# jkk-research/urban_road_filter

Hardware: AMD Instinct MI355X
Metric: scans/sec (64-ring x 2048-column cloud) (higher is better)
Workload: dtype f32+f64; 1 GPU; cfg3: batch of 1024 independent 64x2048 street sweeps per GPU, all three detectors + blind_spots, reference default parameters with ROI x,y widened to +-200 m, inputs resident in HBM (SoA x/y/z); scans_per_gpu=1024

## Files before the change

urban_road_filter_amd/csrc/urf_api.hip:

```cpp
#include <hip/hip_runtime.h>

#include <cmath>
#include <cstdio>
#include <cstdlib>
#include <cstring>
#include <ctime>
#include <string>
#include <vector>
#if defined(__SSE2__)
#include <emmintrin.h>
#include <xmmintrin.h>
#endif

#include "urf.h"
#ifdef URF_ENABLE_TEST_HOOKS
#include "urf_test_hooks.h"
#endif
#include "urf_internal.hpp"
#include "urf_kernels.hpp"
#include "urf_front.hpp"

#define URF_ASYNC_SLOTS 4
static_assert(URF_ASYNC_SLOTS == URF_MAX_IN_FLIGHT, "include/urf.h documents the number of sweeps in flight");

template <class T, bool Host = false>
struct lazy_buf {
    T* p = nullptr;
    size_t cap = 0;
    lazy_buf() = default;
    lazy_buf(const lazy_buf&) = delete;
    lazy_buf& operator=(const lazy_buf&) = delete;
    ~lazy_buf() { release(); }
    void release()
    {
        if (p)
            (void)(Host ? hipHostFree(p) : hipFree(p));
        p = nullptr;
        cap = 0;
    }
};

#define URF_SCRATCH_SCANS(X)                                                                                                     \
    X(rx, sstride) X(ry, sstride) X(rz, sstride) X(rec, sstride)                                                                 \
    X(sr, sstride) X(sz, sstride) X(sslot, sstride) X(ssrt16, sstride) X(ssrt, sstride) X(wsg, sstride)                          \
    X(big_r, sstride) X(big_z, sstride) X(big_i, sstride)                                                                        \
    X(tile_roi, max_tiles) X(roi_bits, max_tiles * (URF_TILE / 64)) X(troff, max_tiles * (URF_MAX_CHANNELS + 1))                 \
    X(tsoff, max_tiles * (URF_MAX_SECTORS + 1)) X(tmaxs, max_tiles * URF_MAX_CHANNELS)                                           \
    X(rpre, URF_MAX_CHANNELS * (max_tiles + 1)) X(rstart, URF_MAX_CHANNELS * max_tiles)                                          \
    X(angle, URF_MAX_CHANNELS) X(ring_thr, URF_MAX_CHANNELS * 4) X(ring_lut, URF_LUT_CELLS) X(ring_cnt, URF_MAX_CHANNELS)        \
    X(ring_off, URF_MAX_CHANNELS + 1)                                                                                            \
    X(sec_cnt, URF_MAX_SECTORS) X(sec_run, URF_MAX_SECTORS) X(sec_off, URF_MAX_SECTORS + 1) X(star_hit, URF_MAX_SECTORS)         \
    X(star_first, URF_MAX_SECTORS) X(star_list_mid, URF_MAX_SECTORS) X(star_list_big, URF_MAX_SECTORS)                           \
    X(star_list_runs, URF_MAX_SECTORS) X(tie_list, URF_MAX_SECTORS) X(tie_post, URF_MAX_SECTORS)                                 \
    X(table_upto, 1) X(table_redo, 1) X(redo_list, 1) X(table_cause, 1)                                                          \
    X(nan_mask, 4) X(nan_list, 2 * URF_MAX_CHANNELS) X(vis, URF_MAX_CHANNELS)                                                    \
    X(maxdist, URF_MAX_CHANNELS) X(quad, 4)                                                                                      \
    X(curb_cnt, URF_MAX_CHANNELS) X(curb_az, URF_MAX_CHANNELS * URF_CURB_LIST)                                                   \
    X(sufmin, URF_MAX_CHANNELS * URF_DEG_CELLS) X(premax, URF_MAX_CHANNELS * URF_DEG_CELLS)                                      \
    X(stop_f, URF_DEG_CELLS) X(stop_b, URF_DEG_CELLS)                                                                            \
    X(win, URF_MAX_CHANNELS * URF_DEG_CELLS)                                                                                     \
    X(info, 1)                                                                                                                   \
    X(front_ok, 1) X(front_pres, max_tiles * 64) X(front_maxs, max_tiles * 64) X(front_lane_ring, 64)                            \
    X(front_ring_lane, URF_MAX_CHANNELS) X(front_cand, front_cand_cap) X(front_all, front_cand_cap) X(front_ncand, 1)             \
    X(front_list, 1) X(front_st, URF_FRONT_ST_WORDS)
#define URF_SCRATCH_SLOTS(X) X(star_count, 8) X(ring_hint, 1)
#define URF_SCRATCH_CAPTURE(X) X(valpha, sstride) X(seckey, sstride) X(ringkey, sstride) X(rd2, sstride) X(caz, sstride)
#define URF_SCRATCH_ROW_MAJOR(X) X(tx, sstride) X(ty, sstride) X(tz, sstride) X(rows_v, 64) X(rows_ok, 1)
enum urf_scratch_group { URF_SCR_ALWAYS, URF_SCR_CAPTURE, URF_SCR_ROW_MAJOR };

struct __attribute__((visibility("hidden"))) urf_policy {
    uint32_t* flags = nullptr;
    uint64_t epoch = 1;
    bool speculate = true, use_hint = true;
    bool slot_lists = false, slot_nan = false, slot_ties = false;
    int front_mode = 1;
    uint32_t front_tpb = 0;
    bool want_ring_sorted = false;
    bool front_direct = false, front_off = false;
    bool front_rows = false, rows_oom = false, rows_used = false;
    uint32_t rows_probation = 0;

    template <class T>
    void set(T& field, T value)
    {
        if (field != value) {
            field = value;
            epoch++;
        }
    }
    void forget_front()
    {
        set(front_direct, false);
        set(front_off, false);
        flags[URF_FLAG_FRONT_HANDED_BACK] = flags[URF_FLAG_FRONT_ALL_HANDED_BACK] = 0;
    }
    int fold(urf_ctx* c, hipStream_t st);
    void probation_sweep() { lapse(front_rows); }
    void probation_batch(const urf_kargs& a) { lapse(a.front && front_mode != 2 && a.n_scans < URF_FRONT_MIN_SCANS); }
    void lapse(bool counts)
    {
        if (counts && !rows_used && rows_probation && --rows_probation == 0)
            epoch++;
    }
    bool on_redo(int status)
    {
        switch (status) {
        case URF_STATUS_REDO_TABLE: set(speculate, false); return true;
        case URF_STATUS_REDO_HINT: set(use_hint, false); return true;
        case URF_STATUS_REDO_LISTS: set(slot_lists, true); return true;
        case URF_STATUS_REDO_NAN: set(slot_nan, true); return true;
        case URF_STATUS_REDO_TIES: set(slot_ties, true); return true;
        }
        return false;
    }
    void plan(urf_kargs& a, const urf_dev_params& dp, bool slot, bool general_only) const
    {
        a.table_lookahead = speculate ? URF_TABLE_LOOKAHEAD : 0u;
        a.table_hint = (speculate && use_hint) ? 1u : 0u;
        a.optimistic = slot ? ((speculate ? URF_OPT_NO_REPAIR : 0u) | (slot_lists ? 0u : URF_OPT_NO_LISTS) | (slot_nan ? 0u : URF_OPT_NO_NAN) |
                               (slot_ties ? 0u : URF_OPT_NO_TIES)) : 0u;
        const unsigned L = (unsigned)dp.p.channels;
        const bool lasers = L == 64u || L == 32u || L == 16u;
        a.front_lsh = L == 16u ? 4u : (L == 32u ? 5u : 6u);
        const bool shape = front_mode != 0 && !front_off && !general_only && !want_ring_sorted && a.capture == 0 &&
                           lasers && dp.p.curbPoints == 5 && a.tiles <= URF_FRONT_MAX_TILES;
        const bool small_ok = front_rows && (rows_used || rows_probation > 0) && (L == 64u || front_mode == 2);
        a.front = (shape && (slot ? small_ok : (front_mode == 2 || small_ok || a.n_scans >= (L == 64u ? URF_FRONT_MIN_SCANS : (L == 32u ? URF_FRONT_MIN_SCANS_32 : URF_FRONT_MIN_SCANS_16))))) ? 1u : 0u;
        a.front_sight = (shape && !a.front && !front_rows && !rows_oom && (L == 64u || front_mode == 2)) ? 1u : 0u;
        a.front_tpb = front_tpb ? front_tpb : (a.n_scans >= URF_FRONT_TPB_SCANS ? URF_FRONT_TPB_LARGE : (a.n_scans >= 16u ? URF_FRONT_TPB_SMALL : 1u));
        a.front_lists = (a.front && !front_direct && !slot) ? 1u : 0u;
        a.front_rows = (a.front && front_rows) ? 1u : 0u;
    }
};

enum urf_last_kind { URF_LAST_NONE, URF_LAST_SOA, URF_LAST_PC2, URF_LAST_SWEEP };
struct urf_last_call {
    int kind = URF_LAST_NONE;
    uint32_t scans = 0;
    urf_kargs a;
    urf_dev_params dp;
    uint32_t row = 0;
    uint64_t gen = 0;
};

struct urf_ctx {
    int device = 0;
    uint32_t max_points = 0, max_batch = 0;
    uint32_t max_tiles = 0;
    uint32_t sstride = 0;
    uint32_t debug_flags = 0;
    unsigned n_cus = 256;
    hipStream_t own_stream = nullptr;
    hipStream_t stream = nullptr;
    urf_params params;
    urf_dev_params dp;
    urf_kargs k;
    std::vector<void*> allocs;
    lazy_buf<float> sx, sy, sz;
    struct slot_t {
        lazy_buf<uint8_t, true> h_in;
        lazy_buf<uint8_t> d_raw;
        lazy_buf<uint8_t, true> h_labels;
        lazy_buf<uint8_t> d_labels;
        lazy_buf<urf_scan_info, true> h_info;
        hipEvent_t ev_done = nullptr;
        hipGraph_t graph = nullptr;
        hipGraphExec_t exec = nullptr;
        uint64_t key[3] = { 0, 0, 0 };
        urf_kargs cap_a;
        urf_dev_params cap_dp;
        bool pending = false, used = false;
        uint64_t gen = 0;
        uint32_t n_points = 0, ticket = 0;
        uint32_t point_step = 0, off_x = 0, off_y = 0, off_z = 0;
        bool planes = false;
    } slots[URF_ASYNC_SLOTS];
    bool streams_made = false;
    urf_policy pol;
    uint32_t n_rerun = 0;
    hipStream_t row_stream[URF_ASYNC_SLOTS] = { nullptr, nullptr, nullptr, nullptr };
    hipEvent_t ev_main = nullptr;
    uint64_t main_seq = 1;
    uint64_t row_seen[URF_ASYNC_SLOTS] = { 0, 0, 0, 0 };
    uint64_t row_gen[URF_ASYNC_SLOTS] = { 0, 0, 0, 0 };
    uint32_t next_ticket = 0;
    lazy_buf<unsigned long long> ord_keys;
    lazy_buf<uint32_t> ord_pos;
    lazy_buf<uint32_t> ord_cls;
    lazy_buf<uint32_t> ord_lists;
    lazy_buf<float> mk_d;
    lazy_buf<uint32_t> mk_pos;
    lazy_buf<uint8_t> mk_red;
    lazy_buf<float> mk_out;
    lazy_buf<int32_t> mk_ghost;
    uint32_t* compact_cnt = nullptr;
    lazy_buf<urf_u32x4> cl_tiles;
    lazy_buf<uint32_t> cl_lists;
    float* d_newY = nullptr;
    urf_beam* d_beams = nullptr;
    uint32_t beams_cap = 0;
    int capture = 0;
    bool timing = false;
    std::vector<std::vector<hipEvent_t>> timing_events;
    size_t timing_used = 0;
    uint32_t* offsets_copy = nullptr;
    hipStream_t side_stream = nullptr;
    hipEvent_t ev_fork = nullptr, ev_join = nullptr;
    urf_last_call last;
    std::string last_error;
    double ht[8] = { 0, 0, 0, 0, 0, 0, 0, 0 };
    bool ht_on = false;
};

#define URF_HIP(ctx, call)                                                              \
    do {                                                                                \
        hipError_t e_ = (call);                                                         \
        if (e_ != hipSuccess) {                                                         \
            (ctx)->last_error = std::string(#call) + ": " + hipGetErrorString(e_);      \
            return e_ == hipErrorOutOfMemory ? URF_ERR_OOM : URF_ERR_HIP;               \
        }                                                                               \
    } while (0)

template <class T>
static int dev_alloc(urf_ctx* c, T** p, size_t count)
{
    void* v = nullptr;
    URF_HIP(c, hipMalloc(&v, (count ? count : 1) * sizeof(T)));
    c->allocs.push_back(v);
    *p = (T*)v;
    return URF_OK;
}

template <class T, bool Host>
static int grow(urf_ctx* c, lazy_buf<T, Host>& b, size_t count, hipStream_t st = nullptr)
{
    if (count <= b.cap)
        return URF_OK;
    if (st)
        URF_HIP(c, hipStreamSynchronize(st));
    b.release();
    void* v = nullptr;
    URF_HIP(c, Host ? hipHostMalloc(&v, count * sizeof(T), hipHostMallocDefault) : hipMalloc(&v, count * sizeof(T)));
    b.p = (T*)v;
    b.cap = count;
    return URF_OK;
}

template <class F>
static void scratch_walk(const urf_ctx* c, urf_kargs& k, F&& f)
{
    const size_t sstride = c->sstride, max_tiles = c->max_tiles, front_cand_cap = k.front_cand_cap;
#define URF_X_SCANS(field, n) f(URF_SCR_ALWAYS, k.field, (size_t)c->max_batch, (size_t)(n));
#define URF_X_SLOTS(field, n) f(URF_SCR_ALWAYS, k.field, (size_t)URF_ASYNC_SLOTS, (size_t)(n));
#define URF_X_CAPTURE(field, n) f(URF_SCR_CAPTURE, k.field, (size_t)c->max_batch, (size_t)(n));
#define URF_X_ROW_MAJOR(field, n) f(URF_SCR_ROW_MAJOR, k.field, (size_t)c->max_batch, (size_t)(n));
    URF_SCRATCH_SCANS(URF_X_SCANS)
    URF_SCRATCH_SLOTS(URF_X_SLOTS)
    URF_SCRATCH_CAPTURE(URF_X_CAPTURE)
    URF_SCRATCH_ROW_MAJOR(URF_X_ROW_MAJOR)
#undef URF_X_SCANS
#undef URF_X_SLOTS
#undef URF_X_CAPTURE
#undef URF_X_ROW_MAJOR
}

static int scratch_alloc(urf_ctx* c, urf_scratch_group group)
{
    int rc = URF_OK;
    scratch_walk(c, c->k, [&](urf_scratch_group g, auto*& p, size_t rows, size_t n) {
        if (g == group && !p && rc == URF_OK)
            rc = dev_alloc(c, &p, rows * n);
    });
    return rc;
}

int urf_policy::fold(urf_ctx* c, hipStream_t st)
{
    if (front_mode != 0 && !front_rows && !rows_oom && flags[URF_FLAG_ROWS_SIGHTED]) {
        URF_HIP(c, hipStreamSynchronize(st));
        if (scratch_alloc(c, URF_SCR_ROW_MAJOR) == URF_OK) {
            set(front_rows, true);
            rows_probation = 16;
            forget_front();
        } else {
            set(rows_oom, true);
            c->last_error.clear();
        }
    }
    if (front_rows && flags[URF_FLAG_ROWS_TAKEN])
        set(rows_used, true);
    if (flags[URF_FLAG_LOOKAHEAD_FAILED])
        set(speculate, false);
    if (flags[URF_FLAG_HINT_FAILED])
        set(use_hint, false);
    if (flags[URF_FLAG_FRONT_HANDED_BACK])
        set(front_direct, true);
    if (flags[URF_FLAG_FRONT_ALL_HANDED_BACK] && front_mode != 2)
        set(front_off, true);
    return URF_OK;
}

static void beam_init(std::vector<urf_beam>& beams, int rep, float width)
{
    beams.resize((size_t)rep);
    const float off = (float)(0.5 * (double)width);
    for (int i = 0; i < rep; i++) {
        const float fi = (float)((double)(i * 2) * M_PI / (double)rep);
        if (std::fabs(std::tan(fi)) > 1) {
            beams[i].yx = 1;
            beams[i].d = (float)std::tan(0.5 * M_PI - (double)fi);
            beams[i].o = std::fabs(off / std::sin(fi));
        } else {
            beams[i].yx = 0;
            beams[i].d = std::tan(fi);
            beams[i].o = std::fabs(off / std::cos(fi));
        }
    }
}

static float urf_angle_threshold(float angle_filter)
{
    auto alpha_of = [](float b) { return (float)((double)(urf_acosf(b) * 180.0f) / M_PI); };
    auto from_key = [](uint32_t k) {
        const uint32_t one = 0x3f800000u;
        const uint32_t u = k <= one ? 0x80000000u | (one - k) : k - one - 1u;
        float f;
        std::memcpy(&f, &u, 4);
        return f;
    };
    if (!(alpha_of(1.0f) <= angle_filter))
        return 2.0f;
    uint32_t lo = 0, hi = 2u * 0x3f800000u + 1u;
    while (lo < hi) {
        const uint32_t mid = lo + (hi - lo) / 2;
        if (alpha_of(from_key(mid)) <= angle_filter)
            hi = mid;
        else
            lo = mid + 1;
    }
    return from_key(lo);
}

static int upload_params(urf_ctx* c)
{
    const urf_params& p = c->params;
    urf_dev_params& dp = c->dp;
    dp.p = p;
    dp.slope_param = (float)((double)p.angleFilter3 * (M_PI / 180));
    dp.Kfi = (float)((double)p.sectors / (2 * M_PI));
    dp.fwd_limit = 360.0f - p.beamZone;
    dp.bwd_limit = 0.0f + p.beamZone;
    dp.inv_cp = 1.0f / (float)p.curbPoints;
    dp.x_angle_thr = urf_angle_threshold(p.angleFilter1);
    dp.z_angle_thr = urf_angle_threshold(p.angleFilter2);
    dp.sec_keybits = 1;
    while ((1u << dp.sec_keybits) <= (unsigned)p.sectors)
        dp.sec_keybits++;
    dp.ring_keybits = 1;
    while ((1u << dp.ring_keybits) <= (unsigned)p.channels)
        dp.ring_keybits++;
    dp.exp_flags = c->debug_flags;
    dp.sector_margin = URF_FAST_SECTOR_ERR * (p.sectors > 360 ? (float)p.sectors / 360.0f : 1.0f);
    std::vector<urf_beam> beams;
    beam_init(beams, p.sectors, p.beam_width);
    URF_HIP(c, hipMemcpyAsync(c->d_beams, beams.data(), beams.size() * sizeof(urf_beam), hipMemcpyHostToDevice, c->stream));
    URF_HIP(c, hipStreamSynchronize(c->stream));
    return URF_OK;
}

extern "C" int urf_create(urf_ctx** out, int device_id, uint32_t max_points, uint32_t max_batch)
{
    if (!out || max_points == 0 || max_batch == 0)
        return URF_ERR_INVALID_ARG;
    *out = nullptr;
    const unsigned long long max_tiles = ((unsigned long long)max_points + URF_TILE - 1) / URF_TILE;
    const unsigned long long sstride = max_tiles * URF_TILE + URF_SCAN_PAD;
    if (max_tiles > URF_MAX_TILES || sstride * max_batch >= (1ull << 32))
        return URF_ERR_CAPACITY;
    int ndev = 0;
    if (hipGetDeviceCount(&ndev) != hipSuccess || ndev <= 0 || device_id < 0 || device_id >= ndev)
        return URF_ERR_NO_DEVICE;
    urf_ctx* c = new urf_ctx();
    c->device = device_id;
    c->max_points = max_points;
    c->max_batch = max_batch;
    c->max_tiles = (uint32_t)max_tiles;
    c->sstride = (uint32_t)sstride;
    int rc = URF_OK;
    auto fail = [&](int code) {
        urf_destroy(c);
        return code;
    };
    if (hipSetDevice(device_id) != hipSuccess)
        return fail(URF_ERR_NO_DEVICE);
    if (hipStreamCreateWithFlags(&c->own_stream, hipStreamNonBlocking) != hipSuccess)
        return fail(URF_ERR_HIP);
    c->stream = c->own_stream;
    {
        hipDeviceProp_t prop;
        if (hipGetDeviceProperties(&prop, device_id) == hipSuccess && prop.multiProcessorCount > 0)
            c->n_cus = (unsigned)prop.multiProcessorCount;
    }
    urf_default_params(&c->params);
    std::memset(&c->k, 0, sizeof(c->k));
    std::memset(&c->last.a, 0, sizeof(c->last.a));
    urf_kargs& k = c->k;
    k.front_cand_cap = max_points / 8 > 4096 ? max_points / 8 : 4096;
    if ((rc = scratch_alloc(c, URF_SCR_ALWAYS)) != URF_OK || (rc = dev_alloc(c, &c->offsets_copy, (size_t)max_batch + 1)) != URF_OK ||
        (rc = dev_alloc(c, &c->compact_cnt, (size_t)max_batch * c->max_tiles * 4)) != URF_OK ||
        (rc = dev_alloc(c, &c->d_newY, (size_t)max_points)) != URF_OK || (rc = dev_alloc(c, &c->d_beams, (size_t)URF_MAX_SECTORS)) != URF_OK)
        return fail(rc);
    {
        urf_wu* tab = nullptr;
        const size_t nt = (size_t)max_points + 32;
        if ((rc = dev_alloc(c, &tab, nt)) != URF_OK)
            return fail(rc);
        hipLaunchKernelGGL(k_walk_table, dim3((unsigned)((nt + 255) / 256)), dim3(256), 0, c->stream, tab, (unsigned)nt);
        k.walk_tab = tab;
    }
    k.sstride = c->sstride;
    if (const char* e = std::getenv("URF_FRONT_TPB"))
        c->pol.front_tpb = (uint32_t)std::atoi(e) > 0 ? (uint32_t)std::atoi(e) : c->pol.front_tpb;
    {
        void* hp = nullptr;
        if (hipHostMalloc(&hp, URF_FLAG_WORDS * sizeof(uint32_t), hipHostMallocMapped) != hipSuccess)
            return fail(URF_ERR_HIP);
        c->pol.flags = (uint32_t*)hp;
        std::memset(hp, 0, URF_FLAG_WORDS * sizeof(uint32_t));
        if (hipMemset(k.ring_hint, 0, URF_ASYNC_SLOTS * sizeof(uint32_t)) != hipSuccess)
            return fail(URF_ERR_HIP);
        void* dp_ = nullptr;
        if (hipHostGetDevicePointer(&dp_, hp, 0) != hipSuccess)
            return fail(URF_ERR_HIP);
        k.flags = (uint32_t*)dp_;
// ... 1412 lines not shown
```

urban_road_filter_amd/csrc/urf_device.hpp:

```cpp
#ifndef URF_DEVICE_HPP
#define URF_DEVICE_HPP

#include <hip/hip_runtime.h>

#include "urf_internal.hpp"
#include "urf_libm.h"

#define URF_WAVE 64

__device__ __forceinline__ unsigned urf_lane() { return __lane_id(); }

__device__ __forceinline__ unsigned long long urf_match_any(unsigned key, unsigned nbits)
{
    unsigned long long m = ~0ull;
    for (unsigned b = 0; b < nbits; b++) {
        const bool bit = (key >> b) & 1u;
        const unsigned long long bal = __ballot(bit);
        m &= bit ? bal : ~bal;
    }
    return m;
}

__device__ __forceinline__ unsigned long long urf_match_any_fast(unsigned key, unsigned nbits)
{
// ... 45 lines not shown
}
__device__ __forceinline__ unsigned urf_wave_max(unsigned v)
{
    URF_DPP_STEP(urf_umax, 0u, 0x111, 0xf);
    URF_DPP_STEP(urf_umax, 0u, 0x112, 0xf);
    URF_DPP_STEP(urf_umax, 0u, 0x114, 0xf);
    URF_DPP_STEP(urf_umax, 0u, 0x118, 0xf);
    URF_DPP_STEP(urf_umax, 0u, 0x142, 0xa);
    URF_DPP_STEP(urf_umax, 0u, 0x143, 0xc);
    return (unsigned)__builtin_amdgcn_readlane((int)v, 63);
}

__device__ __forceinline__ unsigned urf_uadd(unsigned a, unsigned b) { return a + b; }
__device__ __forceinline__ unsigned urf_wave_scan_add(unsigned v)
{
    URF_DPP_STEP(urf_uadd, 0u, 0x111, 0xf);
    URF_DPP_STEP(urf_uadd, 0u, 0x112, 0xf);
    URF_DPP_STEP(urf_uadd, 0u, 0x114, 0xf);
    URF_DPP_STEP(urf_uadd, 0u, 0x118, 0xf);
    URF_DPP_STEP(urf_uadd, 0u, 0x142, 0xa);
    URF_DPP_STEP(urf_uadd, 0u, 0x143, 0xc);
    return v;
}
__device__ __forceinline__ unsigned urf_wave_scan_max(unsigned v)
{
    URF_DPP_STEP(urf_umax, 0u, 0x111, 0xf);
    URF_DPP_STEP(urf_umax, 0u, 0x112, 0xf);
    URF_DPP_STEP(urf_umax, 0u, 0x114, 0xf);
    URF_DPP_STEP(urf_umax, 0u, 0x118, 0xf);
    URF_DPP_STEP(urf_umax, 0u, 0x142, 0xa);
    URF_DPP_STEP(urf_umax, 0u, 0x143, 0xc);
    return v;
}

__device__ __forceinline__ void urf_wave_lds_sync()
{
    __builtin_amdgcn_fence(__ATOMIC_RELEASE, "wavefront");
    __builtin_amdgcn_wave_barrier();
    __builtin_amdgcn_fence(__ATOMIC_ACQUIRE, "wavefront");
}

__device__ __forceinline__ void urf_scan_range(const urf_kargs& a, unsigned s, unsigned& off, unsigned& len)
{
    if (a.offsets) {
        off = a.offsets[s];
        len = a.offsets[s + 1] - off;
        len = len > a.max_len ? a.max_len : len;
    } else {
        off = s * a.n_per_scan;
        len = a.n_per_scan;
    }
}

__device__ __forceinline__ unsigned urf_sbase(const urf_kargs& a, unsigned s) { return s * a.sstride; }

__device__ __forceinline__ unsigned urf_ring_slot(const urf_kargs& a, unsigned s, unsigned C, unsigned c, unsigned ntiles,
                                                  unsigned p)
{
    const unsigned* P = a.rpre + ((size_t)s * C + c) * (a.tiles + 1);
    unsigned lo = 0, hi = ntiles;
    while (hi - lo > 1) {
        const unsigned mid = (lo + hi) >> 1;
        if (P[mid] <= p)
            lo = mid;
        else
            hi = mid;
    }
    return lo * URF_TILE + a.rstart[((size_t)s * C + c) * a.tiles + lo] + (p - P[lo]);
}


__device__ __forceinline__ double urf_div_pi(double a)
{
    const double rpi = 0x1.45f306dc9c883p-2;
    const double q = a * rpi;
    const double r = __builtin_fma(-q, URF_PI_D, a);
    return __builtin_fma(r, rpi, q);
}

__device__ __forceinline__ bool urf_in_roi(const urf_params& p, float x, float y, float z)
{
    return x >= p.min_X && x <= p.max_X && y >= p.min_Y && y <= p.max_Y &&
           z >= p.min_Z && z <= p.max_Z && (x + y) + z != 0.0f;
}

__device__ __forceinline__ float urf_vertical_angle(float x, float y, float z)
{
    const float d = (float)__builtin_sqrt((double)x * (double)x + (double)y * (double)y + (double)z * (double)z);
    float b = __builtin_fabsf(z) / d;
    if (b < -1.0f)
        b = -1.0f;
    else if (b > 1.0f)
        b = 1.0f;
    if (z < 0.0f)
        return (float)urf_div_pi((double)(urf_acosf(b) * 180.0f));
    return (float)(urf_div_pi((double)(urf_asinf(b) * 180.0f)) + 90.0);
}

__device__ __forceinline__ float urf_azimuth(float x, float y, float* d_out)
{
    const float d = (float)__builtin_sqrt((double)x * (double)x + (double)y * (double)y);
    *d_out = d;
    float b = __builtin_fabsf(x) / d;
    if (b < -1.0f)
        b = -1.0f;
    else if (b > 1.0f)
        b = 1.0f;
    const double t = urf_div_pi((double)(urf_asinf(b) * 180.0f));
    if (x >= 0.0f && y <= 0.0f)
        return (float)t;
    if (x >= 0.0f && y > 0.0f)
        return (float)(180.0 - t);
    if (x < 0.0f && y >= 0.0f)
        return (float)(180.0 + t);
    return (float)(360.0 - t);
}

__device__ __forceinline__ unsigned urf_sector(float x, float y, float Kfi, unsigned sectors)
{
    float fi = urf_atan2f(y, x);
    if (fi < 0.0f)
        fi = (float)((double)fi + 2.0 * URF_PI_D);
    const int f = (int)(fi * Kfi);
    return ((unsigned)f >= sectors) ? 0u : (unsigned)f;
}

#define URF_FAST_ATAN_ERR 2.0e-6f
__device__ __forceinline__ float urf_fast_atan2f(float y, float x)
{
    const float ax = __builtin_fabsf(x), ay = __builtin_fabsf(y);
    const float mx = ax > ay ? ax : ay, mn = ax > ay ? ay : ax;
    const float t = mn * __builtin_amdgcn_rcpf(mx);
    const bool big = t > 0.41421357f;
    const float tt = big ? (t - 1.0f) * __builtin_amdgcn_rcpf(t + 1.0f) : t;
    const float v = tt * tt;
    float q = -0.06451718869358958f;
    q = __builtin_fmaf(q, v, 0.10743668324830098f);
    q = __builtin_fmaf(q, v, -0.14263949753605723f);
    q = __builtin_fmaf(q, v, 0.1999954031495797f);
    q = __builtin_fmaf(q, v, -0.33333331760434554f);
    float r = __builtin_fmaf(tt * v, q, tt);
    if (big)
        r += 0.78539816339744831f;
    if (ay > ax)
        r = 1.57079632679489662f - r;
    if (x < 0.0f)
        r = 3.14159265358979324f - r;
    return y < 0.0f ? -r : r;
}

#define URF_FAST_VALPHA_ERR 3.0e-4f
#define URF_FAST_MIN 1.0e-15f
#define URF_FAST_MAX 1.0e18f
__device__ __forceinline__ bool urf_fast_vertical_angle(float x, float y, float z, float* out)
{
    const float rho = __builtin_amdgcn_sqrtf(x * x + y * y);
    *out = urf_fast_atan2f(rho, -z) * 57.295779513082323f;
    return (rho >= URF_FAST_MIN) & (rho <= URF_FAST_MAX) & (__builtin_fabsf(z) <= 4.0f * rho);
}

#define URF_FAST_MIN2 2.0e-30f
#define URF_FAST_MAX2 1.0e36f
__device__ __forceinline__ bool urf_fast_cot(float x, float y, float z, float* u_out, bool* planar_ok)
{
    const float rho2 = x * x + y * y;
    const float u = -z * __builtin_amdgcn_rsqf(rho2);
    *u_out = u;
    *planar_ok = (rho2 >= URF_FAST_MIN2) & (rho2 <= URF_FAST_MAX2);
    return *planar_ok & (__builtin_fabsf(u) <= URF_LUT_UMAX);
}

__host__ __device__ __forceinline__ double urf_cot_deg(double deg)
{
    deg = deg < 1.0 ? 1.0 : (deg > 179.0 ? 179.0 : deg);
    const double h = (90.0 - deg) * (URF_PI_D / 360.0);
    const double v = h * h;
    double sn = -1.0 / 121645100408832000.0;
    sn = __builtin_fma(sn, v, 1.0 / 355687428096000.0);
    sn = __builtin_fma(sn, v, -1.0 / 1307674368000.0);
    sn = __builtin_fma(sn, v, 1.0 / 6227020800.0);
    sn = __builtin_fma(sn, v, -1.0 / 39916800.0);
    sn = __builtin_fma(sn, v, 1.0 / 362880.0);
    sn = __builtin_fma(sn, v, -1.0 / 5040.0);
    sn = __builtin_fma(sn, v, 1.0 / 120.0);
    sn = __builtin_fma(sn, v, -1.0 / 6.0);
    sn = __builtin_fma(sn * v, h, h);
    double cs = 1.0 / 6402373705728000.0;
    cs = __builtin_fma(cs, v, -1.0 / 20922789888000.0);
    cs = __builtin_fma(cs, v, 1.0 / 87178291200.0);
    cs = __builtin_fma(cs, v, -1.0 / 479001600.0);
    cs = __builtin_fma(cs, v, 1.0 / 3628800.0);
    cs = __builtin_fma(cs, v, -1.0 / 40320.0);
    cs = __builtin_fma(cs, v, 1.0 / 720.0);
    cs = __builtin_fma(cs, v, -1.0 / 24.0);
    cs = __builtin_fma(cs, v, 0.5);
    cs = __builtin_fma(-cs, v, 1.0);
    const double th = sn / cs;
    return 2.0 * th / (1.0 - th * th);
}

struct urf_ring_thr { float x, y, z, w; };
__device__ __forceinline__ urf_ring_thr urf_ring_thresholds(float angle, float interval, float e)
{
    const double a = (double)angle, iv = (double)interval, ee = (double)e;
    urf_ring_thr t;
    t.x = (float)urf_cot_deg(a + iv + ee);
    t.y = (float)urf_cot_deg(a + iv - ee);
    t.z = (float)urf_cot_deg(a - iv + ee);
    t.w = (float)urf_cot_deg(a - iv - ee);
    return t;
}

__device__ __forceinline__ float urf_ring_threshold(float angle, float interval, float e, unsigned which)
{
    const double a = (double)angle, iv = (double)interval, ee = (double)e;
    const double arg = which == 0 ? a + iv + ee : (which == 1 ? a + iv - ee : (which == 2 ? a - iv + ee : a - iv - ee));
    return (float)urf_cot_deg(arg);
}

#define URF_FAST_SECTOR_ERR 2.5e-4f
__device__ __forceinline__ float urf_fast_polar(float x, float y)
{
    const float fi = urf_fast_atan2f(y, x);
    return fi < 0.0f ? fi + 6.28318530717958648f : fi;
}
__device__ __forceinline__ int urf_fast_sector_of(float fi, float x, float y, float Kfi, unsigned sectors, float margin)
{
    const float mx = __builtin_fmaxf(__builtin_fabsf(x), __builtin_fabsf(y));
    const float u = fi * Kfi;
    const float f = __builtin_floorf(u);
    const float fr = u - f;
    const bool ok = (mx >= URF_FAST_MIN) & (mx <= URF_FAST_MAX) & (fr > margin) & (fr < 1.0f - margin) & (f >= 0.0f) &
                    (f < (float)sectors);
    return ok ? (int)f : -1;
}
__device__ __forceinline__ int urf_fast_sector_ranged(float fi, float Kfi, unsigned sectors, float margin)
{
    const float u = fi * Kfi;
    const float f = __builtin_floorf(u);
    const float fr = u - f;
    const bool ok = (fr > margin) & (fr < 1.0f - margin) & (f < (float)sectors);
    return ok ? (int)f : -1;
}
__device__ __forceinline__ int urf_fast_sector(float x, float y, float Kfi, unsigned sectors, float margin)
{
    return urf_fast_sector_of(urf_fast_polar(x, y), x, y, Kfi, sectors, margin);
}

#define URF_FAST_AZ_ERR 5.0e-4f
#define URF_FAST_AZ_RATIO 1024.0f
__device__ __forceinline__ float urf_fast_az_eps(float az)
{
    const float delta = __builtin_fminf(__builtin_fabsf(az - 90.0f), __builtin_fabsf(az - 270.0f));
    return URF_FAST_AZ_ERR + 6.0e-4f * __builtin_amdgcn_rcpf(__builtin_fmaxf(delta, 0.04f));
}
__device__ __forceinline__ float urf_fast_azimuth_of(float fi)
{
    const float az = fi * 57.295779513082323f + 90.0f;
    return az >= 360.0f ? az - 360.0f : az;
}
static_assert(URF_TILE == URF_REC_SRC_MASK + 1u, "the record's source field holds an index inside a tile");
__device__ __forceinline__ unsigned urf_az_code(float az)
{
    const unsigned c = (unsigned)(az * URF_REC_AZ_SCALE);
    return c < URF_REC_AZ_UNKNOWN - 1u ? c : URF_REC_AZ_UNKNOWN - 1u;
}
__device__ __forceinline__ float urf_az_decode(unsigned code)
{
    return code == URF_REC_AZ_UNKNOWN ? URF_AZ_UNKNOWN : ((float)code + 0.5f) * URF_REC_AZ_STEP;
}
__device__ __forceinline__ bool urf_fast_az_ok(float x, float y)
{
    const float ax = __builtin_fabsf(x), ay = __builtin_fabsf(y);
    return (ay * URF_FAST_AZ_RATIO >= ax) & (ay >= URF_FAST_MIN) & (ax <= URF_FAST_MAX) & (ay <= URF_FAST_MAX);
}
__device__ __forceinline__ bool urf_fast_azimuth(float x, float y, float* out)
{
    *out = urf_fast_azimuth_of(urf_fast_polar(x, y));
    return urf_fast_az_ok(x, y);
}

__device__ __forceinline__ bool urf_in_beam(const urf_beam& b, float x, float y)
{
    if (b.yx) {
        const float c = b.d * y;
        return (c - b.o) < x && x < (c + b.o);
    }
    const float c = b.d * x;
    return (c - b.o) < y && y < (c + b.o);
}

__device__ __forceinline__ float urf_sqrt_rn_normal(float x)
{
    float r = __builtin_amdgcn_sqrtf(x);
    const float rd = __uint_as_float(__float_as_uint(r) - 1u), ru = __uint_as_float(__float_as_uint(r) + 1u);
    const float ed = __builtin_fmaf(-rd, r, x), eu = __builtin_fmaf(-ru, r, x);
    r = ed <= 0.0f ? rd : r;
    r = eu > 0.0f ? ru : r;
    return r;
}

__device__ __forceinline__ unsigned urf_fbits(float f) { return __float_as_uint(f); }

#endif
```

urban_road_filter_amd/csrc/urf_front.hpp:

```cpp
#ifndef URF_FRONT_HPP
#define URF_FRONT_HPP

#define URF_FRONT_HPRE 8u
#ifndef URF_FRONT_HPOST
#define URF_FRONT_HPOST 8u
#endif
#define URF_FRONT_LANES 64u
#define URF_FRONT_STEPS (URF_TILE / URF_FRONT_LANES)
#define URF_FRONT_MIN_SCANS 192u
#define URF_FRONT_MIN_SCANS_32 0xffffffffu
#define URF_FRONT_MIN_SCANS_16 0xffffffffu
#define URF_FRONT_TPB_SMALL 2u
#define URF_FRONT_TPB_LARGE 4u
#define URF_FRONT_TPB_SCANS 512u
#define URF_FRONT_MAX_TILES 128u
#define URF_FRONT_RING_NONE 0x7fu
#define URF_FC_XZ 1u
#define URF_FC_ZZ 2u
#define URF_FC_EDGE_X 4u
#define URF_FC_EDGE_Z 8u
#ifndef URF_FRONT_NT
#define URF_FRONT_NT 0
#endif
#ifndef URF_FRONT_WAVES
#define URF_FRONT_WAVES 5
#endif

struct urf_front_thr {
    float y, z, below;
};
__device__ __forceinline__ urf_front_thr urf_front_load_thr(const urf_kargs& a, unsigned s, unsigned C, unsigned e, unsigned nR)
{
    urf_front_thr t;
    const bool valid = e < nR;
    const float4 tv = ((const float4*)a.ring_thr)[(size_t)s * C + (valid ? e : 0u)];
    const float bl = a.ring_thr[((size_t)s * C + ((valid && e) ? e - 1u : 0u)) * 4];
    t.y = valid ? tv.y : __builtin_inff();
    t.z = tv.z;
    t.below = e ? bl : __builtin_inff();
    return t;
}

__device__ __forceinline__ __amdgpu_buffer_rsrc_t urf_buf(const void* p, unsigned bytes)
{
    return __builtin_amdgcn_make_buffer_rsrc((void*)p, 0, (int)bytes, 0x00020000);
}
#define URF_OOB 0xffffffffu

__device__ __forceinline__ void urf_front_src(const urf_kargs& a, unsigned s, unsigned off, unsigned ok, const float*& gx, const float*& gy, const float*& gz)
{
    const bool rows = ok == URF_FRONT_ROWS;
    const size_t o = rows ? (size_t)urf_sbase(a, s) : (size_t)off;
    gx = (rows ? (const float*)a.tx : a.x) + o;
    gy = (rows ? (const float*)a.ty : a.y) + o;
    gz = (rows ? (const float*)a.tz : a.z) + o;
}

__global__ __launch_bounds__(256) void k_transpose(urf_kargs a)
{
    __shared__ float T[3][64 * 33];
    const unsigned s = blockIdx.y, t = blockIdx.x, tid = threadIdx.x;
    const unsigned lsh = a.front_lsh, L = 1u << lsh, wsh = 11u - lsh, W = 1u << wsh, RS = W + 1u;
    static_assert(URF_TILE == 2048u, "a tile's columns: 1 << (11 - lsh)");
    if (a.front_ok[s] != URF_FRONT_ROWS)
        return;
    unsigned off, len;
    urf_scan_range(a, s, off, len);
    const unsigned F = len >> lsh, f0 = t * W;
    if (f0 >= F)
        return;
    const unsigned c = tid & (W - 1u), r8 = tid >> wsh, RP = 256u >> wsh;
    const bool in = f0 + c < F;
    float vx[8], vy[8], vz[8];
#pragma unroll
    for (unsigned j = 0; j < 8; j++) {
        const size_t i = (size_t)off + (size_t)(j * RP + r8) * F + f0 + (in ? c : 0u);
        vx[j] = a.x[i];
        vy[j] = a.y[i];
        vz[j] = a.z[i];
    }
#pragma unroll
    for (unsigned j = 0; j < 8; j++) {
        T[0][(j * RP + r8) * RS + c] = vx[j];
        T[1][(j * RP + r8) * RS + c] = vy[j];
        T[2][(j * RP + r8) * RS + c] = vz[j];
    }
    __syncthreads();
    const size_t ob = (size_t)urf_sbase(a, s) + (size_t)f0 * L;
    const unsigned nf = F - f0 < W ? F - f0 : W;
#pragma unroll
    for (unsigned j = 0; j < 8; j++) {
        const unsigned v = j * 256u + tid, f = v >> lsh, l = v & (L - 1u);
        if (f < nf) {
            a.tx[ob + v] = T[0][l * RS + f];
            a.ty[ob + v] = T[1][l * RS + f];
            a.tz[ob + v] = T[2][l * RS + f];
        }
    }
}

#define URF_FO_ADOPT 0x20000000u
#define URF_FO_NONE 0x40000000u
#define URF_FO_FAIL 0x80000000u
__device__ __noinline__ unsigned urf_front_open(const float* tab, unsigned nR, float interval, float x, float y, float z, unsigned sectors, float Kfi,
                                                unsigned E, unsigned econf)
{
    const urf_exact_key ek = urf_exact_keys_body(tab, nR, interval, x, y, z, sectors, Kfi);
    unsigned r = sectors ? ((ek.sector + 1u) & 0x7ffu) << 1 : 0u;
    if (ek.ring == URF_RING_NONE)
        r |= URF_FO_NONE;
    else if (x == 0.0f && y == 0.0f)
        r |= URF_FO_FAIL;
    else if (ek.ring == E)
        r |= 1u;
    else if (!econf)
        r |= 1u | URF_FO_ADOPT | (ek.ring << 12);
    else
        r |= URF_FO_FAIL;
    return r;
}

#define URF_FRONT_CBUF 256u
__device__ __forceinline__ void urf_front_flush(const urf_kargs& a, unsigned s, urf_u2* cbuf, unsigned& ncb, bool& overflow)
{
    if (ncb == 0u)
        return;
    urf_wave_lds_sync();
    unsigned base = 0;
    if (urf_lane() == 0u)
        base = atomicAdd(&a.front_ncand[s], ncb);
    base = (unsigned)__builtin_amdgcn_readfirstlane((int)base);
    for (unsigned j = urf_lane(); j < ncb; j += 64u) {
        if (base + j < a.front_cand_cap)
            a.front_cand[(size_t)s * a.front_cand_cap + base + j] = cbuf[j];
        else
            overflow = true;
    }
    urf_wave_lds_sync();
    ncb = 0;
}
__device__ __forceinline__ void urf_front_push(urf_u2* cbuf, unsigned& ncb, bool has, unsigned idx, unsigned what)
{
    const unsigned long long m = __ballot(has);
    if (has)
        cbuf[ncb + urf_popc_below(m)] = urf_u2{ idx, what };
    ncb += (unsigned)__popcll(m);
}

template <bool STAR, bool BEAM, unsigned L>
__device__ __forceinline__ void urf_front_body(const urf_kargs& a, const urf_dev_params& dp, urf_u2* cbuf)
{
    const unsigned s = blockIdx.y, b = blockIdx.x, lane = threadIdx.x;
    unsigned off, len;
    urf_scan_range(a, s, off, len);
    const unsigned TPB = a.front_tpb;
    const unsigned t_first = b * TPB;
    if (t_first * URF_TILE >= len)
        return;
    const unsigned ok = a.front_ok[s];
    if (ok == 0u)
        return;
    constexpr unsigned C = L;
    constexpr unsigned STEPS = URF_TILE / L;
    static_assert(L == 64u || L == 32u || L == 16u, "a firing fills the wave, half of it or a quarter");
    const unsigned K = (unsigned)dp.p.sectors;
    const unsigned nf = (len + L - 1u) / L;
    const unsigned F0 = t_first * STEPS;
    const unsigned F1 = F0 + TPB * STEPS < nf ? F0 + TPB * STEPS : nf;
    const unsigned Fs = F0 > URF_FRONT_HPRE ? F0 - URF_FRONT_HPRE : 0u;
    const unsigned Fe = F1 + URF_FRONT_HPOST < nf ? F1 + URF_FRONT_HPOST : nf;
    const bool from_start = Fs == 0u;
    const bool to_end = Fe == nf;
    static_assert(URF_FRONT_HPRE % 4u == 0u && STEPS % 4u == 0u, "the march runs in groups of four firings");
    const unsigned sb = urf_sbase(a, s);
    const float *gx, *gy, *gz;
    urf_front_src(a, s, off, ok, gx, gy, gz);
    const __amdgpu_buffer_rsrc_t brec = urf_buf(a.rec + sb, len * 4u);
    const __amdgpu_buffer_rsrc_t bsr = urf_buf(a.sr + sb, a.tiles * URF_TILE * 4u), bsz = urf_buf(a.sz + sb, a.tiles * URF_TILE * 4u);
    const __amdgpu_buffer_rsrc_t bss = urf_buf(a.sslot + sb, a.tiles * URF_TILE * 2u);
    const unsigned nR = a.info[s].n_rings;
    const unsigned upto_v = a.table_upto[s];
    const unsigned upto = ok == URF_FRONT_ROWS ? 0u : (nR < C ? upto_v : 0xffffffffu);
    const float* const tab = a.angle + (size_t)s * dp.p.channels;
    const float curbH = dp.p.curbHeight;
    const bool use_x = dp.p.x_zero_method != 0, use_z = dp.p.z_zero_method != 0;

    unsigned E = lane;
    bool econf = false;
    urf_front_thr th = urf_front_load_thr(a, s, C, E, nR);
    bool failed = false, overflow = false;
    unsigned long long failed_m = 0;
    unsigned ncb = 0;

    float w0 = 0.f, w1 = 0.f, w2 = 0.f, w3 = 0.f, w4 = 0.f, w5 = 0.f, w6 = 0.f, w7 = 0.f, w8 = 0.f, w9 = 0.f, w10 = 0.f;
    unsigned fwA = 0, fwB = 0, fwC = 0;
    unsigned wc = 0;
    unsigned tot = 0, nin = 0;
    double maxs = 0.0;
    unsigned pw = 0;
    unsigned troi = 0, tstar = 0;
    int stepkey_v = (int)URF_SEC_NONE, stepcnt_v = 0;
    int stepkey_w = (int)URF_SEC_NONE, stepcnt_w = 0;

    auto step = [&](auto ph, const unsigned f, const float x, const float y, const float z) {
        constexpr unsigned PH = decltype(ph)::value;
        const unsigned stp = f % STEPS;
        const unsigned i = f * L + lane;
        const bool roi = (L == 64u || lane < L) && i < len && urf_in_roi(dp.p, x, y, z);
        const unsigned long long roim = __ballot(roi);
        if (PH == 1u && lane == 0u) {
            if (L == 64u)
                a.roi_bits[((size_t)s * a.tiles + f / STEPS) * STEPS + stp] = roim;
            else if (L == 32u)
                ((uint32_t*)(a.roi_bits + (size_t)s * a.tiles * (URF_TILE / 64u)))[f] = (uint32_t)roim;
            else
                ((uint16_t*)(a.roi_bits + (size_t)s * a.tiles * (URF_TILE / 64u)))[f] = (uint16_t)roim;
        }
        if (roim == 0ull)
            return;
        const float rho2 = x * x + y * y;
        const float u = -z * __builtin_amdgcn_rsqf(rho2);
        const bool fast = (rho2 >= URF_FAST_MIN2) & (rho2 <= URF_FAST_MAX2) & (__builtin_fabsf(u) <= URF_LUT_UMAX) & roi;
        const bool on_f = fast & (u >= th.y) & (u <= th.z) & (u < th.below);
        float fi = 0.f;
        int fs = -1;
        if (PH == 1u) {
            fi = urf_fast_polar(x, y);
            if (STAR)
                fs = fast ? urf_fast_sector_ranged(fi, dp.Kfi, K, dp.sector_margin) : -1;
        }
        bool on = on_f;
        const bool open = roi && !(on_f && (PH != 1u || !STAR || fs >= 0));
        if (open) {
            const unsigned r = urf_front_open(tab, nR, dp.p.interval, x, y, z, (PH == 1u && STAR) ? K : 0u, dp.Kfi, E, econf ? 1u : 0u);
            on = (r & 1u) != 0u;
            fs = (int)((r >> 1) & 0x7ffu) - 1;
            if (r & URF_FO_FAIL)
                failed = true;
            if (PH == 1u && (r & URF_FO_NONE) && i >= upto)
                a.table_redo[s] = 1u;
            if (r & URF_FO_ADOPT) {
                E = (r >> 12) & 0x7fu;
                th = urf_front_load_thr(a, s, C, E, nR);
            }
        }
        if (PH == 1u) {
            const unsigned azc_v = urf_az_code(urf_fast_azimuth_of(fi));
            const unsigned azc = urf_fast_az_ok(x, y) ? azc_v : URF_REC_AZ_UNKNOWN;
            __builtin_amdgcn_raw_buffer_store_b32((azc << URF_REC_AZ_SHIFT) | (on ? E : URF_FRONT_RING_NONE), brec, (L == 64u || lane < L) ? i * 4u : URF_OOB, 0, URF_FRONT_NT);
            if (STAR) {
                unsigned sk = (unsigned)fs;
                if (BEAM && roi && !urf_in_beam(a.beams[fs < 0 ? 0 : fs], x, y))
                    sk = URF_SEC_NONE;
                const unsigned long long psm = roim & __builtin_amdgcn_ballot_w64(sk != URF_SEC_NONE) & __builtin_amdgcn_ballot_w64((int)sk >= 0);
                const bool ons = roi && sk != URF_SEC_NONE && (int)sk >= 0;
                const unsigned src = psm ? (unsigned)__ffsll((long long)psm) - 1u : 0u;
                const unsigned f0 = psm ? (unsigned)__builtin_amdgcn_readlane((int)sk, (int)src) : URF_SEC_NONE;
                failed_m |= psm & __builtin_amdgcn_ballot_w64(sk != f0);
                const unsigned so = (f / STEPS) * URF_TILE + tstar + urf_popc_below(psm);
                const unsigned o4 = ons ? so * 4u : URF_OOB;
                const float pr = urf_sqrt_rn_normal(rho2);
                failed_m |= psm & ~(__builtin_amdgcn_ballot_w64(rho2 >= 0x1p-90f) & __builtin_amdgcn_ballot_w64(rho2 <= 0x1p126f));
                __builtin_amdgcn_raw_buffer_store_b32(__float_as_uint(pr), bsr, o4, 0, URF_FRONT_NT);
                __builtin_amdgcn_raw_buffer_store_b32(__float_as_uint(z), bsz, o4, 0, URF_FRONT_NT);
                __builtin_amdgcn_raw_buffer_store_b16((short)((stp * L + lane) | (on ? 0u : URF_SLOT_OFF)), bss, ons ? so * 2u : URF_OOB, 0, URF_FRONT_NT);
                if (STEPS <= 64u || stp < 64u) {
                    stepkey_v = lane == stp ? (int)f0 : stepkey_v;
                    stepcnt_v = lane == stp ? (int)__popcll(psm) : stepcnt_v;
                } else {
                    stepkey_w = lane == stp - 64u ? (int)f0 : stepkey_w;
                    stepcnt_w = lane == stp - 64u ? (int)__popcll(psm) : stepcnt_w;
                }
                tstar += (unsigned)__popcll(psm);
            }
            troi += (unsigned)__popcll(roim);
        }
        if (on) {
            if (PH == 1u) {
                const double s2 = (double)x * (double)x + (double)y * (double)y;
                maxs = s2 > maxs ? s2 : maxs;
                pw |= 1u << (f & 31u);
            }
            econf = true;
            w0 = w1; w1 = w2; w2 = w3; w3 = w4; w4 = w5; w5 = w6; w6 = w7; w7 = w8; w8 = w9; w9 = w10;
            w10 = z;
            fwA = __builtin_amdgcn_alignbit(fwB, fwA, 16);
            fwB = __builtin_amdgcn_alignbit(fwC, fwB, 16);
            fwC = __builtin_amdgcn_alignbit(f - Fs, fwC, 16);
            wc = wc < 11u ? wc + 1u : 11u;
            if (PH >= 1u)
                tot++;
            if (PH == 1u)
                nin++;
        }
        if (PH == 0u)
            return;
        const bool full = wc == 11u;
        const bool c_in = on & (tot >= 6u) & (tot - 5u <= nin);
        const bool p_in = on & (tot >= 4u) & (tot - 3u <= nin);
        const float a5 = __builtin_fabsf(w5);
        float m1, m2, t1, t2;
        asm("v_max3_f32 %0, |%1|, |%2|, |%3|" : "=v"(t1) : "v"(w0), "v"(w1), "v"(w2));
        asm("v_max3_f32 %0, %1, |%2|, |%3|" : "=v"(t1) : "v"(t1), "v"(w3), "v"(w4));
        asm("v_max_f32_e64 %0, %1, |%2|" : "=v"(m1) : "v"(t1), "v"(w5));
        asm("v_max3_f32 %0, |%1|, |%2|, |%3|" : "=v"(t2) : "v"(w10), "v"(w9), "v"(w8));
        asm("v_max3_f32 %0, %1, |%2|, |%3|" : "=v"(t2) : "v"(t2), "v"(w7), "v"(w6));
        asm("v_max_f32_e64 %0, %1, |%2|" : "=v"(m2) : "v"(t2), "v"(w5));
        const bool hz = ((m1 - a5 >= curbH) | (m2 - a5 >= curbH)) & (__builtin_fabsf(m1 - m2) >= 0.05f);
        const bool hx = ((__builtin_fabsf(w5 - w7) >= curbH) | (__builtin_fabsf(w10 - w7) >= curbH)) & (__builtin_fabsf(w5 - w10) >= 0.05f);
        bool zz = false, xz = false, ez = false, ex = false;
        if (use_z) {
            zz = c_in && full && hz;
            if (!from_start)
                ez = c_in && !full;
        }
        if (use_x) {
            xz = p_in && full && hx;
            if (!from_start)
                ex = p_in && !full;
        }
        if (__ballot(zz | xz | ez | ex) != 0ull) {
            urf_front_push(cbuf, ncb, zz | ez, ((fwA & 0xffffu) + Fs) * L + lane, zz ? URF_FC_ZZ : URF_FC_EDGE_Z);
            urf_front_push(cbuf, ncb, xz | ex, ((fwB & 0xffffu) + Fs) * L + lane, xz ? URF_FC_XZ : URF_FC_EDGE_X);
            if (ncb > URF_FRONT_CBUF - 128u)
                urf_front_flush(a, s, cbuf, ncb, overflow);
        }
    };
    auto pres_end = [&](const unsigned pt) {
        if (lane < L)
            a.front_pres[(size_t)s * a.tiles * 64u + (size_t)pt * L + lane] = pw;
        pw = 0;
    };
    auto tile_end = [&](const unsigned t) {
        const size_t row = (size_t)s * a.tiles + t;
        if (L == 64u) {
            a.front_pres[row * 64u + lane] = pw;
            pw = 0;
        }
        if (lane == 0)
            a.tile_roi[row] = troi;
        if (STAR && STEPS > 32u) {
            constexpr unsigned NH = STEPS > 64u ? 2u : 1u;
            unsigned fk[NH], sbase_h[NH];
            unsigned carry = 0, total = 0;
#pragma unroll
            for (unsigned h = 0; h < NH; h++) {
                const unsigned key = (unsigned)(h ? stepkey_w : stepkey_v), sc = (unsigned)(h ? stepcnt_w : stepcnt_v);
                const unsigned k1 = key != URF_SEC_NONE ? key + 1u : 0u;
                unsigned m = urf_wave_scan_max(k1);
                m = m > carry ? m : carry;
                unsigned exc = (unsigned)__shfl_up((int)m, 1);
                exc = lane == 0 ? carry : exc;
                if (__ballot(k1 != 0u && k1 < exc) != 0ull)
                    failed = true;
                fk[h] = m;
                carry = (unsigned)__builtin_amdgcn_readlane((int)m, 63);
                const unsigned sinc = urf_wave_scan_add(sc) + total;
                sbase_h[h] = sinc - sc;
                total = (unsigned)__builtin_amdgcn_readlane((int)sinc, 63);
            }
            for (unsigned k0 = 0; k0 <= K; k0 += 64u) {
                const unsigned k = k0 + lane;
                unsigned cnt = 0;
#pragma unroll
                for (unsigned h = 0; h < NH; h++) {
                    unsigned lo = 0;
#pragma unroll
                    for (unsigned st = 32u; st > 0; st >>= 1) {
                        const unsigned v = (unsigned)__shfl((int)fk[h], (int)(lo + st - 1u));
                        lo += v < k + 1u ? st : 0u;
                    }
                    const unsigned v = (unsigned)__shfl((int)fk[h], (int)lo);
                    lo += (lo == 63u && v < k + 1u) ? 1u : 0u;
                    cnt += lo;
                }
                unsigned so = total;
#pragma unroll
                for (unsigned h = 0; h < NH; h++) {
                    const unsigned v = (unsigned)__shfl((int)sbase_h[h], (int)(cnt & 63u));
                    so = (cnt >> 6) == h ? v : so;
                }
                if (k <= K)
                    a.tsoff[row * (K + 1) + k] = (uint16_t)so;
            }
        }
        if (STAR && STEPS == 32u) {
            const unsigned k1 = (lane < URF_FRONT_STEPS && (unsigned)stepkey_v != URF_SEC_NONE) ? (unsigned)stepkey_v + 1u : 0u;
            const unsigned fk = urf_wave_scan_max(k1);
            unsigned exc = (unsigned)__shfl_up((int)fk, 1);
            exc = lane == 0 ? 0u : exc;
            if (__ballot(k1 != 0u && k1 < exc) != 0ull)
                failed = true;
            const unsigned sc = lane < URF_FRONT_STEPS ? (unsigned)stepcnt_v : 0u;
            const unsigned sinc = urf_wave_scan_add(sc);
            const unsigned sbase_l = sinc - sc;
            for (unsigned k0 = 0; k0 <= K; k0 += 64u) {
                const unsigned k = k0 + lane;
                unsigned lo = 0;
#pragma unroll
                for (unsigned st = URF_FRONT_STEPS / 2; st > 0; st >>= 1) {
                    const unsigned v = (unsigned)__shfl((int)fk, (int)(lo + st - 1u));
                    lo += v < k + 1u ? st : 0u;
                }
                {
                    const unsigned v = (unsigned)__shfl((int)fk, (int)lo);
                    lo += (lo == URF_FRONT_STEPS - 1u && v < k + 1u) ? 1u : 0u;
                }
                const unsigned so = (unsigned)__shfl((int)sbase_l, (int)lo);
                if (k <= K)
                    a.tsoff[row * (K + 1) + k] = (uint16_t)so;
            }
        }
        troi = 0;
        tstar = 0;
        stepkey_v = (int)URF_SEC_NONE;
        stepcnt_v = 0;
        stepkey_w = (int)URF_SEC_NONE;
        stepcnt_w = 0;
    };

    float px[4], py[4], pz[4];
    auto ld = [&](const unsigned j, const unsigned f) {
        const unsigned i = f * L + lane, o = ((L == 64u || lane < L) && i < len) ? i : len - 1u;
        px[j] = gx[o];
        py[j] = gy[o];
        pz[j] = gz[o];
    };
#pragma unroll
    for (unsigned j = 0; j < 4; j++)
        ld(j, Fs + j);
    for (unsigned f = Fs; f < F0; f += 4) {
#pragma unroll
        for (unsigned j = 0; j < 4; j++) {
            step(std::integral_constant<unsigned, 0u>{}, f + j, px[j], py[j], pz[j]);
            ld(j, f + j + 4u);
        }
    }
    for (unsigned f = F0; f < F1; f += 4) {
#pragma unroll
        for (unsigned j = 0; j < 4; j++) {
            if (f + j < F1)
                step(std::integral_constant<unsigned, 1u>{}, f + j, px[j], py[j], pz[j]);
            ld(j, f + j + 4u);
        }
        if (L != 64u && (((f + 4u) & 31u) == 0u || f + 4u >= F1))
            pres_end(f >> 5);
        if (((f + 4u) % STEPS) == 0u || f + 4u >= F1) {
            tile_end(f / STEPS);
            if (failed_m != 0ull || __ballot(failed | overflow) != 0ull) {
                a.front_ok[s] = 0u;
                if (ok == URF_FRONT_ROWS)
                    a.table_redo[s] = 1u;
                return;
            }
        }
    }
    for (unsigned f = F1; f < Fe; f += 4) {
#pragma unroll
        for (unsigned j = 0; j < 4; j++) {
            if (f + j < Fe)
                step(std::integral_constant<unsigned, 2u>{}, f + j, px[j], py[j], pz[j]);
            ld(j, f + j + 4u);
        }
    }
    if (!to_end) {
        const unsigned fr[5] = { fwA >> 16, fwB & 0xffffu, fwB >> 16, fwC & 0xffffu, fwC >> 16 };
#pragma unroll
        for (unsigned e = 0; e < 5; e++) {
            const unsigned back = 4u - e;
            const bool in = tot > back && tot - back <= nin;
            const unsigned what = (use_z ? URF_FC_EDGE_Z : 0u) | ((use_x && e >= 2u) ? URF_FC_EDGE_X : 0u);
            if (ncb > URF_FRONT_CBUF - 64u)
                urf_front_flush(a, s, cbuf, ncb, overflow);
            urf_front_push(cbuf, ncb, in && what != 0u, (fr[e] + Fs) * L + lane, what);
        }
    }
    urf_front_flush(a, s, cbuf, ncb, overflow);
    a.front_maxs[((size_t)s * a.tiles + b) * 64u + lane] = (unsigned long long)__double_as_longlong(maxs);
    if (econf) {
        const unsigned o1 = atomicCAS(&a.front_lane_ring[(size_t)s * 64u + lane], 0xffffffffu, E);
        const unsigned o2 = atomicCAS(&a.front_ring_lane[(size_t)s * C + E], 0xffffffffu, lane);
        failed = failed | (o1 != 0xffffffffu && o1 != E) | (o2 != 0xffffffffu && o2 != lane);
    }
    if (failed_m != 0ull || __ballot(failed | overflow) != 0ull) {
        a.front_ok[s] = 0u;
        if (ok == URF_FRONT_ROWS)
            a.table_redo[s] = 1u;
    }
}

template <unsigned L>
__device__ __forceinline__ void urf_front_kernel(const urf_kargs& a, const urf_dev_params& dp, urf_u2* cbuf)
{
    if (!dp.p.star_shaped_method)
        urf_front_body<false, false, L>(a, dp, cbuf);
    else if (!dp.p.starbeam_filter)
        urf_front_body<true, false, L>(a, dp, cbuf);
    else
        urf_front_body<true, true, L>(a, dp, cbuf);
}
#define URF_FRONT_KERNEL(name, L)                                                                                                             \
    __global__ __launch_bounds__(64) __attribute__((amdgpu_waves_per_eu(URF_FRONT_WAVES, URF_FRONT_WAVES))) void name(urf_kargs a, urf_dev_params dp) \
    {                                                                                                                                         \
        __shared__ urf_u2 cbuf[URF_FRONT_CBUF];                                                                                               \
        urf_front_kernel<L>(a, dp, cbuf);                                                                                                     \
    }
URF_FRONT_KERNEL(k_front, 64u)
URF_FRONT_KERNEL(k_front32, 32u)
URF_FRONT_KERNEL(k_front16, 16u)

#define URF_FRONT_ST_WORDS 72u
#define URF_FINISH_CHUNK 768u
#ifndef URF_FINISH_THREADS
#define URF_FINISH_THREADS 256
#endif
struct urf_finish_shared {
    unsigned n[64];
    unsigned ring[64];
    unsigned ncurb[URF_FRONT_LANES];
    int q[4];
    unsigned n_pend;
    unsigned nx, nz;
    unsigned qsum[URF_FINISH_THREADS / 64][64];
};

__device__ __forceinline__ unsigned urf_front_prev(const unsigned* P, unsigned lsh, unsigned l, unsigned f)
{
    unsigned t = f >> 5;
    unsigned w = P[(t << lsh) + l] & ((1u << (f & 31u)) - 1u);
    while (w == 0u) {
        if (t == 0u)
            return 0xffffffffu;
        t--;
        w = P[(t << lsh) + l];
    }
    return t * 32u + 31u - (unsigned)__clz((int)w);
}
__device__ __forceinline__ unsigned urf_front_next(const unsigned* P, unsigned lsh, unsigned ntiles, unsigned l, unsigned f)
{
    unsigned t = f >> 5;
    unsigned w = (f & 31u) == 31u ? 0u : P[(t << lsh) + l] & ~((2u << (f & 31u)) - 1u);
    while (w == 0u) {
        t++;
        if (t >= ntiles)
            return 0xffffffffu;
        w = P[(t << lsh) + l];
    }
    return t * 32u + (unsigned)__ffs((int)w) - 1u;
}

__global__ __launch_bounds__(URF_FINISH_THREADS) void k_front_finish(urf_kargs a, urf_dev_params dp, unsigned part)
{
    __shared__ urf_finish_shared S;
    extern __shared__ unsigned sh_finish[];
    const unsigned s = blockIdx.x, tid = threadIdx.x;
    const unsigned ok = a.front_ok[s];
    if (!ok)
        return;
    unsigned off, len;
    urf_scan_range(a, s, off, len);
    const unsigned ntiles = (len + URF_TILE - 1) / URF_TILE;
    const unsigned lsh = a.front_lsh, L = 1u << lsh, lm = L - 1u;
    const unsigned npt = (((len + lm) >> lsh) + 31u) >> 5;
    const unsigned C = (unsigned)dp.p.channels, K = (unsigned)dp.p.sectors;
    const urf_scan_info in = a.info[s];
    if (in.status != URF_OK)
        return;
    unsigned* const P = sh_finish;
    uint16_t* const B = (uint16_t*)(sh_finish + a.tiles * 64u);
    urf_u2* const chunk = (urf_u2*)(sh_finish + a.tiles * 96u);
    unsigned* const st = a.front_st + (size_t)s * URF_FRONT_ST_WORDS;
    urf_u2* const pend = a.front_all + (size_t)s * a.front_cand_cap;
    const unsigned sb = urf_sbase(a, s);
    const float *gx, *gy, *gz;
    urf_front_src(a, s, off, ok, gx, gy, gz);
    auto passed = [&](unsigned idx, unsigned flag) {
        const unsigned e = atomicAdd(&S.n_pend, 1u);
        if (e < a.front_cand_cap)
            pend[e] = urf_u2{ idx, flag };
    };
    unsigned m_from = 0;
    if (part != 2u) {
    const urf_u2* const cand = a.front_cand + (size_t)s * a.front_cand_cap;
    const unsigned nc_raw = a.front_ncand[s];
    const unsigned nc = nc_raw < a.front_cand_cap ? nc_raw : a.front_cand_cap;
    for (unsigned k = tid; k < npt * L; k += URF_FINISH_THREADS)
        P[k] = a.front_pres[(size_t)s * a.tiles * 64u + k];
    if (tid < URF_FRONT_LANES)
        S.ncurb[tid] = 0;
    if (tid < 64)
        S.ring[tid] = a.front_lane_ring[(size_t)s * 64u + tid];
    if (tid == 0) {
        st[70] = 0;
        S.q[0] = (int)urf_fbits(0.f);
        S.q[1] = (int)urf_fbits(180.f);
        S.q[2] = (int)urf_fbits(180.f);
        S.q[3] = (int)urf_fbits(360.f);
        S.n_pend = 0;
    }
    __syncthreads();
    {
        constexpr unsigned NP = URF_FINISH_THREADS / 64u;
        const unsigned l = tid & 63u, prt = tid >> 6;
        const unsigned nt = l < L ? npt : 0u;
        const unsigned tq = (nt + NP - 1u) / NP, ta = prt * tq < nt ? prt * tq : nt, tb = ta + tq < nt ? ta + tq : nt;
        unsigned run = 0;
        for (unsigned t = ta; t < tb; t++)
            run += (unsigned)__popc(P[(t << lsh) + l]);
        S.qsum[prt][l] = run;
        __syncthreads();
        unsigned add = 0, all = 0;
        for (unsigned p = 0; p < NP; p++) {
            add += p < prt ? S.qsum[p][l] : 0u;
            all += S.qsum[p][l];
        }
        for (unsigned t = ta; t < tb; t++) {
            B[(t << lsh) + l] = (uint16_t)add;
            add += (unsigned)__popc(P[(t << lsh) + l]);
        }
        if (prt == 0)
            S.n[l] = all;
    }
    if (tid < C)
        a.ring_cnt[(size_t)s * C + tid] = 0;
    __syncthreads();
    if (tid < 64) {
        const unsigned r = S.ring[tid], n = r != 0xffffffffu ? S.n[tid] : 0u;
        unsigned tot = n;
        for (int o = 32; o > 0; o >>= 1)
            tot += __shfl_xor(tot, o);
        if (r != 0xffffffffu) {
            a.ring_cnt[(size_t)s * C + r] = n;
            unsigned long long m = 0;
            const unsigned nblk = (ntiles + a.front_tpb - 1u) / a.front_tpb;
            for (unsigned b0 = 0; b0 < nblk; b0 += 8u) {
                unsigned long long v[8];
#pragma unroll
                for (unsigned b = 0; b < 8; b++)
                    v[b] = a.front_maxs[((size_t)s * a.tiles + (b0 + b < nblk ? b0 + b : b0)) * 64u + tid];
#pragma unroll
                for (unsigned b = 0; b < 8; b++)
                    m = v[b] > m ? v[b] : m;
            }
            a.maxdist[(size_t)s * C + r] = (float)__builtin_sqrt(__longlong_as_double((long long)m));
            a.vis[(size_t)s * C + r] = urf_vis{ __builtin_inff(), -__builtin_inff() };
            if (r == 10u)
                st[70] = n;
        }
        if (tid == 0)
            st[69] = tot;
    }
    constexpr unsigned CH = URF_FINISH_CHUNK;
    for (unsigned c0 = 0; c0 < nc; c0 += CH) {
        const unsigned cn = nc - c0 < CH ? nc - c0 : CH;
        if (tid == 0) {
            S.nx = 0;
            S.nz = 0;
        }
        __syncthreads();
        for (unsigned e = tid; e < cn; e += URF_FINISH_THREADS) {
            const urf_u2 cd = cand[c0 + e];
            if (cd.y & (URF_FC_XZ | URF_FC_EDGE_X))
                chunk[atomicAdd(&S.nx, 1u)] = cd;
            if (cd.y & (URF_FC_ZZ | URF_FC_EDGE_Z))
                chunk[2u * CH - 1u - atomicAdd(&S.nz, 1u)] = cd;
        }
        __syncthreads();
        const unsigned nx = S.nx, nz = S.nz;
        if (dp.p.x_zero_method)
            for (unsigned e = tid; e < nx; e += URF_FINISH_THREADS) {
                const urf_u2 cd = chunk[e];
                const unsigned idx = cd.x, l = idx & lm, f = idx >> lsh;
                const unsigned n = S.n[l];
                const unsigned p = (unsigned)B[((f >> 5) << lsh) + l] + (unsigned)__popc(P[((f >> 5) << lsh) + l] & ((1u << (f & 31u)) - 1u));
                if (!(p >= 7u && p + 3u < n))
                    continue;
                unsigned fj = urf_front_prev(P, lsh, l, f);
                fj = urf_front_prev(P, lsh, l, fj);
                unsigned f3 = urf_front_next(P, lsh, npt, l, f);
                f3 = urf_front_next(P, lsh, npt, l, f3);
                f3 = urf_front_next(P, lsh, npt, l, f3);
                const unsigned ij = (fj << lsh) + l, i3 = (f3 << lsh) + l;
                const float pz = gz[idx], xj = gx[ij], yj = gy[ij], zj = gz[ij], x3 = gx[i3], y3 = gy[i3], z3 = gz[i3];
                const float nyj = a.newY[p - 2u], ny2 = a.newY[p], ny3 = a.newY[p + 3u];
                bool heights = true;
                if (cd.y & URF_FC_EDGE_X)
                    heights = (__builtin_fabsf(zj - pz) >= dp.p.curbHeight || __builtin_fabsf(z3 - pz) >= dp.p.curbHeight) &&
                              (double)__builtin_fabsf(zj - z3) >= 0.05;
                if (heights && urf_x_zero_angle_vals(nyj, ny2, ny3, dp.p.angleFilter1, dp.x_angle_thr, xj, yj, x3, y3, zj, pz, z3))
                    passed(idx, 2u);
            }
        if (dp.p.z_zero_method)
            for (unsigned e = tid; e < nz; e += URF_FINISH_THREADS) {
                const urf_u2 cd = chunk[2u * CH - 1u - e];
                const unsigned idx = cd.x, l = idx & lm, f = idx >> lsh;
                const unsigned n = S.n[l];
                const unsigned p = (unsigned)B[((f >> 5) << lsh) + l] + (unsigned)__popc(P[((f >> 5) << lsh) + l] & ((1u << (f & 31u)) - 1u));
                if (!(p >= 5u && p + 5u < n))
                    continue;
                unsigned im[5], ip[5];
                {
                    unsigned g = f;
#pragma unroll
                    for (unsigned k = 0; k < 5; k++) {
                        g = urf_front_prev(P, lsh, l, g);
                        im[k] = (g << lsh) + l;
                    }
                    g = f;
#pragma unroll
                    for (unsigned k = 0; k < 5; k++) {
                        g = urf_front_next(P, lsh, npt, l, g);
                        ip[k] = (g << lsh) + l;
                    }
                }
                const bool needz = (cd.y & URF_FC_EDGE_Z) != 0u;
                float xm[5], ym[5], zm[5] = { 0.f, 0.f, 0.f, 0.f, 0.f }, xp[5], yp[5], zp[5] = { 0.f, 0.f, 0.f, 0.f, 0.f };
                const float px = gx[idx], py = gy[idx], pz = gz[idx];
#pragma unroll
                for (unsigned k = 0; k < 5; k++) {
                    xm[k] = gx[im[k]];
                    ym[k] = gy[im[k]];
                    xp[k] = gx[ip[k]];
                    yp[k] = gy[ip[k]];
                }
                if (__ballot(needz) != 0ull) {
#pragma unroll
                    for (unsigned k = 0; k < 5; k++) {
                        zm[k] = gz[needz ? im[k] : idx];
                        zp[k] = gz[needz ? ip[k] : idx];
                    }
                }
                bool heights = true;
                if (needz) {
                    const float azp = __builtin_fabsf(pz);
                    float max1 = azp, max2 = azp;
#pragma unroll
                    for (unsigned k = 0; k < 5; k++) {
                        const float za = __builtin_fabsf(zm[k]), zb = __builtin_fabsf(zp[k]);
                        max1 = za > max1 ? za : max1;
                        max2 = zb > max2 ? zb : max2;
                    }
                    heights = (max1 - azp >= dp.p.curbHeight || max2 - azp >= dp.p.curbHeight) && (double)__builtin_fabsf(max1 - max2) >= 0.05;
                }
                if (heights) {
                    auto xy = [&](int pos, float& xx, float& yy) {
                        const int rel = pos - (int)p;
                        xx = rel < 0 ? xm[-rel - 1] : xp[rel - 1];
                        yy = rel < 0 ? ym[-rel - 1] : yp[rel - 1];
                    };
                    if (urf_z_zero_angle(dp.inv_cp, dp.p.angleFilter2, dp.z_angle_thr, xy, (int)p, 5, px, py))
                        passed(idx, 4u);
                }
            }
        __syncthreads();
    }
    } else {
        if (tid < URF_FRONT_LANES) {
            S.ncurb[tid] = st[tid];
            S.ring[tid] = a.front_lane_ring[(size_t)s * 64u + tid];
        }
        if (tid < 4)
            S.q[tid] = (int)st[64u + tid];
        if (tid == 0)
            S.n_pend = st[68];
        m_from = st[68];
        __syncthreads();
    }
    if (part != 1u && dp.p.star_shaped_method)
        for (unsigned k = tid; k < K; k += URF_FINISH_THREADS) {
            const int h = a.star_hit[(size_t)s * K + k];
            if (h >= 0)
                passed((unsigned)h, 1u);
        }
    __syncthreads();
    const unsigned n_pend = S.n_pend < a.front_cand_cap ? S.n_pend : a.front_cand_cap;
    for (unsigned e = m_from + tid; e < n_pend; e += URF_FINISH_THREADS) {
        const urf_u2 pd = pend[e];
        const unsigned idx = pd.x, r = S.ring[idx & lm];
        const float px = gx[idx], py = gy[idx];
        const unsigned old = atomicOr(&a.rec[sb + idx], pd.y << URF_REC_FLAG_SHIFT);
        float d2;
        const float az = urf_azimuth(px, py, &d2);
        urf_u2 out = urf_u2{ 0u, 0xffffffffu };
        if (((old >> URF_REC_FLAG_SHIFT) & 7u) == 0u) {
            const unsigned ec = atomicAdd(&S.ncurb[r], 1u);
            if (ec < URF_CURB_LIST)
                a.curb_az[((size_t)s * C + r) * URF_CURB_LIST + ec] = az;
            out = urf_u2{ __float_as_uint(az), r };
            if (r == 1u && dp.p.blind_spots) {
                const int ab = (int)urf_fbits(az);
                if (az >= 0.f && az < 90.f)
                    atomicMax(&S.q[0], ab);
                else if (az >= 90.f && az < 180.f)
                    atomicMin(&S.q[1], ab);
                else if (az >= 180.f && az < 270.f)
                    atomicMax(&S.q[2], ab);
                else if (az < 360.f)
                    atomicMin(&S.q[3], ab);
// ... 253 lines not shown
```

urban_road_filter_amd/csrc/urf_internal.hpp:

```cpp
#ifndef URF_INTERNAL_HPP
#define URF_INTERNAL_HPP

#include <cstddef>
#include <cstdint>

#include "urf.h"

#define URF_MAX_CHANNELS    128
#define URF_MAX_SECTORS     1022
#define URF_MAX_CURB_POINTS 30
#define URF_LUT_UMAX        4.0f
#define URF_LUT_SCALE       512.0f
#define URF_LUT_CELLS       4100
#define URF_DEG_CELLS       361

#define URF_TILE            2048
#ifndef URF_TILE_THREADS
#define URF_TILE_THREADS    512
#endif
#define URF_TILE_GROUPS     (URF_TILE / 64)
#define URF_MAX_TILES       4096
#define URF_SCAN_PAD        512
#define URF_SLOT_NONE       0xFFFFu
#define URF_SLOT_OFF        0x8000u
#define URF_TABLE_LOOKAHEAD 8192

#define URF_REC_SRC_MASK    0x7FFu
#define URF_REC_FLAG_SHIFT  11
#define URF_REC_AZ_SHIFT    14
#define URF_REC_AZ_UNKNOWN  0x3FFFFu
#define URF_REC_AZ_SCALE    (262143.0f / 360.0f)
#define URF_REC_AZ_STEP     (360.0f / 262143.0f)
#define URF_REC_AZ_QERR     9.0e-4f
#define URF_OPT_NO_REPAIR 1u
#define URF_OPT_NO_LISTS 2u
#define URF_OPT_NO_NAN 4u
#define URF_OPT_NO_TIES 8u
#define URF_STATUS_REDO_TABLE 0x7f000001
#define URF_STATUS_REDO_LISTS 0x7f000002
#define URF_STATUS_REDO_NAN 0x7f000003
#define URF_STATUS_REDO_HINT 0x7f000004
#define URF_STATUS_REDO_TIES 0x7f000005
enum urf_flag {
    URF_FLAG_LOOKAHEAD_FAILED = 0,
    URF_FLAG_HINT_FAILED = 1,
    URF_FLAG_FRONT_HANDED_BACK = 2,
    URF_FLAG_FRONT_ALL_HANDED_BACK = 3,
    URF_FLAG_ROWS_SIGHTED = 4,
    URF_FLAG_ROWS_TAKEN = 6,
    URF_FLAG_WORDS = 8
};
#define URF_TIE_FLAG 0x80000000u
#define URF_TIE_NEXT 0x40000000u
#define URF_TIE_DONE 0x20000000u
#define URF_TIE_POST 0x10000000u
#define URF_TIE_INDEX 0x00ffffffu
#define URF_TIE_CAP 2048u
#define URF_AZ_UNKNOWN      -1.0f
#define URF_RING_NONE       0xFFu
#define URF_SEC_NONE        0x3FFu

int urf_validate_params(const urf_params* p);

struct urf_beam {
    int32_t yx;
    float   d;
    float   o;
};

struct urf_dev_params {
    urf_params p;
    float    slope_param;
    float    Kfi;
    float    sector_margin;
    float    fwd_limit;
    float    bwd_limit;
    float    inv_cp;
    float    x_angle_thr;
    float    z_angle_thr;
    uint32_t sec_keybits;
    uint32_t ring_keybits;
    uint32_t exp_flags;
};

#define URF_RUNS_FLAG 0x40000000u
struct urf_sec_run { uint32_t a0, c0, a1, nruns; };

struct alignas(8) urf_sg { float slp, g; };
struct alignas(8) urf_wu { float w, u; };

struct alignas(8) urf_vis { float f_hi, b_lo; };

struct alignas(8) urf_u2 { uint32_t x, y; };

struct urf_win { float hi, lo; };

struct urf_kargs {
    const float* x;
    const float* y;
    const float* z;
    const uint32_t* offsets;
    uint32_t n_per_scan;
    uint32_t n_scans;
    uint32_t max_len;
    uint32_t tiles;
    uint32_t sstride;
    uint32_t table_lookahead;
    uint32_t table_hint;
    uint32_t optimistic;
    uint32_t capture;
    uint32_t  front;
    uint32_t  front_tpb;
    uint32_t  front_cand_cap;
    uint32_t  front_pad_;
    uint8_t* labels;
    urf_scan_info* info;
    float*    valpha;
    uint16_t* seckey;
    uint8_t*  ringkey;
    float*    caz;
    float*    rx;
    float*    ry;
    float*    rz;
    uint32_t* rec;
    float*    rd2;
    float*    sr;
    float*    sz;
    uint16_t* sslot;
    uint16_t* ssrt16;
    uint32_t* ssrt;
    urf_sg*   wsg;
    const urf_wu* walk_tab;
    uint32_t* tile_roi;
    uint16_t* troff;
    uint16_t* tsoff;
    unsigned long long* tmaxs;
    uint32_t* rpre;
    uint16_t* rstart;
    float*    angle;
    uint8_t*  ring_lut;
    float*    ring_thr;
    uint32_t* ring_cnt;
    uint32_t* ring_off;
    uint32_t* sec_cnt;
    urf_sec_run* sec_run;
    uint32_t* sec_off;
    int32_t*  star_hit;
    uint32_t* star_first;
    uint32_t* star_list_mid;
    uint32_t* star_list_big;
    uint32_t* star_list_runs;
    uint32_t* tie_list;
    uint32_t* tie_post;
    uint32_t* star_count;
    uint32_t* table_upto;
    uint32_t* table_redo;
    uint32_t* redo_list;
    uint32_t* table_cause;
    uint32_t* ring_hint;
    uint32_t* flags;
    float*    big_r;
    float*    big_z;
    uint32_t* big_i;
    uint32_t* nan_mask;
    uint32_t* nan_list;
    urf_vis*  vis;
    float*    maxdist;
    float*    quad;
    uint32_t* curb_cnt;
    float*    curb_az;
    float*    sufmin;
    float*    premax;
    int16_t*  stop_f;
    int16_t*  stop_b;
    unsigned long long* roi_bits;
    urf_win*  win;
    const float*    newY;
    const urf_beam* beams;
    uint32_t* front_ok;
    uint32_t* front_pres;
    unsigned long long* front_maxs;
    uint32_t* front_lane_ring;
    uint32_t* front_ring_lane;
    urf_u2*   front_cand;
    urf_u2*   front_all;
    uint32_t* front_ncand;
    uint32_t* front_st;
    uint32_t* front_list;
    uint32_t  front_lsh;
    uint32_t  front_lists;
    uint32_t  front_rows;
    uint32_t  front_sight;
    float*    rows_v;
    uint32_t* rows_ok;
    float*    tx;
    float*    ty;
    float*    tz;
};
#define URF_FRONT_ROWS 2u

#endif
```

urban_road_filter_amd/csrc/urf_k_split.hpp:

```cpp
#ifndef URF_K_SPLIT_HPP
#define URF_K_SPLIT_HPP

#define URF_SLOT(lp) ((lp) + ((lp) >> 5))
#define URF_SLOTS (URF_TILE + URF_TILE / 32)
#define URF_TILE_WAVES (URF_TILE_THREADS / 64)
#define URF_WAVE_PTS (URF_TILE / URF_TILE_WAVES)

__host__ __device__ inline unsigned urf_align16(unsigned v) { return (v + 15u) & ~15u; }

#define URF_SPLIT_MISC_WORDS 336
__host__ __device__ inline size_t urf_split_lds_bytes(unsigned C, unsigned K, bool star)
{
    const unsigned Ks = star ? K : 0;
    const size_t fixed = URF_MAX_CHANNELS * (4 + 4 + 16) + urf_align16(URF_LUT_CELLS) + urf_align16((C + 1) * 4) +
                         urf_align16((Ks + 1) * 4) + URF_SPLIT_MISC_WORDS * 4 + urf_align16(C * 8);
    const size_t phase_a = 5 * (size_t)URF_TILE + urf_align16(2 * URF_TILE_WAVES * (C + Ks));
    const size_t phase_b = 4 * (size_t)URF_SLOTS * 4;
    return fixed + (phase_a > phase_b ? phase_a : phase_b);
}

struct urf_exact_key {
    unsigned ring, sector;
    float valpha;
};
// ... 592 lines not shown
            const unsigned sl = URF_SLOT(lp[q]);
            stx[sl] = __float_as_uint(x);
            sty[sl] = __float_as_uint(y);
            stz[sl] = __float_as_uint(z);
            str[sl] = (azc[q] << URF_REC_AZ_SHIFT) | li;
        }
        if (sp[q] != 0xffffffffu) {
            const unsigned so = sp[q] & (URF_TILE - 1u);
            __builtin_nontemporal_store(__builtin_sqrtf(x * x + y * y), &o_sr[so]);
            __builtin_nontemporal_store(z, &o_sz[so]);
            __builtin_nontemporal_store((uint16_t)(lp[q] != 0xffffffffu ? lp[q] : URF_SLOT_NONE), &o_ss[so]);
        }
    }
    __syncthreads();
    URF_PHASE_MARK;
    const unsigned tile_ring_pts = koff[C];
    {
        float* __restrict__ const o_rx = a.rx + tb;
        float* __restrict__ const o_ry = a.ry + tb;
        float* __restrict__ const o_rz = a.rz + tb;
        uint32_t* __restrict__ const o_rec = a.rec + tb;
        for (unsigned j = tid; j < tile_ring_pts; j += URF_TILE_THREADS) {
            const unsigned sl = URF_SLOT(j);
            __builtin_nontemporal_store(__uint_as_float(stx[sl]), &o_rx[j]);
            __builtin_nontemporal_store(__uint_as_float(sty[sl]), &o_ry[j]);
            __builtin_nontemporal_store(__uint_as_float(stz[sl]), &o_rz[j]);
            __builtin_nontemporal_store(str[sl], &o_rec[j]);
        }
    }
    const size_t row = (size_t)s * a.tiles + t;
    for (unsigned k = tid; k <= C; k += URF_TILE_THREADS)
        a.troff[row * (C + 1) + k] = (uint16_t)koff[k];
    for (unsigned k = tid; k < C; k += URF_TILE_THREADS)
        a.tmaxs[row * C + k] = tmax[k];
    if (star)
        for (unsigned k = tid; k <= K; k += URF_TILE_THREADS)
            a.tsoff[row * (K + 1) + k] = (uint16_t)soff[k];
    if (tid == 0)
        a.tile_roi[row] = misc[0];
    URF_PHASE_MARK;
    URF_PHASE_DUMP("k_split");
}

__global__ __launch_bounds__(URF_TILE_THREADS) __attribute__((amdgpu_waves_per_eu(URF_SPLIT_WAVES_PER_EU, URF_SPLIT_WAVES_PER_EU))) void k_split(urf_kargs a, urf_dev_params dp)
{
    extern __shared__ __attribute__((aligned(16))) unsigned char sh_split[];
    if (blockIdx.x == 0 && blockIdx.y == 0 && threadIdx.x == 0)
        *a.ring_hint = 0;
    if (a.front && __builtin_amdgcn_readfirstlane((int)((const uint32_t* __restrict__)a.front_ok)[blockIdx.y]))
        return;
    urf_split_tile(a, dp, blockIdx.y, blockIdx.x, sh_split, threadIdx.x);
}

__global__ __launch_bounds__(URF_TILE_THREADS) __attribute__((amdgpu_waves_per_eu(URF_SPLIT_WAVES_PER_EU, URF_SPLIT_WAVES_PER_EU))) void k_split_repair(urf_kargs a, urf_dev_params dp)
{
    extern __shared__ __attribute__((aligned(16))) unsigned char sh_split[];
    const unsigned n = a.star_count[2];
    for (unsigned w = blockIdx.x; w < n * a.tiles; w += gridDim.x) {
        unsigned tid_i = threadIdx.x;
        asm volatile("" : "+v"(tid_i));
        urf_split_tile(a, dp, a.redo_list[w / a.tiles], w % a.tiles, sh_split, tid_i);
        __syncthreads();
    }
}

__global__ __launch_bounds__(URF_TILE_THREADS) __attribute__((amdgpu_waves_per_eu(URF_SPLIT_WAVES_PER_EU, URF_SPLIT_WAVES_PER_EU))) void k_split_list(urf_kargs a, urf_dev_params dp)
{
    extern __shared__ __attribute__((aligned(16))) unsigned char sh_split[];
    if (blockIdx.x == 0 && threadIdx.x == 0)
        *a.ring_hint = 0;
    const unsigned n = a.star_count[6];
    for (unsigned w = blockIdx.x; w < n * a.tiles; w += gridDim.x) {
        unsigned tid_i = threadIdx.x;
        asm volatile("" : "+v"(tid_i));
        urf_split_tile(a, dp, a.front_list[w / a.tiles], w % a.tiles, sh_split, tid_i);
        __syncthreads();
    }
}

__device__ void urf_scan_keys_256(const unsigned* cnt, unsigned* offs, unsigned K, unsigned* sh )
{
    const unsigned tid = threadIdx.x;
    unsigned v[4], sum = 0;
    for (int e = 0; e < 4; e++) {
        const unsigned k = tid * 4 + e;
        v[e] = k < K ? cnt[k] : 0;
        sum += v[e];
    }
    const unsigned inc = urf_wave_scan_add(sum);
    __syncthreads();
    if (urf_lane() == 63)
        sh[tid >> 6] = inc;
    __syncthreads();
    unsigned wbase = 0;
    for (unsigned w = 0; w < (tid >> 6); w++)
        wbase += sh[w];
    unsigned run = wbase + inc - sum;
    for (int e = 0; e < 4; e++) {
        const unsigned k = tid * 4 + e;
        if (k < K)
            offs[k] = run;
        run += v[e];
        if (k + 1 == K)
            offs[K] = run;
    }
    __syncthreads();
}

struct urf_index_shared {
    uint16_t cnt[64][66];
    uint16_t st[64][66];
    unsigned carry[64];
};
__device__ void urf_index_family(urf_index_shared& L, const uint16_t* toff, unsigned nkeys, unsigned k0, unsigned ntiles,
                                 unsigned tstride, unsigned* pre, uint16_t* start, unsigned* cnt)
{
    const unsigned tid = threadIdx.x, lane = tid & 63, wave = tid >> 6;
    const unsigned rowlen = nkeys + 1;
    if (k0 < nkeys) {
        const unsigned key = k0 + lane;
        if (tid < 64)
            L.carry[tid] = 0;
        for (unsigned t0 = 0; t0 < ntiles; t0 += 64) {
            unsigned fv0[16], fv1[16];
#pragma unroll
            for (unsigned pass = 0; pass < 16; pass++) {
                const unsigned tt = t0 + pass * 4 + wave;
                const bool in = tt < ntiles && key < nkeys;
                const unsigned idx = in ? tt * rowlen + key : 0u;
                fv0[pass] = toff[idx];
                fv1[pass] = toff[idx + 1];
                fv0[pass] = in ? fv0[pass] : 0u;
                fv1[pass] = in ? fv1[pass] : 0u;
            }
#pragma unroll
            for (unsigned pass = 0; pass < 16; pass++) {
                const unsigned u = pass * 4 + wave;
                L.cnt[lane][u] = (uint16_t)(fv1[pass] - fv0[pass]);
                L.st[lane][u] = (uint16_t)fv0[pass];
            }
            __syncthreads();
#pragma unroll 4
            for (unsigned pass = 0; pass < 16; pass++) {
                const unsigned r = pass * 4 + wave, kk = k0 + r, tt = t0 + lane;
                const unsigned c = L.cnt[r][lane];
                const unsigned incl = urf_wave_scan_add(c);
                const unsigned base = L.carry[r];
                if (kk < nkeys && tt < ntiles) {
                    pre[(size_t)kk * (tstride + 1) + tt] = base + incl - c;
                    start[(size_t)kk * tstride + tt] = L.st[r][lane];
                }
                if (lane == 63)
                    L.carry[r] = base + incl;
            }
            __syncthreads();
        }
        if (tid < 64 && key < nkeys) {
            pre[(size_t)key * (tstride + 1) + ntiles] = L.carry[tid];
            cnt[key] = L.carry[tid];
        }
        __syncthreads();
    }
}

__device__ __forceinline__ unsigned urf_scan_piece(const urf_kargs& a, unsigned s, unsigned ntiles, unsigned* sh )
{
    const unsigned tid = threadIdx.x;
    unsigned piece = 0;
    for (unsigned t = tid; t < ntiles; t += 256)
        piece += a.tile_roi[(size_t)s * a.tiles + t];
    for (int o = 32; o > 0; o >>= 1)
        piece += __shfl_xor(piece, o);
    if (urf_lane() == 0)
        sh[tid >> 6] = piece;
    __syncthreads();
    piece = sh[0] + sh[1] + sh[2] + sh[3];
    __syncthreads();
    return piece;
}

template <unsigned NK>
__device__ __forceinline__ void urf_index_sectors(const urf_kargs& a, unsigned s, unsigned K, unsigned ntiles)
{
    const unsigned tid = threadIdx.x;
    const uint16_t* toff = a.tsoff + (size_t)s * a.tiles * (K + 1);
    for (unsigned kp = 0; kp < K; kp += 256 * NK) {
        unsigned run[NK], mx[NK];
        urf_sec_run sr[NK];
#pragma unroll
        for (unsigned h = 0; h < NK; h++) {
            run[h] = 0;
            mx[h] = 0;
            sr[h] = urf_sec_run{ 0u, 0u, 0u, 0u };
        }
        for (unsigned t0 = 0; t0 < ntiles; t0 += 16) {
            unsigned v0[NK][16], v1[NK][16];
#pragma unroll
            for (unsigned h = 0; h < NK; h++)
#pragma unroll
                for (unsigned u = 0; u < 16; u++) {
                    const unsigned k = kp + h * 256 + tid;
                    const bool in = t0 + u < ntiles && k < K;
                    const unsigned idx = in ? (t0 + u) * (K + 1) + k : 0u;
                    v0[h][u] = (unsigned)toff[idx];
                    v1[h][u] = (unsigned)toff[idx + 1];
                    v0[h][u] = in ? v0[h][u] : 0u;
                    v1[h][u] = in ? v1[h][u] : 0u;
                }
#pragma unroll
            for (unsigned h = 0; h < NK; h++)
#pragma unroll
                for (unsigned u = 0; u < 16; u++) {
                    const unsigned c = v1[h][u] - v0[h][u], ad = (t0 + u) * URF_TILE + v0[h][u];
                    const bool first = (c != 0u) & (sr[h].nruns == 0u), second = (c != 0u) & (sr[h].nruns == 1u);
                    sr[h].a0 = first ? ad : sr[h].a0;
                    sr[h].c0 = first ? c : sr[h].c0;
                    sr[h].a1 = second ? ad : sr[h].a1;
                    sr[h].nruns += c != 0u;
                    run[h] += c;
                    mx[h] = c > mx[h] ? c : mx[h];
                }
        }
#pragma unroll
        for (unsigned h = 0; h < NK; h++) {
            const unsigned k = kp + h * 256 + tid;
            if (k < K) {
                if (sr[h].nruns > 2u && ntiles <= 64u && mx[h] <= URF_STAR_SMALL_CAP / 64u)
                    sr[h].nruns |= URF_RUNS_FLAG;
                a.sec_cnt[(size_t)s * K + k] = run[h];
                a.sec_run[(size_t)s * K + k] = sr[h];
            }
        }
    }
}

__device__ __forceinline__ void urf_index_body(const urf_kargs& a, const urf_dev_params& dp, urf_index_shared& L, unsigned* sh)
{
    const unsigned s = blockIdx.x, tid = threadIdx.x;
    unsigned off, len;
    urf_scan_range(a, s, off, len);
    const unsigned ntiles = (len + URF_TILE - 1) / URF_TILE;
    const unsigned C = (unsigned)dp.p.channels, K = (unsigned)dp.p.sectors;
    if ((a.optimistic & URF_OPT_NO_REPAIR) && a.table_redo[s]) {
        if (tid == 0)
            a.info[s].status = (a.table_cause[s] & 3u) == 2u ? URF_STATUS_REDO_HINT : URF_STATUS_REDO_TABLE;
        return;
    }
    if (a.optimistic & URF_OPT_NO_NAN) {
        const uint4 nm = *(const uint4*)(a.nan_mask + (size_t)s * 4);
        if (nm.x | nm.y | nm.z | nm.w) {
            if (tid == 0)
                a.info[s].status = URF_STATUS_REDO_NAN;
            return;
        }
    }
    {
        const unsigned piece = urf_scan_piece(a, s, ntiles, sh);
        if (tid == 0) {
            a.info[s].n_roi = piece;
            if (piece < 30) {
                a.info[s].status = URF_TOO_FEW_POINTS;
                a.info[s].n_rings = 0;
            }
        }
        if (piece < 30)
            return;
    }
    if (dp.p.star_shaped_method) {
        urf_index_sectors<1u>(a, s, K, ntiles);
    }
    const bool fused = a.front && a.front_ok[s];
    if (fused && tid == 0)
        atomicMax(a.ring_hint, a.info[s].n_rings);
    if (!fused) {
    for (unsigned k0 = 0; k0 < C; k0 += 64)
        urf_index_family(L, a.troff + (size_t)s * a.tiles * (C + 1), C, k0, ntiles, a.tiles, a.rpre + (size_t)s * C * (a.tiles + 1),
                         a.rstart + (size_t)s * C * a.tiles, a.ring_cnt + (size_t)s * C);
    urf_scan_keys_256(&a.ring_cnt[(size_t)s * C], &a.ring_off[(size_t)s * (C + 1)], C, sh);
    }
    if (!fused) {
        unsigned tot = 0;
        for (unsigned k = tid; k < C; k += 256)
            tot += a.ring_cnt[(size_t)s * C + k];
        for (int o = 32; o > 0; o >>= 1)
            tot += __shfl_xor(tot, o);
        if (urf_lane() == 0)
            sh[4 + (tid >> 6)] = tot;
        __syncthreads();
        if (tid == 0) {
            urf_scan_info* o = &a.info[s];
            o->n_ring_pts = sh[4] + sh[5] + sh[6] + sh[7];
            o->n_ring10 = o->n_rings > 10 ? a.ring_cnt[(size_t)s * C + 10] : 0;
            atomicMax(a.ring_hint, o->n_rings);
        }
    }
    if (!dp.p.star_shaped_method)
        return;
    __syncthreads();
    urf_scan_keys_256(&a.sec_cnt[(size_t)s * K], &a.sec_off[(size_t)s * (K + 1)], K, sh);
    for (unsigned k0 = 0; k0 < K; k0 += 256) {
        const unsigned k = k0 + tid;
        const unsigned c = k < K ? a.sec_cnt[(size_t)s * K + k] : 0;
        const unsigned nr = k < K ? a.sec_run[(size_t)s * K + k].nruns : 0;
        const bool runs = (nr & URF_RUNS_FLAG) != 0u && c >= 2 && c <= URF_STAR_SMALL_CAP;
        const bool mid = (c > URF_STAR_SMALL_CAP || (nr > 2 && c >= 2 && !runs)) && c <= URF_STAR_MID_CAP_, big = c > URF_STAR_MID_CAP_;
        const unsigned long long bm = __ballot(mid), bb = __ballot(big), br = __ballot(runs);
        unsigned pm = 0, pb = 0, pr = 0;
        if ((a.optimistic & URF_OPT_NO_LISTS) && (bm | bb | br) && urf_lane() == 0)
            a.info[s].status = URF_STATUS_REDO_LISTS;
        if (urf_lane() == 0) {
            if (bm)
                pm = atomicAdd(&a.star_count[0], (unsigned)__popcll(bm));
            if (bb)
                pb = atomicAdd(&a.star_count[1], (unsigned)__popcll(bb));
            if (br)
                pr = atomicAdd(&a.star_count[7], (unsigned)__popcll(br));
        }
        pm = __shfl(pm, 0);
        pb = __shfl(pb, 0);
        pr = __shfl(pr, 0);
        if (runs)
            a.star_list_runs[pr + urf_popc_below(br)] = s * K + k;
        if (mid)
            a.star_list_mid[pm + urf_popc_below(bm)] = s * K + k;
        if (big)
            a.star_list_big[pb + urf_popc_below(bb)] = s * K + k;
    }
}

__global__ __launch_bounds__(256) void k_index(urf_kargs a, urf_dev_params dp)
{
    __shared__ urf_index_shared L;
    __shared__ unsigned sh[8];
    urf_index_body(a, dp, L, sh);
}


#endif
```

urban_road_filter_amd/csrc/urf_k_star.hpp:

```cpp
#ifndef URF_K_STAR_HPP
#define URF_K_STAR_HPP


__device__ __forceinline__ unsigned long long urf_wave_sort64(unsigned long long key)
{
    const unsigned lane = urf_lane();
#pragma unroll
    for (unsigned kk = 2; kk <= 64; kk <<= 1) {
#pragma unroll
        for (unsigned j = kk >> 1; j > 0; j >>= 1) {
            const unsigned lo = __shfl_xor((unsigned)key, (int)j);
            const unsigned hi = __shfl_xor((unsigned)(key >> 32), (int)j);
            const unsigned long long other = ((unsigned long long)hi << 32) | lo;
            const bool lower = (lane & j) == 0;
            const bool up = (lane & kk) == 0 || kk == 64;
            const bool take_min = lower == up;
            const bool other_less = other < key;
            key = (take_min == other_less) ? other : key;
        }
    }
    return key;
}

__device__ __forceinline__ unsigned urf_count_less64(const unsigned long long* blk, unsigned long long key)
{
    unsigned pos = 0;
#pragma unroll
    for (unsigned step = 32; step > 0; step >>= 1)
        if (blk[pos + step - 1] < key)
            pos += step;
    if (blk[pos] < key)
        pos++;
    return pos;
}

struct urf_run_row {
    unsigned st, cnt;
};
__device__ __forceinline__ urf_run_row urf_sector_run_row(const urf_kargs& a, unsigned s, unsigned K, unsigned k, unsigned t0)
{
    const unsigned t = t0 + urf_lane();
    const uint16_t* row = a.tsoff + ((size_t)s * a.tiles + (t < a.tiles ? t : 0)) * (K + 1) + k;
    urf_run_row r;
    r.st = (unsigned)row[0];
    r.cnt = (unsigned)row[1] - r.st;
    return r;
}
__device__ __forceinline__ unsigned urf_sector_runs(const urf_kargs& a, unsigned s, unsigned K, unsigned k, unsigned ntiles,
                                                    const urf_run_row& first, unsigned* runP, unsigned* runA)
{
    const unsigned lane = urf_lane();
    unsigned nr = 0, carry = 0;
    for (unsigned t0 = 0; t0 < ntiles; t0 += 64) {
        const unsigned t = t0 + lane;
        urf_run_row r = first;
        if (t0)
            r = urf_sector_run_row(a, s, K, k, t0);
        const unsigned c = t < ntiles ? r.cnt : 0;
        const unsigned inc = urf_wave_scan_add(c);
        const unsigned p0 = carry + inc - c;
        const unsigned long long m = __ballot(c != 0);
        if (c) {
            const unsigned idx = nr + urf_popc_below(m);
            runP[idx] = p0;
            runA[idx] = t * URF_TILE + r.st - p0;
        }
        nr += (unsigned)__popcll(m);
        carry += (unsigned)__shfl((int)inc, 63);
    }
    return nr;
}

template <unsigned MAXB, bool RUNS = false>
__device__ __forceinline__ bool urf_star_sort_sector(const urf_kargs& a, const urf_dev_params& dp, unsigned sb, unsigned obase, unsigned n,
                                                     const urf_sec_run& two, unsigned long long* A, unsigned* cnt,
                                                     unsigned* sh_first, uint32_t* star_first_out, unsigned run_adr = 0, unsigned run_cnt = 0)
{
    constexpr unsigned NB = URF_STAR_NB, PL = NB / 64;
    auto CI = [](unsigned c) { return c; };
    const unsigned lane = threadIdx.x;
    const unsigned Bn = (n + 63) >> 6;
    const unsigned B = RUNS ? urf_wave_max(run_cnt) : Bn;
    URF_PHASE_ACC_DECL;
    unsigned long long key[MAXB];
    float zreg[MAXB];
    unsigned sreg[MAXB];
    unsigned rmin = 0xffffffffu, rmax = 0;
    {
        const unsigned a1m = two.a1 - two.c0;
        unsigned adr[MAXB], rbv[MAXB], slv[MAXB];
#pragma unroll
        for (unsigned q = 0; q < MAXB; q++) {
            const unsigned i = q * 64 + lane, ic = i < n ? i : n - 1u;
            adr[q] = RUNS ? run_adr + (q < run_cnt ? q : 0u) : ic + (ic < two.c0 ? two.a0 : a1m);
        }
#pragma unroll
        for (unsigned q = 0; q < MAXB; q++) {
            rbv[q] = 0;
            zreg[q] = 0.f;
            slv[q] = 0;
            if (q < B) {
                rbv[q] = urf_fbits(a.sr[sb + adr[q]]);
                zreg[q] = a.sz[sb + adr[q]];
                if (RUNS)
                    slv[q] = a.sslot[sb + adr[q]];
            }
        }
#pragma unroll
        for (unsigned q = 0; q < MAXB; q++) {
            const bool valid = RUNS ? q < run_cnt : q * 64 + lane < n;
            sreg[q] = RUNS ? ((slv[q] & URF_SLOT_OFF) ? 0xffffffffu : (adr[q] & ~(URF_TILE - 1u)) + slv[q]) : q * 64 + lane;
            key[q] = valid ? ((unsigned long long)rbv[q] << 32) | adr[q] : ~0ull;
            rmin = valid && rbv[q] < rmin ? rbv[q] : rmin;
            rmax = valid && rbv[q] > rmax ? rbv[q] : rmax;
        }
    }
    for (unsigned c = lane; c <= NB; c += 64)
        cnt[c] = 0;
    rmin = urf_wave_min(rmin);
    rmax = urf_wave_max(rmax);
    const unsigned range = rmax - rmin;
    const unsigned sh = range < NB ? 0u : (unsigned)(32 - __clz((int)range)) - URF_STAR_LOG_NB;
    __syncthreads();
    URF_PHASE_ACC(0);

    unsigned bkt[MAXB], wq[MAXB];
#pragma unroll
    for (unsigned q = 0; q < MAXB; q++) {
        bkt[q] = 0;
        wq[q] = 0;
        if (q < B && key[q] != ~0ull) {
            bkt[q] = ((unsigned)(key[q] >> 32) - rmin) >> sh;
            wq[q] = atomicAdd(&cnt[CI(bkt[q])], 1u);
        }
    }
    __syncthreads();
    URF_PHASE_ACC(1);
    unsigned maxc = 0;
    {
        unsigned c8[PL], sum = 0;
#pragma unroll
        for (unsigned e = 0; e < PL; e++) {
            c8[e] = cnt[CI(lane * PL + e)];
            sum += c8[e];
            maxc = c8[e] > maxc ? c8[e] : maxc;
        }
        unsigned inc = sum;
        for (int o = 1; o < 64; o <<= 1) {
            const unsigned w = __shfl_up(inc, o);
            if ((int)lane >= o)
                inc += w;
        }
        unsigned run = inc - sum;
#pragma unroll
        for (unsigned e = 0; e < PL; e++) {
            cnt[CI(lane * PL + e)] = run;
            run += c8[e];
        }
        if (lane == 63)
            cnt[CI(NB)] = run;
        for (int o = 32; o > 0; o >>= 1) {
            const unsigned w = __shfl_xor(maxc, o);
            maxc = w > maxc ? w : maxc;
        }
    }
    __syncthreads();
    URF_PHASE_ACC(2);

    unsigned rank[MAXB];
    if (maxc <= 64 && !(dp.exp_flags & 4u)) {
        unsigned ol[MAXB];
#pragma unroll
        for (unsigned q = 0; q < MAXB; q++) {
            ol[q] = 1;
            if (!(q < B && key[q] != ~0ull))
                bkt[q] = 0xffff0000u + q;
        }
#pragma unroll
        for (unsigned q = 0; q < MAXB; q++)
#pragma unroll
            for (unsigned r = q + 1; r < MAXB; r++) {
                const unsigned same = bkt[q] == bkt[r];
                const unsigned lt = key[q] < key[r];
                ol[q] += same + ((same & (lt ^ 1u)) << 8);
                ol[r] += same + ((same & lt) << 8);
            }
        bool need = false;
        unsigned bb[MAXB];
#pragma unroll
        for (unsigned q = 0; q < MAXB; q++) {
            bb[q] = 0;
            if (q < B && key[q] != ~0ull) {
                const unsigned b0 = cnt[CI(bkt[q])];
                bb[q] = b0 | ((cnt[CI(bkt[q] + 1)] - b0) << 16);
                need = need || (bb[q] >> 16) != (ol[q] & 0xffu);
            }
            rank[q] = (bb[q] & 0xffffu) + (ol[q] >> 8);
        }
        if (__any(need)) {
            static_assert(MAXB * 64 <= 384, "the rank slots live behind the keys in A");
            uint16_t* RK = (uint16_t*)(A + 384);
#pragma unroll
            for (unsigned q = 0; q < MAXB; q++)
                if (q < B && key[q] != ~0ull) {
                    const unsigned pos = (bb[q] & 0xffffu) + wq[q];
                    A[pos] = key[q];
                    RK[pos] = (bb[q] >> 16) != (ol[q] & 0xffu) ? (uint16_t)0xffffu : (uint16_t)0;
                }
            __syncthreads();
#pragma unroll
            for (unsigned q = 0; q < MAXB; q++) {
                const unsigned pos = q * 64 + lane;
                if (q < Bn && pos < n && RK[pos] == 0xffffu) {
                    const unsigned long long kk = A[pos];
                    const unsigned bk = ((unsigned)(kk >> 32) - rmin) >> sh;
                    const unsigned b0 = cnt[CI(bk)], b1 = cnt[CI(bk + 1)];
                    unsigned r = b0, t = b0;
                    for (; t + 3 < b1; t += 4) {
                        const unsigned long long k0 = A[t], k1 = A[t + 1], k2 = A[t + 2], k3 = A[t + 3];
                        r += (k0 < kk) + (k1 < kk) + (k2 < kk) + (k3 < kk);
                    }
                    if (t + 1 < b1) {
                        const unsigned long long k0 = A[t], k1 = A[t + 1];
                        r += (k0 < kk) + (k1 < kk);
                        t += 2;
                    }
                    if (t < b1)
                        r += A[t] < kk;
                    RK[pos] = (uint16_t)r;
                }
            }
            __syncthreads();
#pragma unroll
            for (unsigned q = 0; q < MAXB; q++)
                if (q < B && key[q] != ~0ull && (bb[q] >> 16) != (ol[q] & 0xffu))
                    rank[q] = RK[(bb[q] & 0xffffu) + wq[q]];
        }
    } else {
#pragma unroll
        for (unsigned q = 0; q < MAXB; q++)
            if (q < B) {
                key[q] = urf_wave_sort64(key[q]);
                A[q * 64 + lane] = key[q];
                if (key[q] != ~0ull) {
                    const unsigned adr = (unsigned)key[q];
                    zreg[q] = a.sz[sb + adr];
                    if (RUNS) {
                        const unsigned sl = a.sslot[sb + adr];
                        sreg[q] = (sl & URF_SLOT_OFF) ? 0xffffffffu : (adr & ~(URF_TILE - 1u)) + sl;
                    } else {
                        sreg[q] = (two.nruns == 2 && adr >= two.a1) ? two.c0 + (adr - two.a1) : adr - two.a0;
                    }
                }
            }
        __syncthreads();
#pragma unroll
        for (unsigned q = 0; q < MAXB; q++) {
            rank[q] = lane;
            if (q < B && key[q] != ~0ull)
                for (unsigned p = 0; p < B; p++)
                    if (p != q)
                        rank[q] += urf_count_less64(A + p * 64, key[q]);
        }
    }
    __syncthreads();
    URF_PHASE_ACC(3);
    uint2* RZ = (uint2*)A;
    unsigned* S = cnt;
    static_assert(URF_STAR_NB + 1 >= MAXB * 64, "S reuses the bucket counters: one word per point of the sector");
#pragma unroll
    for (unsigned q = 0; q < MAXB; q++)
        if (q < B && key[q] != ~0ull) {
            RZ[rank[q]] = make_uint2((unsigned)(key[q] >> 32), __float_as_uint(zreg[q]));
            S[rank[q]] = sreg[q];
        }
    __syncthreads();
    URF_PHASE_ACC(4);
    const float slope_param = dp.slope_param, kdist = dp.p.kdist_param;
    bool tie = false;
#pragma unroll
    for (unsigned q = 0; q < MAXB; q++) {
        const unsigned i = q * 64 + lane;
        if (q * 64 >= n)
            break;
        if (i < n) {
            float slp = 0.f, g = 0.f;
            if (i >= 1) {
                const uint2 pa = RZ[i - 1], pb = RZ[i];
                const float ax = __uint_as_float(pa.x), bx = __uint_as_float(pb.x);
                slp = (__uint_as_float(pb.y) - __uint_as_float(pa.y)) / (bx - ax);
                g = (bx - ax) * kdist;
                tie = tie || (pa.x == pb.x && pa.y != pb.y);
                if (slp > slope_param)
                    atomicMin(sh_first, i);
            }
            if (RUNS)
                a.ssrt[obase + i] = S[i];
            else
                a.ssrt16[obase + i] = (uint16_t)S[i];
            a.wsg[obase + i] = urf_sg{ slp, g };
        }
        __syncthreads();
        if (*sh_first < (q + 1) * 64)
            break;
    }
    const unsigned first = *sh_first;
    unsigned next = 0;
    if (lane == 0 && first < n)
        for (unsigned j = first + 1; j < n && RZ[j].x == RZ[first].x; j++) {
            next = URF_TIE_NEXT;
            tie = tie || RZ[j].y != RZ[first].y;
        }
    const bool any_tie = __any(tie);
    if (lane == 0)
        *star_first_out = (first < n - 1 ? first : n - 1) | (any_tie ? URF_TIE_FLAG : 0u) | next;
    URF_PHASE_ACC(5);
#ifdef URF_EXP_PHASE_CLOCK
    if (threadIdx.x == 0 && blockIdx.y == gridDim.y / 2 && blockIdx.x >= 100 && blockIdx.x < 104)
        printf("k_star_sort_small sector %u n %u: load %llu count %llu scan %llu rank %llu place %llu tail %llu\n", blockIdx.x, n, ph_t[0], ph_t[1], ph_t[2], ph_t[3], ph_t[4], ph_t[5]);
#endif
    return any_tie;
}

__device__ __forceinline__ void urf_tie_found(const urf_kargs& a, unsigned s, unsigned sk)
{
    a.tie_list[atomicAdd(&a.star_count[4], 1u)] = sk;
    if (a.optimistic & URF_OPT_NO_TIES)
        a.info[s].status = URF_STATUS_REDO_TIES;
}


#ifndef URF_SMALL_WAVES
#define URF_SMALL_WAVES 6
#endif
__global__ __launch_bounds__(URF_STAR_THREADS) __attribute__((amdgpu_waves_per_eu(URF_SMALL_WAVES, URF_SMALL_WAVES))) void k_star_sort_small(urf_kargs a, urf_dev_params dp)
{
    constexpr unsigned NB = URF_STAR_NB;
    __shared__ unsigned long long A[8 * 64];
    __shared__ unsigned cnt[NB + 1];
    __shared__ unsigned sh_first;
    const unsigned k = blockIdx.x, s = blockIdx.y, lane = threadIdx.x;
    const unsigned K = (unsigned)dp.p.sectors;
    const int status = a.info[s].status;
    const unsigned so0 = a.sec_off[(size_t)s * (K + 1) + k], so1 = a.sec_off[(size_t)s * (K + 1) + k + 1];
    const urf_sec_run two = a.sec_run[(size_t)s * K + k];
    if (status != URF_OK)
        return;
    const unsigned n = so1 - so0;
    if (n > URF_STAR_SMALL_CAP || (two.nruns > 2 && n >= 2))
        return;
    if (n < 2) {
        if (lane == 0)
            a.star_first[(size_t)s * K + k] = 0;
        return;
    }
    const unsigned sb = urf_sbase(a, s), obase = sb + so0;
    if (lane == 0)
        sh_first = n;
    const bool tie = urf_star_sort_sector<URF_STAR_SMALL_CAP / 64>(a, dp, sb, obase, n, two, A, cnt, &sh_first, &a.star_first[(size_t)s * K + k]);
    if (tie && lane == 0)
        urf_tie_found(a, s, s * K + k);
}

__global__ __launch_bounds__(URF_STAR_THREADS) __attribute__((amdgpu_waves_per_eu(5, 5))) void k_star_sort_runs(urf_kargs a, urf_dev_params dp)
{
    constexpr unsigned NB = URF_STAR_NB;
    __shared__ unsigned long long A[8 * 64];
    __shared__ unsigned cnt[NB + 1];
    __shared__ unsigned sh_first;
    const unsigned count = a.star_count[7], lane = threadIdx.x;
    const unsigned K = (unsigned)dp.p.sectors;
    for (unsigned w = blockIdx.x; w < count; w += gridDim.x) {
        const unsigned sk = a.star_list_runs[w], s = sk / K, k = sk % K;
        if (a.info[s].status != URF_OK)
            continue;
        unsigned off, len;
        urf_scan_range(a, s, off, len);
        const unsigned ntiles = (len + URF_TILE - 1) / URF_TILE;
        const unsigned so0 = a.sec_off[(size_t)s * (K + 1) + k], so1 = a.sec_off[(size_t)s * (K + 1) + k + 1];
        const urf_sec_run two = a.sec_run[sk];
        const unsigned n = so1 - so0;
        unsigned c0 = 0, c1 = 0;
        if (lane < ntiles) {
            const uint16_t* row = a.tsoff + ((size_t)s * a.tiles + lane) * (K + 1) + k;
            c0 = row[0];
            c1 = row[1];
        }
        const unsigned sb = urf_sbase(a, s), obase = sb + so0;
        if (lane == 0)
            sh_first = n;
        const bool tie = urf_star_sort_sector<URF_STAR_SMALL_CAP / 64, true>(a, dp, sb, obase, n, two, A, cnt, &sh_first, &a.star_first[sk],
                                                                              c1 > c0 ? lane * URF_TILE + c0 : 0u, c1 - c0);
        if (tie && lane == 0)
            urf_tie_found(a, s, sk);
        __syncthreads();
    }
}

template <int NT>
__device__ __forceinline__ void urf_bitonic_keys(unsigned long long* keys, unsigned n)
{
    unsigned P = 1;
    while (P < n)
        P <<= 1;
    for (unsigned kk = 2; kk <= P; kk <<= 1) {
        for (unsigned j = kk >> 1; j > 0; j >>= 1) {
            const bool flip = (j == (kk >> 1));
            for (unsigned tt = threadIdx.x; tt < (P >> 1); tt += NT) {
                const unsigned lo = ((tt & ~(j - 1)) << 1) | (tt & (j - 1));
                const unsigned hi = flip ? ((lo & ~(kk - 1)) + (kk - 1) - (lo & (kk - 1))) : lo + j;
                if (hi < n) {
                    const unsigned long long ka = keys[lo], kb = keys[hi];
                    if (ka > kb) {
                        keys[lo] = kb;
                        keys[hi] = ka;
                    }
                }
            }
            __syncthreads();
        }
    }
}

struct urf_sort_shared {
    unsigned rmin, rmax, maxc;
    unsigned w[8];
};
#define URF_BLOCK_CNT(NB, NT) ((NB) + 1)
template <int NT, int EPT, int NB>
__device__ __forceinline__ void urf_block_rank_keys(unsigned long long (&key)[EPT], unsigned n, unsigned long long* A,
                                                    unsigned* cnt, urf_sort_shared* sh, bool force_general, unsigned (&rank)[EPT] URF_PH_PARAMS)
{
    static_assert(NB % NT == 0 && NT / 64 <= 8, "bucket scan layout");
    auto CI = [](unsigned c) { return c; };
    const unsigned tid = threadIdx.x, lane = tid & 63, wave = tid >> 6;
    if (tid == 0) {
        unsigned ones = 0xffffffffu, zero = 0u;
        asm volatile("" : "+v"(ones), "+v"(zero));
        sh->rmin = ones;
        sh->rmax = zero;
        sh->maxc = zero;
    }
    for (unsigned c = tid; c <= NB; c += NT)
        cnt[c] = 0;
    __syncthreads();
    URF_PHASE_ACC(4);
    unsigned rmin = 0xffffffffu, rmax = 0;
#pragma unroll
    for (int e = 0; e < EPT; e++)
        if (key[e] != ~0ull) {
            const unsigned rb = (unsigned)(key[e] >> 32);
            rmin = rb < rmin ? rb : rmin;
            rmax = rb > rmax ? rb : rmax;
        }
    rmin = urf_wave_min(rmin);
    rmax = urf_wave_max(rmax);
    if (lane == 0) {
        atomicMin(&sh->rmin, rmin);
        atomicMax(&sh->rmax, rmax);
    }
    __syncthreads();
    URF_PHASE_ACC(5);
    rmin = sh->rmin;
    const unsigned range = sh->rmax - rmin;
    unsigned shf = 0;
    while ((range >> shf) >= (unsigned)NB)
        shf++;
    unsigned bkt[EPT], wq[EPT];
#pragma unroll
    for (int e = 0; e < EPT; e++) {
        bkt[e] = 0;
        wq[e] = 0;
        if (key[e] != ~0ull) {
            bkt[e] = ((unsigned)(key[e] >> 32) - rmin) >> shf;
            wq[e] = atomicAdd(&cnt[CI(bkt[e])], 1u);
        }
    }
    __syncthreads();
    URF_PHASE_ACC(6);
    {
        unsigned c8[NB / NT], sum = 0, maxc = 0;
#pragma unroll
        for (int e = 0; e < NB / NT; e++) {
            c8[e] = cnt[CI(tid * (NB / NT) + e)];
            sum += c8[e];
            maxc = c8[e] > maxc ? c8[e] : maxc;
        }
        const unsigned inc = urf_wave_scan_add(sum);
        if (lane == 63)
            sh->w[wave] = inc;
        maxc = urf_wave_max(maxc);
        if (lane == 0)
            atomicMax(&sh->maxc, maxc);
        __syncthreads();
        unsigned run = inc - sum;
        for (unsigned v = 0; v < wave; v++)
            run += sh->w[v];
#pragma unroll
        for (int e = 0; e < NB / NT; e++) {
            cnt[CI(tid * (NB / NT) + e)] = run;
            run += c8[e];
        }
        if (tid == NT - 1)
            cnt[CI(NB)] = run;
    }
    __syncthreads();
    URF_PHASE_ACC(7);
    if (sh->maxc <= 256 && !force_general) {
#pragma unroll
        for (int e = 0; e < EPT; e++)
            if (key[e] != ~0ull)
                A[cnt[CI(bkt[e])] + wq[e]] = key[e];
        __syncthreads();
        URF_PHASE_ACC(8);
#pragma unroll
        for (int e = 0; e < EPT; e++) {
            const unsigned pos = tid + (unsigned)e * NT;
            key[e] = pos < n ? A[pos] : ~0ull;
        }
#pragma unroll
        for (int e = 0; e < EPT; e++) {
            rank[e] = 0;
            if (key[e] != ~0ull) {
                const unsigned b = ((unsigned)(key[e] >> 32) - rmin) >> shf;
                const unsigned b0 = cnt[CI(b)], b1 = cnt[CI(b + 1)];
                unsigned r = b0, t = b0;
                for (; t + 1 < b1; t += 2) {
                    const unsigned long long k0 = A[t], k1 = A[t + 1];
                    r += (k0 < key[e]) + (k1 < key[e]);
                }
                if (t < b1)
                    r += A[t] < key[e];
                rank[e] = r;
            }
        }
        __syncthreads();
        URF_PHASE_ACC(9);
    } else {
#pragma unroll
        for (int e = 0; e < EPT; e++) {
            const unsigned i = tid + (unsigned)e * NT;
            if (i < n)
                A[i] = key[e];
        }
        __syncthreads();
        urf_bitonic_keys<NT>(A, n);
#pragma unroll
        for (int e = 0; e < EPT; e++) {
            unsigned lo = 0, hi = n;
            while (lo < hi) {
                const unsigned mid = (lo + hi) >> 1;
                if (A[mid] < key[e])
                    lo = mid + 1;
                else
                    hi = mid;
            }
            rank[e] = lo;
        }
        __syncthreads();
    }
}

template <int NT, int EPT, int NB>
__device__ __forceinline__ void urf_block_sort_keys(unsigned long long (&key)[EPT], unsigned n, unsigned long long* A,
                                                    unsigned* cnt, urf_sort_shared* sh, bool force_general)
{
    unsigned rank[EPT];
    URF_PHASE_ACC_DECL;
    urf_block_rank_keys<NT, EPT, NB>(key, n, A, cnt, sh, force_general, rank URF_PH_ARGS);
#pragma unroll
    for (int e = 0; e < EPT; e++)
        if (key[e] != ~0ull)
            A[rank[e]] = key[e];
    __syncthreads();
}

#ifndef URF_STAR_MID_THREADS
#define URF_STAR_MID_THREADS 512
#endif
#define URF_STAR_MID_CAP 2048
#ifndef URF_MID_WAVES
#define URF_MID_WAVES 8
#endif
__global__ __launch_bounds__(URF_STAR_MID_THREADS) __attribute__((amdgpu_waves_per_eu(URF_MID_WAVES, URF_MID_WAVES))) void k_star_sort_mid(urf_kargs a, urf_dev_params dp)
{
    constexpr unsigned NT = URF_STAR_MID_THREADS, NB = 2048, EPT = URF_STAR_MID_CAP / NT;
    __shared__ unsigned long long A[URF_STAR_MID_CAP];
    __shared__ unsigned cnt[URF_BLOCK_CNT(NB, NT)];
    __shared__ urf_sort_shared ssh;
    __shared__ unsigned sh_first, sh_nruns, sh_tie;
    const unsigned K = (unsigned)dp.p.sectors;
    const unsigned count = a.star_count[0];
    const unsigned tid = threadIdx.x;
    URF_PHASE_ACC_DECL;
    auto list_entry = [&](unsigned w) -> unsigned { return w < count ? a.star_list_mid[w] : 0u; };
    auto rfl = [](unsigned v) -> unsigned { return (unsigned)__builtin_amdgcn_readfirstlane((int)v); };
    struct urf_mid_desc {
        unsigned sk, n, so, a0, c0, a1, nruns;
    };
    urf_mid_desc cur;
    cur.sk = rfl(list_entry(blockIdx.x));
    {
        const urf_sec_run t = a.sec_run[cur.sk];
        cur.n = rfl(a.sec_cnt[cur.sk]);
        cur.so = rfl(a.sec_off[(size_t)(cur.sk / K) * (K + 1) + cur.sk % K]);
        cur.a0 = rfl(t.a0);
        cur.c0 = rfl(t.c0);
        cur.a1 = rfl(t.a1);
        cur.nruns = rfl(t.nruns);
    }
    unsigned sk_next = rfl(list_entry(blockIdx.x + gridDim.x));
    for (unsigned w = blockIdx.x; w < count; w += gridDim.x) {
        const unsigned sk = cur.sk;
        const unsigned s = sk / K, k = sk % K;
        unsigned off, len;
        urf_scan_range(a, s, off, len);
        const unsigned n = cur.n;
        const unsigned sb = urf_sbase(a, s);
        const unsigned obase = sb + cur.so;
        const unsigned two_a0 = cur.a0, two_c0 = cur.c0, two_a1 = cur.a1;
        const bool simple = cur.nruns <= 2u;
        unsigned* runP = (unsigned*)A;
        unsigned* runA = runP + URF_STAR_MID_CAP;
        if (!simple && tid < 64) {
            const unsigned nr = urf_sector_runs(a, s, K, k, (len + URF_TILE - 1) / URF_TILE, urf_sector_run_row(a, s, K, k, 0), runP, runA);
            if (tid == 0)
                sh_nruns = nr;
        }
        if (tid == 0) {
            sh_first = n;
            sh_tie = 0;
        }
        __syncthreads();
        URF_PHASE_ACC(0);
        const unsigned nruns = simple ? 0u : sh_nruns;
        unsigned long long key[EPT];
        float zreg[EPT];
        unsigned sreg[EPT];
        unsigned r = 0;
#pragma unroll
        for (unsigned e = 0; e < EPT; e++) {
            const unsigned i = tid + e * NT;
            key[e] = ~0ull;
            zreg[e] = 0.f;
            sreg[e] = 0;
            if (i < n) {
                unsigned adr = i < two_c0 ? two_a0 + i : two_a1 + (i - two_c0);
                if (!simple) {
                    while (r + 1 < nruns && i >= runP[r + 1])
                        r++;
                    adr = runA[r] + i;
                }
                key[e] = ((unsigned long long)urf_fbits(a.sr[sb + adr]) << 32) | adr;
            }
        }
        const unsigned n_nx = a.sec_cnt[sk_next];
        const unsigned so_nx = a.sec_off[(size_t)(sk_next / K) * (K + 1) + sk_next % K];
        const urf_sec_run two_nx = a.sec_run[sk_next];
        const unsigned sk_nx2 = list_entry(w + 2 * gridDim.x);
        __syncthreads();
        URF_PHASE_ACC(1);
        unsigned rank[EPT];
        urf_block_rank_keys<NT, EPT, NB>(key, n, A, cnt, &ssh, (dp.exp_flags & 4u) != 0, rank URF_PH_ARGS);
#pragma unroll
        for (unsigned e = 0; e < EPT; e++)
            if (key[e] != ~0ull) {
                const unsigned adr = (unsigned)key[e];
                zreg[e] = a.sz[sb + adr];
                if (simple) {
                    sreg[e] = adr >= two_a1 && two_a1 > two_a0 ? two_c0 + (adr - two_a1) : adr - two_a0;
                } else {
                    const unsigned sl = a.sslot[sb + adr];
                    sreg[e] = (sl & URF_SLOT_OFF) ? 0xffffffffu : (adr & ~(URF_TILE - 1u)) + sl;
                }
            }
        URF_PHASE_ACC(2);
        unsigned* R = (unsigned*)A;
        float* Z = (float*)A + URF_STAR_MID_CAP;
        unsigned* S = cnt;
#pragma unroll
        for (unsigned e = 0; e < EPT; e++)
            if (key[e] != ~0ull) {
                R[rank[e]] = (unsigned)(key[e] >> 32);
                Z[rank[e]] = zreg[e];
                S[rank[e]] = sreg[e];
            }
        {
            urf_mid_desc nx;
            nx.sk = sk_next;
            nx.n = rfl(n_nx);
            nx.so = rfl(so_nx);
            nx.a0 = rfl(two_nx.a0);
            nx.c0 = rfl(two_nx.c0);
            nx.a1 = rfl(two_nx.a1);
            nx.nruns = rfl(two_nx.nruns);
// ... 106 lines not shown
            R[i] = a.sr[adr];
            Z[i] = a.sz[adr];
            I[i] = (sl & URF_SLOT_OFF) ? 0xffffffffu : lo * URF_TILE + sl;
            Pq[i] = i;
        }
        __threadfence_block();
        __syncthreads();
        unsigned P2 = 1;
        while (P2 < n)
            P2 <<= 1;
        for (unsigned kk = 2; kk <= P2; kk <<= 1) {
            for (unsigned j = kk >> 1; j > 0; j >>= 1) {
                const bool flip = (j == (kk >> 1));
                for (unsigned tt = threadIdx.x; tt < (P2 >> 1); tt += 256) {
                    const unsigned lo = ((tt & ~(j - 1)) << 1) | (tt & (j - 1));
                    const unsigned hi = flip ? ((lo & ~(kk - 1)) + (kk - 1) - (lo & (kk - 1))) : lo + j;
                    if (hi < n) {
                        const unsigned long long ka = ((unsigned long long)urf_fbits(R[lo]) << 32) | Pq[lo];
                        const unsigned long long kb = ((unsigned long long)urf_fbits(R[hi]) << 32) | Pq[hi];
                        if (ka > kb) {
                            const float r0 = R[lo], z0 = Z[lo];
                            const unsigned i0 = I[lo], p0 = Pq[lo];
                            R[lo] = R[hi]; Z[lo] = Z[hi]; I[lo] = I[hi]; Pq[lo] = Pq[hi];
                            R[hi] = r0; Z[hi] = z0; I[hi] = i0; Pq[hi] = p0;
                        }
                    }
                }
                __threadfence_block();
                __syncthreads();
            }
        }
        unsigned first = n;
        for (unsigned i = threadIdx.x; i < n; i += 256) {
            float slp = 0.f, g = 0.f;
            if (i >= 1) {
                slp = (Z[i] - Z[i - 1]) / (R[i] - R[i - 1]);
                g = (R[i] - R[i - 1]) * kdist;
                if (R[i] == R[i - 1])
                    sh_tie = 1u;
                if (slp > slope_param && i < first)
                    first = i;
            }
            a.wsg[base + i] = urf_sg{ slp, g };
        }
        __syncthreads();
        for (unsigned i = threadIdx.x; i < n; i += 256)
            a.ssrt[base + i] = I[i];
        atomicMin(&sh_first, first);
        __syncthreads();
        if (threadIdx.x == 0) {
            a.star_first[sk] = (sh_first < n - 1 ? sh_first : n - 1) | (sh_tie ? URF_TIE_FLAG : 0u);
            if (sh_tie)
                urf_tie_found(a, s, sk);
        }
        __syncthreads();
    }
}

__device__ __forceinline__ int urf_walk_slot_to_ring_pos(const urf_kargs& a, unsigned s, unsigned C, unsigned v);
struct urf_tie_lds {
    typedef unsigned* rptr;
    typedef unsigned* iptr;
    static __device__ __forceinline__ void sync() { urf_wave_lds_sync(); }
};
struct urf_tie_glb {
    typedef volatile unsigned* rptr;
    typedef volatile unsigned* iptr;
    static __device__ __forceinline__ void sync()
    {
        __threadfence_block();
        __builtin_amdgcn_wave_barrier();
    }
};

template <class RP_, class IP_>
__device__ void urf_tie_adjust_heap(RP_ R, IP_ P, unsigned f, int hole, int len, unsigned v, unsigned pv)
{
    const int top = hole;
    int second = hole;
    while (second < (len - 1) / 2) {
        second = 2 * (second + 1);
        if (R[f + second] < R[f + second - 1])
            second--;
        R[f + hole] = R[f + second];
        P[f + hole] = P[f + second];
        hole = second;
    }
    if ((len & 1) == 0 && second == (len - 2) / 2) {
        second = 2 * (second + 1);
        R[f + hole] = R[f + second - 1];
        P[f + hole] = P[f + second - 1];
        hole = second - 1;
    }
    int parent = (hole - 1) / 2;
    while (hole > top && R[f + parent] < v) {
        R[f + hole] = R[f + parent];
        P[f + hole] = P[f + parent];
        hole = parent;
        parent = (hole - 1) / 2;
    }
    R[f + hole] = v;
    P[f + hole] = pv;
}
template <class RP_, class IP_>
__device__ __noinline__ void urf_tie_heap_sort(RP_ R, IP_ P, unsigned f, unsigned l)
{
    const int len = (int)(l - f);
    if (len >= 2) {
        int parent = (len - 2) / 2;
        for (;;) {
            urf_tie_adjust_heap(R, P, f, parent, len, R[f + parent], P[f + parent]);
            if (parent == 0)
                break;
            parent--;
        }
    }
    for (int last = len - 1; last >= 1; last--) {
        const unsigned v = R[f + last], pv = P[f + last];
        R[f + last] = R[f];
        P[f + last] = P[f];
        urf_tie_adjust_heap(R, P, f, 0, last, v, pv);
    }
}

template <class MEM>
__device__ __forceinline__ unsigned urf_tie_partition(typename MEM::rptr R, typename MEM::iptr P, typename MEM::iptr LP, typename MEM::iptr RP,
                                                      unsigned f, unsigned l)
{
    const unsigned lane = threadIdx.x;
    {
        const unsigned mid = f + (l - f) / 2;
        const unsigned va = R[f + 1], vb = R[mid], vc = R[l - 1];
        unsigned m;
        if (va < vb)
            m = vb < vc ? mid : (va < vc ? l - 1 : f + 1);
        else if (va < vc)
            m = f + 1;
        else if (vb < vc)
            m = l - 1;
        else
            m = mid;
        if (lane == 0) {
            const unsigned r0 = R[f], p0 = P[f];
            R[f] = R[m];
            P[f] = P[m];
            R[m] = r0;
            P[m] = p0;
        }
        MEM::sync();
    }
    const unsigned pv = R[f];
    unsigned tL = 0, tR = 0;
    for (unsigned c0 = f + 1; c0 < l; c0 += 64) {
        const unsigned p = c0 + lane;
        const bool in = p < l;
        const unsigned v = in ? R[p] : 0u;
        const bool isL = in && v >= pv, isR = in && v <= pv;
        const unsigned long long mL = __ballot(isL), mR = __ballot(isR);
        if (isL)
            LP[f + 1 + tL + urf_popc_below(mL)] = p;
        if (isR)
            RP[f + 1 + tR + urf_popc_below(mR)] = p;
        tL += (unsigned)__popcll(mL);
        tR += (unsigned)__popcll(mR);
    }
    MEM::sync();
    const unsigned mn = tL < tR ? tL : tR;
    unsigned ks = 0;
    for (unsigned k0 = 0; k0 < mn; k0 += 64) {
        const unsigned kk = k0 + lane;
        const bool in = kk < mn;
        const unsigned lp = in ? LP[f + 1 + kk] : 0u, rp = in ? RP[f + tR - kk] : 0u;
        const bool ok = in && lp < rp;
        const unsigned long long mo = __ballot(ok), mi = __ballot(in);
        if (ok) {
            const unsigned r0 = R[lp], p0 = P[lp], r1 = R[rp], p1 = P[rp];
            R[lp] = r1;
            P[lp] = p1;
            R[rp] = r0;
            P[rp] = p0;
        }
        ks += (unsigned)__popcll(mo);
        if (mo != mi)
            break;
    }
    MEM::sync();
    const unsigned Lk = ks < tL ? LP[f + 1 + ks] : 0xffffffffu;
    const unsigned Rk = ks > 0 ? RP[f + 1 + tR - ks] : 0xffffffffu;
    return Lk < Rk ? Lk : Rk;
}

template <class MEM>
__device__ __forceinline__ void urf_tie_introsort_loop(unsigned n, typename MEM::rptr R, typename MEM::iptr P, typename MEM::iptr LP,
                                                       typename MEM::iptr RP, int* stk)
{
    const unsigned lane = threadIdx.x;
    const unsigned limit = 2u * (31u - (unsigned)__clz((int)n));
    int top = 0;
    unsigned f = 0, l = n, d = 0;
    for (;;) {
        while (l - f > 16u) {
            if (d == limit) {
                if (lane == 0)
                    urf_tie_heap_sort<typename MEM::rptr, typename MEM::iptr>(R, P, f, l);
                for (unsigned j = f + lane; j < l; j += 64) {
                    LP[j] = j;
                    RP[j] = j + 1;
                }
                MEM::sync();
                f = l;
                break;
            }
            d++;
            const unsigned cut = urf_tie_partition<MEM>(R, P, LP, RP, f, l);
            if (l - cut > 16u) {
                if (lane == 0) {
                    stk[3 * top] = (int)cut;
                    stk[3 * top + 1] = (int)l;
                    stk[3 * top + 2] = (int)d;
                }
                top++;
            } else {
                const unsigned j = cut + lane;
                if (j < l) {
                    LP[j] = cut;
                    RP[j] = l;
                }
            }
            l = cut;
        }
        if (l > f) {
            const unsigned j = f + lane;
            if (j < l) {
                LP[j] = f;
                RP[j] = l;
            }
        }
        if (top == 0)
            break;
        top--;
        urf_wave_lds_sync();
        f = (unsigned)stk[3 * top];
        l = (unsigned)stk[3 * top + 1];
        d = (unsigned)stk[3 * top + 2];
    }
    MEM::sync();
}

template <class MEM>
__device__ __forceinline__ unsigned urf_tie_select(unsigned n, unsigned target, typename MEM::rptr R, typename MEM::iptr P, typename MEM::iptr LP,
                                                   typename MEM::iptr RP)
{
    const unsigned lane = threadIdx.x;
    const unsigned limit = 2u * (31u - (unsigned)__clz((int)n));
    unsigned f = 0, l = n, d = 0;
    while (l - f > 16u) {
        if (d == limit) {
            if (lane == 0)
                urf_tie_heap_sort<typename MEM::rptr, typename MEM::iptr>(R, P, f, l);
            MEM::sync();
            return P[target];
        }
        d++;
        const unsigned cut = urf_tie_partition<MEM>(R, P, LP, RP, f, l);
        if (target < cut)
            l = cut;
        else
            f = cut;
    }
    const unsigned j = f + lane;
    unsigned rank = 0xffffffffu;
    if (j < l) {
        const unsigned v = R[j];
        rank = f;
        for (unsigned i = f; i < l; i++) {
            const unsigned u = R[i];
            rank += (u < v || (u == v && i < j)) ? 1u : 0u;
        }
    }
    const unsigned long long m = __ballot(rank == target);
    return P[f + (unsigned)__ffsll((long long)m) - 1u];
}

template <class MEM>
__device__ __forceinline__ unsigned urf_tie_final_rank(unsigned j, typename MEM::rptr R, typename MEM::iptr LP, typename MEM::iptr RP)
{
    const unsigned sa = LP[j], se = RP[j], v = R[j];
    unsigned rank = sa;
    for (unsigned i = sa; i < se; i++) {
        const unsigned u = R[i];
        rank += (u < v || (u == v && i < j)) ? 1u : 0u;
    }
    return rank;
}

template <class MEM, bool POST>
__device__ __forceinline__ void urf_tie_sector_body(const urf_kargs& a, const urf_dev_params& dp, unsigned sk, unsigned s, unsigned k, unsigned n,
                                                    unsigned hit_i, typename MEM::rptr R, typename MEM::iptr P, typename MEM::iptr LP,
                                                    typename MEM::iptr RP, int* stk)
{
    const unsigned lane = threadIdx.x, K = (unsigned)dp.p.sectors;
    const unsigned sb = urf_sbase(a, s), base = sb + a.sec_off[(size_t)s * (K + 1) + k];
    const urf_sec_run two = a.sec_run[sk];
    const bool simple = two.nruns <= 2;
    {
        unsigned nruns = 0;
        if (!simple) {
            unsigned off, len;
            urf_scan_range(a, s, off, len);
            nruns = urf_sector_runs(a, s, K, k, (len + URF_TILE - 1) / URF_TILE, urf_sector_run_row(a, s, K, k, 0), (unsigned*)LP, (unsigned*)RP);
            MEM::sync();
        }
        unsigned r = 0;
        for (unsigned i = lane; i < n; i += 64) {
            unsigned adr = i < two.c0 ? two.a0 + i : two.a1 + (i - two.c0);
            if (!simple) {
                while (r + 1 < nruns && i >= LP[r + 1])
                    r++;
                adr = RP[r] + i;
            }
            R[i] = urf_fbits(a.sr[sb + adr]);
            P[i] = adr;
        }
    }
    MEM::sync();
    if (a.front && a.front_ok[s] == URF_FRONT_ROWS) {
        for (unsigned i = lane; i < n; i += 64) {
            const unsigned adr = P[i];
            const unsigned sl = (unsigned)a.sslot[sb + adr] & (URF_TILE - 1u);
            LP[i] = ((sl & ((1u << a.front_lsh) - 1u)) << 16) | ((adr / URF_TILE) * (URF_TILE >> a.front_lsh) + (sl >> a.front_lsh));
        }
        MEM::sync();
        for (unsigned i = lane; i < n; i += 64) {
            const unsigned key = LP[i];
            unsigned rank = 0;
            for (unsigned j = 0; j < n; j++)
                rank += LP[j] < key ? 1u : 0u;
            RP[i] = rank;
        }
        MEM::sync();
        for (unsigned i = lane; i < n; i += 64)
            LP[RP[i]] = R[i];
        MEM::sync();
        for (unsigned i = lane; i < n; i += 64)
            R[i] = LP[i];
        MEM::sync();
        for (unsigned i = lane; i < n; i += 64)
            LP[RP[i]] = P[i];
        MEM::sync();
        for (unsigned i = lane; i < n; i += 64)
            P[i] = LP[i];
        MEM::sync();
    }
    if constexpr (POST) {
        const unsigned adr = urf_tie_select<MEM>(n, hit_i, R, P, LP, RP);
        const unsigned sl = a.sslot[sb + adr];
        const unsigned v = (sl & URF_SLOT_OFF) ? 0xffffffffu : (adr & ~(URF_TILE - 1u)) + sl;
        const int hit = urf_walk_slot_to_ring_pos(a, s, (unsigned)dp.p.channels, v);
        if (lane == 0) {
            a.star_hit[sk] = hit;
            a.star_first[sk] = 0;
        }
        MEM::sync();
        return;
    }
    urf_tie_introsort_loop<MEM>(n, R, P, LP, RP, stk);
    for (unsigned j = lane; j < n; j += 64)
        LP[j] = urf_tie_final_rank<MEM>(j, R, LP, RP);
    MEM::sync();
    for (unsigned j = lane; j < n; j += 64)
        RP[LP[j]] = P[j];
    MEM::sync();
    for (unsigned j = lane; j < n; j += 64)
        P[LP[j]] = R[j];
    MEM::sync();
    for (unsigned i = lane; i < n; i += 64)
        R[i] = __float_as_uint(a.sz[sb + RP[i]]);
    MEM::sync();
    const float slope_param = dp.slope_param, kdist = dp.p.kdist_param;
    const bool fmt16 = simple && n <= URF_STAR_MID_CAP_;
    unsigned first = n;
    for (unsigned i0 = 0; i0 < n; i0 += 64) {
        const unsigned i = i0 + lane;
        bool hit = false;
        if (i < n) {
            float slp = 0.f, g = 0.f;
            if (i >= 1) {
                const float ax = __uint_as_float(P[i - 1]), bx = __uint_as_float(P[i]);
                slp = (__uint_as_float(R[i]) - __uint_as_float(R[i - 1])) / (bx - ax);
                g = (bx - ax) * kdist;
                hit = slp > slope_param;
            }
            const unsigned adr = RP[i];
            if (fmt16) {
                a.ssrt16[base + i] = (uint16_t)((two.nruns == 2 && adr >= two.a1) ? two.c0 + (adr - two.a1) : adr - two.a0);
            } else {
                const unsigned sl = a.sslot[sb + adr];
                a.ssrt[base + i] = (sl & URF_SLOT_OFF) ? 0xffffffffu : (adr & ~(URF_TILE - 1u)) + sl;
            }
            a.wsg[base + i] = urf_sg{ slp, g };
        }
        const unsigned long long mh = __ballot(hit);
        if (mh) {
            first = i0 + (unsigned)__ffsll((long long)mh) - 1u;
            break;
        }
    }
    if (lane == 0)
        a.star_first[sk] = (first < n - 1 ? first : n - 1) | URF_TIE_DONE;
    MEM::sync();
}

#define URF_TIE_SMALL 512u
template <bool POST, unsigned CAP>
__global__ __launch_bounds__(64) void k_star_ties(urf_kargs a, urf_dev_params dp)
{
    __shared__ unsigned W[4 * CAP];
    __shared__ int stk[3 * 64];
    const unsigned count = a.star_count[POST ? 5 : 4];
    const unsigned K = (unsigned)dp.p.sectors;
    const uint32_t* const list = POST ? a.tie_post : a.tie_list;
    for (unsigned w = blockIdx.x; w < count; w += gridDim.x) {
        {
            const unsigned sk = list[w];
            const unsigned sf = a.star_first[sk];
            if (!(sf & (POST ? URF_TIE_POST : URF_TIE_FLAG)))
                continue;
            const unsigned hit_i = sf & URF_TIE_INDEX;
            const unsigned s = sk / K, k = sk % K;
            if (a.info[s].status != URF_OK)
                continue;
            const unsigned n = a.sec_cnt[sk];
            if (n < 2)
                continue;
            if (CAP == URF_TIE_SMALL ? n > URF_TIE_SMALL : n <= URF_TIE_SMALL)
                continue;
            if (n <= CAP) {
                urf_tie_sector_body<urf_tie_lds, POST>(a, dp, sk, s, k, n, hit_i, W, W + CAP, W + 2 * CAP, W + 3 * CAP, stk);
            } else {
                const unsigned base = urf_sbase(a, s) + a.sec_off[(size_t)s * (K + 1) + k];
                urf_tie_sector_body<urf_tie_glb, POST>(a, dp, sk, s, k, n, hit_i, (unsigned*)a.big_r + base, a.big_i + base,
                                                       (unsigned*)a.big_z + base, a.ssrt + base, stk);
            }
        }
    }
}

#define URF_WALK_CHUNK 16
struct urf_walk_state {
    float avg, dev, nan;
    unsigned hit_i;
    unsigned lim;
};
__device__ __forceinline__ float urf_mul_f32(float x, float y)
{
    float r;
    asm("v_mul_f32 %0, %1, %2" : "=v"(r) : "v"(x), "v"(y));
    return r;
}
__device__ __forceinline__ float urf_add_f32(float x, float y)
{
    float r;
    asm("v_add_f32 %0, %1, %2" : "=v"(r) : "v"(x), "v"(y));
    return r;
}
__device__ __forceinline__ float urf_add_absdiff_f32(float x, float y, float z)
{
    float d, r;
    asm("v_sub_f32 %0, %1, %2" : "=v"(d) : "v"(y), "v"(z));
    asm("v_add_f32_e64 %0, %1, |%2|" : "=v"(r) : "v"(x), "v"(d));
    return r;
}
template <bool ABOVE>
__device__ __forceinline__ bool urf_walk_chunk_fast(urf_walk_state& w_, unsigned c0, const urf_sg (&sg)[URF_WALK_CHUNK],
                                                    const urf_wu* __restrict__ wu, float kdev, float slope_param, int dmin)
{
    float avg = w_.avg, dev = w_.dev;
    const unsigned lim = w_.lim;
    bool h[URF_WALK_CHUNK];
#pragma unroll
    for (unsigned j = 0; j < URF_WALK_CHUNK; j++) {
        const unsigned i = c0 + j;
        h[j] = false;
        if (!ABOVE && j == 0 && c0 == 0)
            continue;
        const float slp = sg[j].slp;
        const float w = wu[j].w, u = wu[j].u;
        float na = avg * w;
        na = na + slp;
        na = na * u;
        float nd = dev * w;
        nd = nd + __builtin_fabsf(slp - na);
        nd = nd * u;
        avg = na;
        dev = nd;
        const bool dyn = urf_mul_f32(urf_mul_f32(urf_mul_f32(slp, slp) - urf_mul_f32(na, na), kdev), sg[j].g) > nd;
        h[j] = (slp > slope_param) | ((ABOVE || (int)i > dmin) & dyn);
    }
    if (__any(lim != 0u && avg != avg))
        return false;
    unsigned hit = 0;
#pragma unroll
    for (int j = URF_WALK_CHUNK - 1; j >= 0; j--)
        hit = h[j] ? c0 + (unsigned)j : hit;
    w_.avg = avg;
    w_.dev = dev;
    if (hit && hit <= lim) {
        w_.hit_i = hit;
        w_.lim = 0;
    }
    return true;
}
__device__ __forceinline__ void urf_walk_chunk_general(urf_walk_state& w_, unsigned c0, const urf_sg* sg , float kdev,
                                                       float slope_param, int dmin)
{
    float avg = w_.avg, dev = w_.dev, nan = w_.nan;
    unsigned hit_i = w_.hit_i, lim = w_.lim;
#pragma unroll 1
    for (unsigned j = 0; j < URF_WALK_CHUNK; j++) {
        const unsigned i = c0 + j;
        const bool active = i >= 1 && i <= lim;
        const float slp = sg[j].slp;
        if (active) {
            if (slp != slp) {
                nan += 1.0f;
            } else {
                const float w = (float)(int)i - nan - 1.0f;
                const float u = 1.0f / ((float)(int)i - nan);
                avg *= w;
                avg += slp;
                avg *= u;
                dev *= w;
                dev += __builtin_fabsf(slp - avg);
                dev *= u;
            }
        }
        const bool h = slp > slope_param ||
                       ((int)i > dmin && (slp * slp - avg * avg) * kdev * sg[j].g > dev);
        if (active && h) {
            hit_i = i;
            lim = 0;
        }
    }
    w_.avg = avg;
    w_.dev = dev;
    w_.nan = nan;
    w_.hit_i = hit_i;
    w_.lim = lim;
}

__device__ __forceinline__ int urf_walk_slot_to_ring_pos(const urf_kargs& a, unsigned s, unsigned C, unsigned v)
{
    int hit = -1;
    if (a.front && a.front_ok[s])
        return (int)v;
    if (v != 0xffffffffu) {
        const unsigned t = v / URF_TILE, j = v % URF_TILE;
        const uint16_t* row = a.troff + ((size_t)s * a.tiles + t) * (C + 1);
        unsigned lo = 0, hi = C;
        while (hi - lo > 1) {
            const unsigned mid = (lo + hi) >> 1;
            if ((unsigned)row[mid] <= j)
                lo = mid;
            else
                hi = mid;
        }
        const unsigned p = a.rpre[((size_t)s * C + lo) * (a.tiles + 1) + t] + (j - (unsigned)row[lo]);
        hit = (int)(a.ring_off[(size_t)s * (C + 1) + lo] + p);
    }
    return hit;
}
__device__ __forceinline__ int urf_walk_report(const urf_kargs& a, unsigned s, unsigned K, unsigned C, unsigned k, unsigned n, unsigned base,
                                               unsigned hit_i)
{
    int hit = -1;
    unsigned v = 0xffffffffu;
    if (hit_i && hit_i < n) {
        const urf_sec_run two = a.sec_run[(size_t)s * K + k];
        if (two.nruns <= 2 && n <= URF_STAR_MID_CAP_) {
            const unsigned i0 = a.ssrt16[base + hit_i];
            const unsigned adr = i0 < two.c0 ? two.a0 + i0 : two.a1 + (i0 - two.c0);
            const unsigned sl = a.sslot[urf_sbase(a, s) + adr];
            v = (sl & URF_SLOT_OFF) ? 0xffffffffu : (adr & ~(URF_TILE - 1u)) + sl;
        } else {
            v = a.ssrt[base + hit_i];
        }
    }
    hit = urf_walk_slot_to_ring_pos(a, s, C, v);
    return hit;
}

__global__ __launch_bounds__(256) void k_walk_table(urf_wu* tab, unsigned n)
{
    const unsigned i = blockIdx.x * 256 + threadIdx.x;
    if (i < n)
        tab[i] = i ? urf_wu{ (float)(int)i - 1.0f, 1.0f / (float)(int)i } : urf_wu{ 0.f, 0.f };
}

typedef urf_sg urf_walk_tile[64][URF_WALK_CHUNK + 2];
__shared__ urf_walk_tile walk_tile;
__shared__ unsigned walk_sbase[64], walk_slast[64];

__device__ __forceinline__ void urf_walk_sequential(urf_walk_state& W, unsigned c_start, unsigned last, unsigned maxlast, const urf_sg* __restrict__ wsg,
                                                    const urf_wu* __restrict__ tab, unsigned lane, float kdev, float slope_param, int dmin)
{
    urf_walk_tile& tile = walk_tile;
    const unsigned* sbase = walk_sbase;
    const unsigned* slast = walk_slast;
    urf_sg v[16];
    unsigned fo[16], fe[16];
#pragma unroll
    for (unsigned r = 0; r < 16; r++) {
        const unsigned sec = r * 4 + (lane >> 4);
        fo[r] = sbase[sec] + (lane & 15);
        fe[r] = sbase[sec] + slast[sec];
    }
    auto fetch = [&](unsigned c0) {
#pragma unroll
        for (unsigned r = 0; r < 16; r++) {
            const unsigned e = fo[r] + c0;
            v[r] = wsg[e < fe[r] ? e : fe[r]];
        }
    };
    auto park = [&]() {
#pragma unroll
        for (unsigned r = 0; r < 16; r++)
            tile[r * 4 + (lane >> 4)][lane & 15] = v[r];
    };
    fetch(c_start);
    park();
    urf_wave_lds_sync();
    for (unsigned c0 = c_start; c0 <= maxlast; c0 += URF_WALK_CHUNK) {
        if (!__any(W.lim != 0))
            break;
        const bool more = c0 + URF_WALK_CHUNK <= maxlast;
        if (more)
            fetch(c0 + URF_WALK_CHUNK);
        urf_sg sg[URF_WALK_CHUNK];
        {
            const float4* row = reinterpret_cast<const float4*>(&tile[lane][0]);
#pragma unroll
            for (unsigned j = 0; j < URF_WALK_CHUNK / 2; j++) {
                const float4 q = row[j];
                sg[2 * j] = urf_sg{ q.x, q.y };
                sg[2 * j + 1] = urf_sg{ q.z, q.w };
            }
        }
        bool walked = false;
        if (!__any(W.nan != 0.0f))
            walked = (c0 != 0 && (int)c0 > dmin) ? urf_walk_chunk_fast<true>(W, c0, sg, tab + c0, kdev, slope_param, dmin)
                                                 : urf_walk_chunk_fast<false>(W, c0, sg, tab + c0, kdev, slope_param, dmin);
        if (!walked)
            urf_walk_chunk_general(W, c0, &tile[lane][0], kdev, slope_param, dmin);
        if (c0 + URF_WALK_CHUNK > last)
            W.lim = 0;
        urf_wave_lds_sync();
        if (more)
            park();
        urf_wave_lds_sync();
    }
}

struct urf_walk_sectors {
    unsigned k, n, base, last, maxlast, sf;
    bool have;
};
__device__ __forceinline__ void urf_walk_twins(const urf_kargs& a, unsigned s, unsigned K, unsigned k, unsigned n, unsigned base, unsigned sf,
                                               unsigned hit_i)
{
    if (hit_i == 0 || (sf & URF_TIE_DONE) || hit_i + 1 >= n)
        return;
    const float gn = a.wsg[base + hit_i + 1].g;
    const bool twin = hit_i == (sf & URF_TIE_INDEX) ? (sf & URF_TIE_NEXT) != 0u : !(gn > 0.0f || gn < 0.0f);
    if (!twin)
        return;
    a.star_first[(size_t)s * K + k] = URF_TIE_POST | hit_i;
    a.tie_post[atomicAdd(&a.star_count[5], 1u)] = s * K + k;
    if (a.optimistic & URF_OPT_NO_TIES)
        a.info[s].status = URF_STATUS_REDO_TIES;
}
__device__ __forceinline__ urf_walk_sectors urf_walk_prologue(const urf_kargs& a, unsigned s, unsigned K, unsigned lane, bool publish)
{
    unsigned* sbase = walk_sbase;
    unsigned* slast = walk_slast;
    urf_walk_sectors q;
    q.k = blockIdx.x * 64 + lane;
    q.have = q.k < K;
    q.n = q.have ? a.sec_cnt[(size_t)s * K + q.k] : 0;
    const unsigned rel = q.have ? a.sec_off[(size_t)s * (K + 1) + q.k] : 0;
    q.base = urf_sbase(a, s) + rel;
    q.sf = q.n >= 2 ? a.star_first[(size_t)s * K + q.k] : 0;
    q.last = q.sf & URF_TIE_INDEX;
    if (publish) {
        sbase[lane] = q.last ? rel : 0u;
        slast[lane] = q.last;
    }
    unsigned maxlast = q.last;
    for (int o = 32; o > 0; o >>= 1) {
        const unsigned w = __shfl_xor(maxlast, o);
        maxlast = w > maxlast ? w : maxlast;
    }
    q.maxlast = (unsigned)__builtin_amdgcn_readfirstlane((int)maxlast);
    return q;
}

__global__ __launch_bounds__(64) void k_star_walk(urf_kargs a, urf_dev_params dp)
{
    urf_walk_tile& tile = walk_tile;
    unsigned* sbase = walk_sbase;
    unsigned* slast = walk_slast;
    const unsigned K = (unsigned)dp.p.sectors;
    const unsigned s = blockIdx.y, lane = threadIdx.x;
    const unsigned k = blockIdx.x * 64 + lane;
    if (a.info[s].status != URF_OK)
        return;
    const unsigned C = (unsigned)dp.p.channels;
    const bool have = k < K;
    const unsigned n = have ? a.sec_cnt[(size_t)s * K + k] : 0;
    const unsigned rel = have ? a.sec_off[(size_t)s * (K + 1) + k] : 0;
    const unsigned base = urf_sbase(a, s) + rel;
    const unsigned sf = n >= 2 ? a.star_first[(size_t)s * K + k] : 0;
    const unsigned last = sf & URF_TIE_INDEX;
    sbase[lane] = last ? rel : 0u;
    slast[lane] = last;
    unsigned maxlast = last;
    for (int o = 32; o > 0; o >>= 1) {
        const unsigned w = __shfl_xor(maxlast, o);
        maxlast = w > maxlast ? w : maxlast;
    }
    maxlast = (unsigned)__builtin_amdgcn_readfirstlane((int)maxlast);
    __syncthreads();

    const urf_sg* __restrict__ wsg = a.wsg + urf_sbase(a, s);
    urf_sg v[16];
    unsigned fo[16], fe[16];
#pragma unroll
    for (unsigned r = 0; r < 16; r++) {
        const unsigned sec = r * 4 + (lane >> 4);
        fo[r] = sbase[sec] + (lane & 15);
        fe[r] = sbase[sec] + slast[sec];
    }
    auto fetch = [&](unsigned c0) {
#pragma unroll
        for (unsigned r = 0; r < 16; r++) {
            const unsigned e = fo[r] + c0;
            v[r] = wsg[e < fe[r] ? e : fe[r]];
        }
    };
    auto park = [&]() {
#pragma unroll
        for (unsigned r = 0; r < 16; r++)
            tile[r * 4 + (lane >> 4)][lane & 15] = v[r];
    };

    const float kdev = dp.p.kdev_param, slope_param = dp.slope_param;
    const int dmin = dp.p.dmin_param;
    urf_walk_state W = { 0.f, 0.f, 0.f, 0u, last };
    fetch(0);
    park();
    __syncthreads();
    for (unsigned c0 = 0; c0 <= maxlast; c0 += URF_WALK_CHUNK) {
        if (!__any(W.lim != 0))
            break;
        const bool more = c0 + URF_WALK_CHUNK <= maxlast;
        if (more)
            fetch(c0 + URF_WALK_CHUNK);
        urf_sg sg[URF_WALK_CHUNK];
        {
            const float4* row = reinterpret_cast<const float4*>(&tile[lane][0]);
#pragma unroll
            for (unsigned j = 0; j < URF_WALK_CHUNK / 2; j++) {
                const float4 q = row[j];
                sg[2 * j] = urf_sg{ q.x, q.y };
                sg[2 * j + 1] = urf_sg{ q.z, q.w };
            }
        }
        bool walked = false;
        if (!__any(W.nan != 0.0f))
            walked = (c0 != 0 && (int)c0 > dmin) ? urf_walk_chunk_fast<true>(W, c0, sg, a.walk_tab + c0, kdev, slope_param, dmin)
                                                 : urf_walk_chunk_fast<false>(W, c0, sg, a.walk_tab + c0, kdev, slope_param, dmin);
        if (!walked)
            urf_walk_chunk_general(W, c0, &tile[lane][0], kdev, slope_param, dmin);
        if (c0 + URF_WALK_CHUNK > last)
            W.lim = 0;
        __syncthreads();
        if (more)
            park();
        __syncthreads();
    }
    const int hit = urf_walk_report(a, s, K, C, k, n, base, W.hit_i);
    if (have) {
        a.star_hit[(size_t)s * K + k] = hit;
        urf_walk_twins(a, s, K, k, n, base, sf, W.hit_i);
    }
}

#define URF_WALK_FEW_THREADS 320
#ifndef URF_WALK_FEW_SCANS
#define URF_WALK_FEW_SCANS 32u
#endif
template <bool ABOVE>
__device__ __forceinline__ unsigned urf_walk_tests_quarter(unsigned i0, const urf_sg (&sg)[4], const float4 (&x)[2], float kdev, float slope_param, int dmin)
{
    float t[4], q[4];
#pragma unroll
    for (unsigned j = 0; j < 4; j++)
        t[j] = urf_mul_f32(sg[j].slp, sg[j].slp);
#pragma unroll
    for (unsigned j = 0; j < 4; j++) {
        const float na = (j & 1) ? x[j >> 1].z : x[j >> 1].x;
        q[j] = urf_mul_f32(na, na);
    }
#pragma unroll
    for (unsigned j = 0; j < 4; j++)
        t[j] = t[j] - q[j];
#pragma unroll
    for (unsigned j = 0; j < 4; j++)
        t[j] = urf_mul_f32(t[j], kdev);
#pragma unroll
    for (unsigned j = 0; j < 4; j++)
        t[j] = urf_mul_f32(t[j], sg[j].g);
    bool h[4];
#pragma unroll
    for (unsigned j = 0; j < 4; j++) {
        const unsigned i = i0 + j;
        const float nd = (j & 1) ? x[j >> 1].w : x[j >> 1].y;
        h[j] = (ABOVE || i != 0) & ((sg[j].slp > slope_param) | ((ABOVE || (int)i > dmin) & (t[j] > nd)));
    }
    unsigned hit = 0;
#pragma unroll
    for (int j = 3; j >= 0; j--)
        hit = h[j] ? i0 + (unsigned)j : hit;
    return hit;
}

__global__ __launch_bounds__(URF_WALK_FEW_THREADS) void k_star_walk_few(urf_kargs a, urf_dev_params dp)
{
    const unsigned* sbase = walk_sbase;
    const unsigned* slast = walk_slast;
    __shared__ urf_walk_tile tile2;
    __shared__ __attribute__((aligned(16))) float X[2][64][2 * URF_WALK_CHUNK + 4];
    __shared__ __attribute__((aligned(16))) unsigned hitb[2][64][4];
    __shared__ unsigned ctl[2], nan_at, fin_hit[64], fin_lim[64];
    const unsigned K = (unsigned)dp.p.sectors;
    const unsigned s = blockIdx.y, wave = (unsigned)__builtin_amdgcn_readfirstlane((int)(threadIdx.x >> 6)), lane = threadIdx.x & 63;
    if (__syncthreads_or(a.info[s].status != URF_OK))
        return;
    const urf_walk_sectors q = urf_walk_prologue(a, s, K, lane, wave == 0);
    if (threadIdx.x == 0) {
        nan_at = 0xffffffffu;
        ctl[0] = 1u;
        ctl[1] = 1u;
    }
    __syncthreads();
    const urf_sg* __restrict__ wsg = a.wsg + urf_sbase(a, s);
    const float kdev = dp.p.kdev_param, slope_param = dp.slope_param;
    const int dmin = dp.p.dmin_param;
    const unsigned last = q.last, nchunks = q.maxlast / URF_WALK_CHUNK + 1;
    const unsigned b = wave ? wave - 1u : 0u;

    urf_sg v[4];
    unsigned fo[4], fe[4];
#pragma unroll
    for (unsigned r = 0; r < 4; r++) {
        const unsigned sec = (4 * b + r) * 4 + (lane >> 4);
        fo[r] = sbase[sec] + (lane & 15);
        fe[r] = sbase[sec] + slast[sec];
    }
    auto fetch = [&](unsigned c0) {
#pragma unroll
        for (unsigned r = 0; r < 4; r++) {
            const unsigned e = fo[r] + c0;
            v[r] = wsg[e < fe[r] ? e : fe[r]];
        }
    };
    auto park = [&](urf_walk_tile& t) {
#pragma unroll
        for (unsigned r = 0; r < 4; r++)
            t[(4 * b + r) * 4 + (lane >> 4)][lane & 15] = v[r];
    };
    if (wave) {
        fetch(0);
// ... 127 lines not shown
```

urban_road_filter_amd/csrc/urf_k_table.hpp:

```cpp
#ifndef URF_K_TABLE_HPP
#define URF_K_TABLE_HPP

__global__ __launch_bounds__(256) void k_pc2_to_soa(const uint8_t* __restrict__ data, unsigned long long n_total,
                                                    unsigned step, unsigned ox, unsigned oy, unsigned oz,
                                                    float* __restrict__ x, float* __restrict__ y, float* __restrict__ z)
{
    const unsigned long long i = (unsigned long long)blockIdx.x * blockDim.x + threadIdx.x;
    if (i >= n_total)
        return;
    const uint8_t* p = data + i * step;
    float fx, fy, fz;
    if ((((unsigned long long)(p + ox) | (unsigned long long)(p + oy) | (unsigned long long)(p + oz)) & 3ull) == 0) {
        fx = *(const float*)(p + ox);
        fy = *(const float*)(p + oy);
        fz = *(const float*)(p + oz);
    } else {
        unsigned bx = 0, by = 0, bz = 0;
        for (int b = 3; b >= 0; b--) {
            bx = (bx << 8) | p[ox + b];
            by = (by << 8) | p[oy + b];
            bz = (bz << 8) | p[oz + b];
        }
        fx = __uint_as_float(bx);
        fy = __uint_as_float(by);
// ... 163 lines not shown
    __syncthreads();

    const float interval = dp.p.interval;
    const unsigned hint = (lookahead && a.table_hint) ? *a.ring_hint : 0u;
    unsigned pos = 0, upto = 0xffffffffu;
    unsigned cause = 0;
    auto insert64 = [&](const float v) {
            unsigned nL = sh_nL, nmatch = sh_nmatch;
            bool zero_seen = sh_zero != 0;
            const unsigned nL0 = nL;
            bool un = v >= 0.0f && !urf_leader_match(SL, nmatch, v, interval);
            unsigned long long m;
            m = __ballot(un);
            if (m != 0 && !zero_seen) {
                const unsigned long long below = m & ((1ull << lane) - 1ull);
                const unsigned rank = (unsigned)__popcll(below);
                const int prev = below ? 63 - __clzll((long long)below) : (int)lane;
                const float pv = __shfl(v, prev);
                const float floor_v = nmatch ? SL[nmatch - 1] : -1.0f;
                const bool ok = !un || (v != 0.0f && (below ? (v > pv && v - pv > interval) : v > floor_v));
                const unsigned cnt = (unsigned)__popcll(m);
                if (__ballot(!ok) == 0 && nL + cnt <= C) {
                    if (un) {
                        L[nL + rank] = v;
                        SL[nmatch + rank] = v;
                    }
                    nL += cnt;
                    nmatch += cnt;
                    un = false;
                }
            }
            if ((m = __ballot(un)) != 0 && !zero_seen && nmatch == 0 && nL + (unsigned)__popcll(m) <= C) {
                float* const stage = SL + 64;
                stage[lane] = un ? v : -1.0f;
                urf_wave_lds_sync();
                bool clash = un && v == 0.0f;
                unsigned srank = 0;
                for (unsigned j = 0; j < 64; j++) {
                    const float w = stage[j];
                    const bool there = w >= 0.0f;
                    clash = clash || (there && un && j < lane && __builtin_fabsf(w - v) <= interval);
                    srank += (there && (w < v || (w == v && j < lane))) ? 1u : 0u;
                }
                if (__ballot(clash) == 0) {
                    const unsigned cnt = (unsigned)__popcll(m);
                    if (un) {
                        L[nL + urf_popc_below(m)] = v;
                        SL[srank] = v;
                    }
                    nL += cnt;
                    nmatch += cnt;
                    un = false;
                }
                urf_wave_lds_sync();
            }
            while ((m = __ballot(un)) != 0 && nL < C) {
                const unsigned f = (unsigned)__ffsll((long long)m) - 1u;
                const float lv = __shfl(v, (int)f);
                bool matchable = false;
                if (lane == 0) {
                    L[nL] = lv;
                    if (!zero_seen && lv != 0.0f) {
                        unsigned k = nmatch;
                        while (k > 0 && SL[k - 1] > lv) {
                            SL[k] = SL[k - 1];
                            k--;
                        }
                        SL[k] = lv;
                    }
                }
                if (!zero_seen) {
                    if (lv == 0.0f)
                        zero_seen = true;
                    else {
                        nmatch++;
                        matchable = true;
                    }
                }
                nL++;
                if (lane <= f)
                    un = false;
                else if (matchable && __builtin_fabsf(lv - v) <= interval)
                    un = false;
            }
            if (lane == 0) {
                sh_nL = nL;
                sh_nmatch = nmatch;
                sh_zero = zero_seen ? 1u : 0u;
                sh_new = nL != nL0;
                if (nL0 == 0u && nL != 0u)
                    T.first_nl = zero_seen ? 0xffffu : nL;
            }
    };
    bool rows = false;
    bool rows_try = first_walk && (a.front || a.front_sight) && C == (1u << a.front_lsh) && len >= 2u * C && (len & (C - 1u)) == 0u;
    if (rows_try && a.front_rows) {
        const unsigned nr = a.rows_ok[s];
        if (nr) {
            if (tid < nr - 1u)
                L[tid] = a.rows_v[(size_t)s * 64u + tid];
            if (tid == 0) {
                sh_nL = nr - 1u;
                a.front_ok[s] = URF_FRONT_ROWS;
                a.flags[URF_FLAG_ROWS_TAKEN] = 1u;
            }
            rows = true;
            upto = 0;
            cause = 3;
            __syncthreads();
        }
    }
    while (!rows && pos < len && sh_nL < C) {
        if (hint && pos && sh_nL >= hint && !sh_zero) {
            upto = pos;
            cause = 2;
            break;
        }
        if (wave == 0) {
            const unsigned i = pos + lane;
            float v = -1.0f;
            if (i < len) {
                const float x = a.x[off + i], y = a.y[off + i], z = a.z[off + i];
                if (urf_in_roi(dp.p, x, y, z))
                    v = urf_vertical_angle(x, y, z);
            }
            insert64(v);
        }
        __syncthreads();
        pos += 64;
        if (sh_new || sh_nL >= C)
            continue;
        const unsigned nmatch = sh_nmatch;
        unsigned quiet = 0;
        while (pos < len) {
            unsigned first = 0xffffffffu;
            float px[URF_TABLE_SCAN_PPT], py[URF_TABLE_SCAN_PPT], pz[URF_TABLE_SCAN_PPT];
#pragma unroll
            for (unsigned q = 0; q < URF_TABLE_SCAN_PPT; q++) {
                const unsigned i = pos + q * URF_TABLE_THREADS + tid;
                const bool on = i < len;
                px[q] = on ? a.x[off + i] : 0.f;
                py[q] = on ? a.y[off + i] : 0.f;
                pz[q] = on ? a.z[off + i] : 0.f;
            }
            {
                const float e = URF_FAST_VALPHA_ERR + 2.0e-5f;
                float vt[URF_TABLE_SCAN_PPT];
                unsigned lb[URF_TABLE_SCAN_PPT], okm = 0, roim = 0;
#pragma unroll
                for (unsigned q = 0; q < URF_TABLE_SCAN_PPT; q++) {
                    const unsigned i = pos + q * URF_TABLE_THREADS + tid;
                    roim |= (unsigned)((i < len) & urf_in_roi(dp.p, px[q], py[q], pz[q])) << q;
                }
                if (__ballot(roim != 0u) != 0ull) {
#pragma unroll
                for (unsigned q = 0; q < URF_TABLE_SCAN_PPT; q++) {
                    okm |= (unsigned)urf_fast_vertical_angle(px[q], py[q], pz[q], &vt[q]) << q;
                    lb[q] = 0;
                }
#pragma unroll
                for (unsigned step = URF_MAX_CHANNELS / 2; step > 0; step >>= 1) {
                    float sv[URF_TABLE_SCAN_PPT];
#pragma unroll
                    for (unsigned q = 0; q < URF_TABLE_SCAN_PPT; q++)
                        sv[q] = SL[(lb[q] + step - 1) & (URF_MAX_CHANNELS - 1)];
#pragma unroll
                    for (unsigned q = 0; q < URF_TABLE_SCAN_PPT; q++)
                        lb[q] += (lb[q] + step - 1 < nmatch && !(sv[q] - vt[q] >= -(interval + e))) ? step : 0u;
                }
                float cv[URF_TABLE_SCAN_PPT];
#pragma unroll
                for (unsigned q = 0; q < URF_TABLE_SCAN_PPT; q++)
                    cv[q] = SL[lb[q] & (URF_MAX_CHANNELS - 1)];
#pragma unroll
                for (unsigned q = 0; q < URF_TABLE_SCAN_PPT; q++)
                    lb[q] += (lb[q] == URF_MAX_CHANNELS - 1 && lb[q] < nmatch && !(cv[q] - vt[q] >= -(interval + e))) ? 1u : 0u;
#pragma unroll
                for (unsigned q = 0; q < URF_TABLE_SCAN_PPT; q++) {
                    const unsigned i = pos + q * URF_TABLE_THREADS + tid;
                    if (!((roim >> q) & 1u))
                        continue;
                    const float d = cv[q] - vt[q];
                    const bool fast = (okm >> q) & 1u;
                    const bool none = lb[q] >= nmatch || d > interval + e;
                    const bool sure = !none && __builtin_fabsf(d) <= interval - e;
                    bool matched;
                    if (fast && (none || sure))
                        matched = sure;
                    else
                        matched = urf_leader_match(SL, nmatch, urf_vertical_angle(px[q], py[q], pz[q]), interval);
                    if (!matched && i < first)
                        first = i;
                }
                }
            }
            for (int o = 32; o > 0; o >>= 1) {
                const unsigned w = __shfl_xor(first, o);
                first = w < first ? w : first;
            }
            if (lane == 0)
                sh_min[wave] = first;
            __syncthreads();
            unsigned m = sh_min[0];
            for (int w = 1; w < URF_TABLE_THREADS / 64; w++)
                m = sh_min[w] < m ? sh_min[w] : m;
            __syncthreads();
            if (m != 0xffffffffu) {
                pos = m;
                break;
            }
            pos += URF_TABLE_THREADS * URF_TABLE_SCAN_PPT;
            quiet += URF_TABLE_THREADS * URF_TABLE_SCAN_PPT;
            if (lookahead && quiet >= lookahead && !sh_zero && pos < len) {
                upto = pos;
                cause = 1;
                break;
            }
        }
        if (upto != 0xffffffffu)
            break;
    }
    __syncthreads();
    if (rows_try && !a.front_rows && !rows) {
        const unsigned nl = T.first_nl;
        if (nl != 0u && nl * (len >> a.front_lsh) <= 63u + (len >> a.front_lsh)) {
            if (tid == 0)
                a.flags[URF_FLAG_ROWS_SIGHTED] = 1u;
            cause |= 4u;
        }
    }
    if (tid == 0) {
        a.table_upto[s] = upto;
        a.table_redo[s] = 0;
        a.table_cause[s] = cause;
    }

    const unsigned n = sh_nL;
    if (tid < n) {
        const float v = L[tid];
        unsigned rank = 0;
        for (unsigned j = 0; j < n; j++) {
            const float w = L[j];
            rank += (w < v) || (w == v && j < tid);
        }
        a.angle[(size_t)s * C + rank] = v;
        SL[rank] = v;
    }
    if (tid == 0)
        a.info[s].n_rings = n;
    __syncthreads();
    {
        const float e = URF_FAST_VALPHA_ERR + 2.0e-5f;
        for (unsigned k = tid; k < 4 * n; k += URF_TABLE_THREADS) {
            const float t = urf_ring_threshold(SL[k >> 2], interval, e, k & 3u);
            a.ring_thr[((size_t)s * C) * 4 + k] = t;
            if ((k & 3u) == 0)
                L[k >> 2] = t;
        }
        __syncthreads();
        uint8_t* lut = a.ring_lut + (size_t)s * URF_LUT_CELLS;
        for (unsigned c0 = tid; c0 < URF_LUT_CELLS; c0 += 4 * URF_TABLE_THREADS) {
            float u1[4];
            unsigned lo[4];
#pragma unroll
            for (unsigned q = 0; q < 4; q++) {
                u1[q] = (float)(c0 + q * URF_TABLE_THREADS + 1) * (1.0f / URF_LUT_SCALE) - URF_LUT_UMAX;
                lo[q] = 0;
            }
#pragma unroll
            for (unsigned step = URF_MAX_CHANNELS; step > 0; step >>= 1) {
                float lv[4];
#pragma unroll
                for (unsigned q = 0; q < 4; q++)
                    lv[q] = L[(lo[q] + step - 1) & (URF_MAX_CHANNELS - 1)];
#pragma unroll
                for (unsigned q = 0; q < 4; q++)
                    lo[q] += (lo[q] + step - 1 < n && lv[q] >= u1[q]) ? step : 0u;
            }
#pragma unroll
            for (unsigned q = 0; q < 4; q++)
                if (c0 + q * URF_TABLE_THREADS < URF_LUT_CELLS)
                    lut[c0 + q * URF_TABLE_THREADS] = (uint8_t)lo[q];
        }
    }
}

__global__ __launch_bounds__(URF_TABLE_THREADS) void k_ring_table(urf_kargs a, urf_dev_params dp)
{
    __shared__ urf_table_shared T;
    if (blockIdx.x == 0 && threadIdx.x < 8)
        a.star_count[threadIdx.x] = 0;
    {
        const unsigned s = blockIdx.x, tid = threadIdx.x;
        if (tid == 0) {
            a.front_ok[s] = a.front;
            a.front_ncand[s] = 0;
        }
        if (a.front) {
            if (tid < 64)
                a.front_lane_ring[(size_t)s * 64 + tid] = 0xffffffffu;
            if (tid < (unsigned)dp.p.channels)
                a.front_ring_lane[(size_t)s * dp.p.channels + tid] = 0xffffffffu;
        }
    }
    urf_ring_table_scan(a, dp, blockIdx.x, a.table_lookahead, T, true);
}

__global__ __launch_bounds__(URF_TABLE_THREADS) void k_table_repair(urf_kargs a, urf_dev_params dp, unsigned collect)
{
    __shared__ urf_table_shared T;
    const unsigned s = blockIdx.x;
    const bool redo = a.table_redo[s] != 0u;
    if (collect && threadIdx.x == 0 && (redo || a.front_ok[s] == 0u)) {
        a.front_ok[s] = 0u;
        const unsigned e = atomicAdd(&a.star_count[6], 1u);
        a.front_list[e] = s;
        a.flags[URF_FLAG_FRONT_HANDED_BACK] = 1u;
        if (e + 1u == a.n_scans)
            a.flags[URF_FLAG_FRONT_ALL_HANDED_BACK] = 1u;
    }
    if (!redo)
        return;
    if (a.front && threadIdx.x == 0)
        a.front_ok[s] = 0u;
    const unsigned cause = a.table_cause[s];
    urf_ring_table_scan(a, dp, s, 0, T, false);
    if (threadIdx.x == 0) {
        if (!collect)
            a.redo_list[atomicAdd(&a.star_count[2], 1u)] = s;
        if (cause != 3u && !(cause & 4u))
            a.flags[cause == 2u ? URF_FLAG_HINT_FAILED : URF_FLAG_LOOKAHEAD_FAILED] = 1u;
    }
}


#endif
```

Baseline: 492,900 scans/s.

## Sort star-shaped sectors in place from source points instead of scattered copies

In the 64-ring front path with the star-shaped detector, the front kernel no longer writes per-point range, height and slot arrays into sector-sorted scratch. Instead it records, for each sector, which firings (64-point columns) contribute, up to six. The star sort and walk kernels then reread x/y/z directly from the source or row-major buffers, recompute range with a square root, and recover point indices through the firing list. This removes three scattered stores per point and their later reads, at the cost of recomputing sqrt, doing readlane-based index lookups, and falling back when a sector spans more than six firings or its participants differ from its ROI word.

```diff
diff --git a/urban_road_filter_amd/csrc/urf_api.hip b/urban_road_filter_amd/csrc/urf_api.hip
--- a/urban_road_filter_amd/csrc/urf_api.hip
+++ b/urban_road_filter_amd/csrc/urf_api.hip
@@ -50,6 +50,7 @@
     X(angle, URF_MAX_CHANNELS) X(ring_thr, URF_MAX_CHANNELS * 4) X(ring_lut, URF_LUT_CELLS) X(ring_cnt, URF_MAX_CHANNELS)        \
     X(ring_off, URF_MAX_CHANNELS + 1)                                                                                            \
     X(sec_cnt, URF_MAX_SECTORS) X(sec_run, URF_MAX_SECTORS) X(sec_off, URF_MAX_SECTORS + 1) X(star_hit, URF_MAX_SECTORS)         \
+    X(sec_nfir, URF_MAX_SECTORS) X(sec_firs, URF_MAX_SECTORS * 8)                                                                \
     X(star_first, URF_MAX_SECTORS) X(star_list_mid, URF_MAX_SECTORS) X(star_list_big, URF_MAX_SECTORS)                           \
     X(star_list_runs, URF_MAX_SECTORS) X(tie_list, URF_MAX_SECTORS) X(tie_post, URF_MAX_SECTORS)                                 \
     X(table_upto, 1) X(table_redo, 1) X(redo_list, 1) X(table_cause, 1)                                                          \
@@ -130,6 +131,8 @@
         a.front_tpb = front_tpb ? front_tpb : (a.n_scans >= URF_FRONT_TPB_SCANS ? URF_FRONT_TPB_LARGE : (a.n_scans >= 16u ? URF_FRONT_TPB_SMALL : 1u));
         a.front_lists = (a.front && !front_direct && !slot) ? 1u : 0u;
         a.front_rows = (a.front && front_rows) ? 1u : 0u;
+        a.star_inplace = (a.front && !slot && a.front_lsh == 6u && dp.p.star_shaped_method && !dp.p.starbeam_filter &&
+                          !(dp.exp_flags & URF_EXP_NO_INPLACE)) ? 1u : 0u;
     }
 };
 
diff --git a/urban_road_filter_amd/csrc/urf_device.hpp b/urban_road_filter_amd/csrc/urf_device.hpp
--- a/urban_road_filter_amd/csrc/urf_device.hpp
+++ b/urban_road_filter_amd/csrc/urf_device.hpp
@@ -371,4 +371,15 @@
 
 __device__ __forceinline__ unsigned urf_fbits(float f) { return __float_as_uint(f); }
 
+#define URF_FRONT_RING_NONE 0x7fu
+
+__device__ __forceinline__ void urf_front_src(const urf_kargs& a, unsigned s, unsigned off, unsigned ok, const float*& gx, const float*& gy, const float*& gz)
+{
+    const bool rows = ok == URF_FRONT_ROWS;
+    const size_t o = rows ? (size_t)urf_sbase(a, s) : (size_t)off;
+    gx = (rows ? (const float*)a.tx : a.x) + o;
+    gy = (rows ? (const float*)a.ty : a.y) + o;
+    gz = (rows ? (const float*)a.tz : a.z) + o;
+}
+
 #endif
diff --git a/urban_road_filter_amd/csrc/urf_front.hpp b/urban_road_filter_amd/csrc/urf_front.hpp
--- a/urban_road_filter_amd/csrc/urf_front.hpp
+++ b/urban_road_filter_amd/csrc/urf_front.hpp
@@ -14,7 +14,6 @@
 #define URF_FRONT_TPB_LARGE 4u
 #define URF_FRONT_TPB_SCANS 512u
 #define URF_FRONT_MAX_TILES 128u
-#define URF_FRONT_RING_NONE 0x7fu
 #define URF_FC_XZ 1u
 #define URF_FC_ZZ 2u
 #define URF_FC_EDGE_X 4u
@@ -47,14 +46,6 @@
 }
 #define URF_OOB 0xffffffffu
 
-__device__ __forceinline__ void urf_front_src(const urf_kargs& a, unsigned s, unsigned off, unsigned ok, const float*& gx, const float*& gy, const float*& gz)
-{
-    const bool rows = ok == URF_FRONT_ROWS;
-    const size_t o = rows ? (size_t)urf_sbase(a, s) : (size_t)off;
-    gx = (rows ? (const float*)a.tx : a.x) + o;
-    gy = (rows ? (const float*)a.ty : a.y) + o;
-    gz = (rows ? (const float*)a.tz : a.z) + o;
-}
 
 __global__ __launch_bounds__(256) void k_transpose(urf_kargs a)
 {
@@ -147,7 +138,7 @@
     ncb += (unsigned)__popcll(m);
 }
 
-template <bool STAR, bool BEAM, unsigned L>
+template <bool STAR, bool BEAM, unsigned L, bool INPLACE = false>
 __device__ __forceinline__ void urf_front_body(const urf_kargs& a, const urf_dev_params& dp, urf_u2* cbuf)
 {
     const unsigned s = blockIdx.y, b = blockIdx.x, lane = threadIdx.x;
@@ -163,6 +154,7 @@
     constexpr unsigned C = L;
     constexpr unsigned STEPS = URF_TILE / L;
     static_assert(L == 64u || L == 32u || L == 16u, "a firing fills the wave, half of it or a quarter");
+    static_assert(!INPLACE || (STAR && !BEAM && L == 64u), "in place: a firing's participants are its region-of-interest points, one word of roi_bits");
     const unsigned K = (unsigned)dp.p.sectors;
     const unsigned nf = (len + L - 1u) / L;
     const unsigned F0 = t_first * STEPS;
@@ -257,13 +249,17 @@
                 const unsigned src = psm ? (unsigned)__ffsll((long long)psm) - 1u : 0u;
                 const unsigned f0 = psm ? (unsigned)__builtin_amdgcn_readlane((int)sk, (int)src) : URF_SEC_NONE;
                 failed_m |= psm & __builtin_amdgcn_ballot_w64(sk != f0);
-                const unsigned so = (f / STEPS) * URF_TILE + tstar + urf_popc_below(psm);
-                const unsigned o4 = ons ? so * 4u : URF_OOB;
-                const float pr = urf_sqrt_rn_normal(rho2);
                 failed_m |= psm & ~(__builtin_amdgcn_ballot_w64(rho2 >= 0x1p-90f) & __builtin_amdgcn_ballot_w64(rho2 <= 0x1p126f));
-                __builtin_amdgcn_raw_buffer_store_b32(__float_as_uint(pr), bsr, o4, 0, URF_FRONT_NT);
-                __builtin_amdgcn_raw_buffer_store_b32(__float_as_uint(z), bsz, o4, 0, URF_FRONT_NT);
-                __builtin_amdgcn_raw_buffer_store_b16((short)((stp * L + lane) | (on ? 0u : URF_SLOT_OFF)), bss, ons ? so * 2u : URF_OOB, 0, URF_FRONT_NT);
+                if (INPLACE) {
+                    failed_m |= psm ^ roim;
+                } else {
+                    const unsigned so = (f / STEPS) * URF_TILE + tstar + urf_popc_below(psm);
+                    const unsigned o4 = ons ? so * 4u : URF_OOB;
+                    const float pr = urf_sqrt_rn_normal(rho2);
+                    __builtin_amdgcn_raw_buffer_store_b32(__float_as_uint(pr), bsr, o4, 0, URF_FRONT_NT);
+                    __builtin_amdgcn_raw_buffer_store_b32(__float_as_uint(z), bsz, o4, 0, URF_FRONT_NT);
+                    __builtin_amdgcn_raw_buffer_store_b16((short)((stp * L + lane) | (on ? 0u : URF_SLOT_OFF)), bss, ons ? so * 2u : URF_OOB, 0, URF_FRONT_NT);
+                }
                 if (STEPS <= 64u || stp < 64u) {
                     stepkey_v = lane == stp ? (int)f0 : stepkey_v;
                     stepcnt_v = lane == stp ? (int)__popcll(psm) : stepcnt_v;
@@ -410,6 +406,14 @@
                 if (k <= K)
                     a.tsoff[row * (K + 1) + k] = (uint16_t)so;
             }
+            if (INPLACE && k1 != 0u) {
+                const size_t sk = (size_t)s * K + (k1 - 1u);
+                const unsigned e = atomicAdd(&a.sec_nfir[sk], 1u);
+                if (e < URF_INPLACE_FIRINGS)
+                    a.sec_firs[sk * 8u + e] = (uint16_t)(t * URF_FRONT_STEPS + lane);
+                else
+                    failed = true;
+            }
         }
         troi = 0;
         tstar = 0;
@@ -494,6 +498,8 @@
 {
     if (!dp.p.star_shaped_method)
         urf_front_body<false, false, L>(a, dp, cbuf);
+    else if (L == 64u && a.star_inplace)
+        urf_front_body<true, false, L, L == 64u>(a, dp, cbuf);
     else if (!dp.p.starbeam_filter)
         urf_front_body<true, false, L>(a, dp, cbuf);
     else
diff --git a/urban_road_filter_amd/csrc/urf_internal.hpp b/urban_road_filter_amd/csrc/urf_internal.hpp
--- a/urban_road_filter_amd/csrc/urf_internal.hpp
+++ b/urban_road_filter_amd/csrc/urf_internal.hpp
@@ -36,6 +36,8 @@
 #define URF_OPT_NO_LISTS 2u
 #define URF_OPT_NO_NAN 4u
 #define URF_OPT_NO_TIES 8u
+#define URF_EXP_NO_INPLACE 32u
+#define URF_INPLACE_FIRINGS 6u
 #define URF_STATUS_REDO_TABLE 0x7f000001
 #define URF_STATUS_REDO_LISTS 0x7f000002
 #define URF_STATUS_REDO_NAN 0x7f000003
@@ -112,7 +114,7 @@
     uint32_t  front;
     uint32_t  front_tpb;
     uint32_t  front_cand_cap;
-    uint32_t  front_pad_;
+    uint32_t  star_inplace;
     uint8_t* labels;
     urf_scan_info* info;
     float*    valpha;
@@ -145,6 +147,8 @@
     uint32_t* sec_cnt;
     urf_sec_run* sec_run;
     uint32_t* sec_off;
+    uint32_t* sec_nfir;
+    uint16_t* sec_firs;
     int32_t*  star_hit;
     uint32_t* star_first;
     uint32_t* star_list_mid;
diff --git a/urban_road_filter_amd/csrc/urf_k_split.hpp b/urban_road_filter_amd/csrc/urf_k_split.hpp
--- a/urban_road_filter_amd/csrc/urf_k_split.hpp
+++ b/urban_road_filter_amd/csrc/urf_k_split.hpp
@@ -918,8 +918,9 @@
         const unsigned k = k0 + tid;
         const unsigned c = k < K ? a.sec_cnt[(size_t)s * K + k] : 0;
         const unsigned nr = k < K ? a.sec_run[(size_t)s * K + k].nruns : 0;
-        const bool runs = (nr & URF_RUNS_FLAG) != 0u && c >= 2 && c <= URF_STAR_SMALL_CAP;
-        const bool mid = (c > URF_STAR_SMALL_CAP || (nr > 2 && c >= 2 && !runs)) && c <= URF_STAR_MID_CAP_, big = c > URF_STAR_MID_CAP_;
+        const bool listed = !(fused && a.star_inplace);
+        const bool runs = listed && (nr & URF_RUNS_FLAG) != 0u && c >= 2 && c <= URF_STAR_SMALL_CAP;
+        const bool mid = listed && (c > URF_STAR_SMALL_CAP || (nr > 2 && c >= 2 && !runs)) && c <= URF_STAR_MID_CAP_, big = listed && c > URF_STAR_MID_CAP_;
         const unsigned long long bm = __ballot(mid), bb = __ballot(big), br = __ballot(runs);
         unsigned pm = 0, pb = 0, pr = 0;
         if ((a.optimistic & URF_OPT_NO_LISTS) && (bm | bb | br) && urf_lane() == 0)
diff --git a/urban_road_filter_amd/csrc/urf_k_star.hpp b/urban_road_filter_amd/csrc/urf_k_star.hpp
--- a/urban_road_filter_amd/csrc/urf_k_star.hpp
+++ b/urban_road_filter_amd/csrc/urf_k_star.hpp
@@ -71,16 +71,78 @@
     return nr;
 }
 
-template <unsigned MAXB, bool RUNS = false>
+#define URF_SORT_PLAIN 0u
+#define URF_SORT_RUNS 1u
+#define URF_SORT_INPLACE 2u
+struct urf_inplace_sec {
+    const float *x, *y, *z;
+    unsigned last;
+    unsigned m;
+    unsigned vf, wlo, whi;
+};
+__device__ __forceinline__ unsigned urf_inplace_firing(const urf_inplace_sec& I, unsigned q)
+{
+    return (unsigned)__builtin_amdgcn_readlane((int)I.vf, (int)q);
+}
+__device__ __forceinline__ unsigned long long urf_inplace_word(const urf_inplace_sec& I, unsigned q)
+{
+    return ((unsigned long long)(unsigned)__builtin_amdgcn_readlane((int)I.whi, (int)q) << 32) | (unsigned)__builtin_amdgcn_readlane((int)I.wlo, (int)q);
+}
+__device__ __forceinline__ unsigned urf_inplace_index(const urf_inplace_sec& I, unsigned o)
+{
+    const unsigned q = o >> 6;
+    unsigned f = urf_inplace_firing(I, 0u);
+#pragma unroll
+    for (unsigned j = 1; j < URF_INPLACE_FIRINGS; j++)
+        f = q == j ? urf_inplace_firing(I, j) : f;
+    return f * 64u + (o & 63u);
+}
+template <bool SORT>
+__device__ __forceinline__ void urf_inplace_load(const urf_kargs& a, unsigned s, unsigned sk, unsigned ok, urf_inplace_sec& I)
+{
+    const unsigned lane = urf_lane();
+    unsigned off, len;
+    urf_scan_range(a, s, off, len);
+    urf_front_src(a, s, off, ok, I.x, I.y, I.z);
+    I.last = len - 1u;
+    const unsigned m_raw = a.sec_nfir[sk];
+    I.m = (unsigned)__builtin_amdgcn_readfirstlane((int)(m_raw < URF_INPLACE_FIRINGS ? m_raw : URF_INPLACE_FIRINGS));
+    unsigned v = lane < I.m ? (unsigned)a.sec_firs[(size_t)sk * 8u + lane] : 0xffffffffu;
+    if (SORT) {
+        unsigned rank = 0;
+#pragma unroll
+        for (unsigned j = 0; j < URF_INPLACE_FIRINGS; j++)
+            rank += (unsigned)__builtin_amdgcn_readlane((int)v, (int)j) < v ? 1u : 0u;
+        if (lane < I.m)
+            a.sec_firs[(size_t)sk * 8u + rank] = (uint16_t)v;
+        unsigned sorted = 0xffffffffu;
+#pragma unroll
+        for (unsigned j = 0; j < URF_INPLACE_FIRINGS; j++) {
+            const unsigned vj = (unsigned)__builtin_amdgcn_readlane((int)v, (int)j), rj = (unsigned)__builtin_amdgcn_readlane((int)rank, (int)j);
+            sorted = (j < I.m && lane == rj) ? vj : sorted;
+        }
+        v = sorted;
+    }
+    const unsigned long long* const words = a.roi_bits + (size_t)s * a.tiles * (URF_TILE / 64u);
+    const unsigned long long w = lane < I.m ? words[v] : 0ull;
+    I.vf = lane < I.m ? v : (unsigned)__builtin_amdgcn_readlane((int)v, 0);
+    I.wlo = (unsigned)w;
+    I.whi = (unsigned)(w >> 32);
+}
+
+template <unsigned MAXB, unsigned MODE = URF_SORT_PLAIN>
 __device__ __forceinline__ bool urf_star_sort_sector(const urf_kargs& a, const urf_dev_params& dp, unsigned sb, unsigned obase, unsigned n,
                                                      const urf_sec_run& two, unsigned long long* A, unsigned* cnt,
-                                                     unsigned* sh_first, uint32_t* star_first_out, unsigned run_adr = 0, unsigned run_cnt = 0)
-{
+                                                     unsigned* sh_first, uint32_t* star_first_out, unsigned run_adr, unsigned run_cnt,
+                                                     const urf_inplace_sec& inp)
+{
+    constexpr bool RUNS = MODE == URF_SORT_RUNS, INPLACE = MODE == URF_SORT_INPLACE;
+    static_assert(!INPLACE || MAXB == URF_INPLACE_FIRINGS, "one firing per round");
     constexpr unsigned NB = URF_STAR_NB, PL = NB / 64;
     auto CI = [](unsigned c) { return c; };
     const unsigned lane = threadIdx.x;
     const unsigned Bn = (n + 63) >> 6;
-    const unsigned B = RUNS ? urf_wave_max(run_cnt) : Bn;
+    const unsigned B = RUNS ? urf_wave_max(run_cnt) : (INPLACE ? inp.m : Bn);
     URF_PHASE_ACC_DECL;
     unsigned long long key[MAXB];
     float zreg[MAXB];
@@ -93,7 +155,29 @@
         for (unsigned q = 0; q < MAXB; q++) {
             const unsigned i = q * 64 + lane, ic = i < n ? i : n - 1u;
             adr[q] = RUNS ? run_adr + (q < run_cnt ? q : 0u) : ic + (ic < two.c0 ? two.a0 : a1m);
-        }
+            if (INPLACE)
+                adr[q] = i;
+        }
+        if (INPLACE) {
+            float px[MAXB], py[MAXB];
+#pragma unroll
+            for (unsigned q = 0; q < MAXB; q++) {
+                px[q] = 0.f;
+                py[q] = 0.f;
+                zreg[q] = 0.f;
+                if (q < B) {
+                    const unsigned i = urf_inplace_firing(inp, q) * 64u + lane, ic = i < inp.last ? i : inp.last;
+                    px[q] = inp.x[ic];
+                    py[q] = inp.y[ic];
+                    zreg[q] = inp.z[ic];
+                }
+            }
+#pragma unroll
+            for (unsigned q = 0; q < MAXB; q++) {
+                rbv[q] = urf_fbits(urf_sqrt_rn_normal(px[q] * px[q] + py[q] * py[q]));
+                slv[q] = 0;
+            }
+        } else {
 #pragma unroll
         for (unsigned q = 0; q < MAXB; q++) {
             rbv[q] = 0;
@@ -106,9 +190,12 @@
                     slv[q] = a.sslot[sb + adr[q]];
             }
         }
+        }
 #pragma unroll
         for (unsigned q = 0; q < MAXB; q++) {
-            const bool valid = RUNS ? q < run_cnt : q * 64 + lane < n;
+            bool valid = RUNS ? q < run_cnt : q * 64 + lane < n;
+            if (INPLACE)
+                valid = q < B && ((urf_inplace_word(inp, q) >> lane) & 1ull) != 0ull;
             sreg[q] = RUNS ? ((slv[q] & URF_SLOT_OFF) ? 0xffffffffu : (adr[q] & ~(URF_TILE - 1u)) + slv[q]) : q * 64 + lane;
             key[q] = valid ? ((unsigned long long)rbv[q] << 32) | adr[q] : ~0ull;
             rmin = valid && rbv[q] < rmin ? rbv[q] : rmin;
@@ -244,8 +331,13 @@
                 A[q * 64 + lane] = key[q];
                 if (key[q] != ~0ull) {
                     const unsigned adr = (unsigned)key[q];
-                    zreg[q] = a.sz[sb + adr];
-                    if (RUNS) {
+                    if (INPLACE)
+                        zreg[q] = inp.z[urf_inplace_index(inp, adr)];
+                    else
+                        zreg[q] = a.sz[sb + adr];
+                    if (INPLACE) {
+                        sreg[q] = adr;
+                    } else if (RUNS) {
                         const unsigned sl = a.sslot[sb + adr];
                         sreg[q] = (sl & URF_SLOT_OFF) ? 0xffffffffu : (adr & ~(URF_TILE - 1u)) + sl;
                     } else {
@@ -347,7 +439,8 @@
     if (status != URF_OK)
         return;
     const unsigned n = so1 - so0;
-    if (n > URF_STAR_SMALL_CAP || (two.nruns > 2 && n >= 2))
+    const unsigned ok = a.star_inplace ? a.front_ok[s] : 0u;
+    if (n > URF_STAR_SMALL_CAP || (!ok && two.nruns > 2 && n >= 2))
         return;
     if (n < 2) {
         if (lane == 0)
@@ -357,7 +450,14 @@
     const unsigned sb = urf_sbase(a, s), obase = sb + so0;
     if (lane == 0)
         sh_first = n;
-    const bool tie = urf_star_sort_sector<URF_STAR_SMALL_CAP / 64>(a, dp, sb, obase, n, two, A, cnt, &sh_first, &a.star_first[(size_t)s * K + k]);
+    bool tie;
+    if (ok) {
+        urf_inplace_sec I;
+        urf_inplace_load<true>(a, s, s * K + k, ok, I);
+        tie = urf_star_sort_sector<URF_STAR_SMALL_CAP / 64, URF_SORT_INPLACE>(a, dp, sb, obase, n, two, A, cnt, &sh_first, &a.star_first[(size_t)s * K + k], 0u, 0u, I);
+    } else {
+        tie = urf_star_sort_sector<URF_STAR_SMALL_CAP / 64>(a, dp, sb, obase, n, two, A, cnt, &sh_first, &a.star_first[(size_t)s * K + k], 0u, 0u, urf_inplace_sec{});
+    }
     if (tie && lane == 0)
         urf_tie_found(a, s, s * K + k);
 }
@@ -389,8 +489,8 @@
         const unsigned sb = urf_sbase(a, s), obase = sb + so0;
         if (lane == 0)
             sh_first = n;
-        const bool tie = urf_star_sort_sector<URF_STAR_SMALL_CAP / 64, true>(a, dp, sb, obase, n, two, A, cnt, &sh_first, &a.star_first[sk],
-                                                                              c1 > c0 ? lane * URF_TILE + c0 : 0u, c1 - c0);
+        const bool tie = urf_star_sort_sector<URF_STAR_SMALL_CAP / 64, URF_SORT_RUNS>(a, dp, sb, obase, n, two, A, cnt, &sh_first, &a.star_first[sk],
+                                                                              c1 > c0 ? lane * URF_TILE + c0 : 0u, c1 - c0, urf_inplace_sec{});
         if (tie && lane == 0)
             urf_tie_found(a, s, sk);
         __syncthreads();
@@ -1103,8 +1203,44 @@
     const unsigned lane = threadIdx.x, K = (unsigned)dp.p.sectors;
     const unsigned sb = urf_sbase(a, s), base = sb + a.sec_off[(size_t)s * (K + 1) + k];
     const urf_sec_run two = a.sec_run[sk];
-    const bool simple = two.nruns <= 2;
-    {
+    const unsigned ok = a.star_inplace ? a.front_ok[s] : 0u;
+    const bool inplace = ok != 0u;
+    const bool simple = inplace || two.nruns <= 2;
+    urf_inplace_sec I;
+    if (inplace)
+        urf_inplace_load<false>(a, s, sk, ok, I);
+    auto range_of = [&](unsigned adr) {
+        if (inplace) {
+            const unsigned i = urf_inplace_index(I, adr);
+            const float x = I.x[i], y = I.y[i];
+            return urf_fbits(urf_sqrt_rn_normal(x * x + y * y));
+        }
+        return urf_fbits(a.sr[sb + adr]);
+    };
+    auto height_of = [&](unsigned adr) { return __float_as_uint(inplace ? I.z[urf_inplace_index(I, adr)] : a.sz[sb + adr]); };
+    auto slot_of = [&](unsigned adr) {
+        if (inplace) {
+            const unsigned i = urf_inplace_index(I, adr);
+            return (a.rec[sb + i] & 0x7fu) == URF_FRONT_RING_NONE ? 0xffffffffu : i;
+        }
+        const unsigned sl = a.sslot[sb + adr];
+        return (sl & URF_SLOT_OFF) ? 0xffffffffu : (adr & ~(URF_TILE - 1u)) + sl;
+    };
+    if (inplace) {
+        unsigned at = 0;
+#pragma unroll
+        for (unsigned q = 0; q < URF_INPLACE_FIRINGS; q++) {
+            const unsigned long long w = urf_inplace_word(I, q);
+            if ((w >> lane) & 1ull) {
+                const unsigned i = at + urf_popc_below(w);
+                if (i < n) {
+                    R[i] = range_of(q * 64u + lane);
+                    P[i] = q * 64u + lane;
+                }
+            }
+            at += (unsigned)__popcll(w);
+        }
+    } else {
         unsigned nruns = 0;
         if (!simple) {
             unsigned off, len;
@@ -1128,6 +1264,10 @@
     if (a.front && a.front_ok[s] == URF_FRONT_ROWS) {
         for (unsigned i = lane; i < n; i += 64) {
             const unsigned adr = P[i];
+            if (inplace) {
+                LP[i] = ((adr & 63u) << 16) | (urf_inplace_index(I, adr) >> 6);
+                continue;
+            }
             const unsigned sl = (unsigned)a.sslot[sb + adr] & (URF_TILE - 1u);
             LP[i] = ((sl & ((1u << a.front_lsh) - 1u)) << 16) | ((adr / URF_TILE) * (URF_TILE >> a.front_lsh) + (sl >> a.front_lsh));
         }
@@ -1155,8 +1295,7 @@
     }
     if constexpr (POST) {
         const unsigned adr = urf_tie_select<MEM>(n, hit_i, R, P, LP, RP);
-        const unsigned sl = a.sslot[sb + adr];
-        const unsigned v = (sl & URF_SLOT_OFF) ? 0xffffffffu : (adr & ~(URF_TILE - 1u)) + sl;
+        const unsigned v = slot_of(adr);
         const int hit = urf_walk_slot_to_ring_pos(a, s, (unsigned)dp.p.channels, v);
         if (lane == 0) {
             a.star_hit[sk] = hit;
@@ -1176,7 +1315,7 @@
         P[LP[j]] = R[j];
     MEM::sync();
     for (unsigned i = lane; i < n; i += 64)
-        R[i] = __float_as_uint(a.sz[sb + RP[i]]);
+        R[i] = height_of(RP[i]);
     MEM::sync();
     const float slope_param = dp.slope_param, kdist = dp.p.kdist_param;
     const bool fmt16 = simple && n <= URF_STAR_MID_CAP_;
@@ -1193,11 +1332,12 @@
                 hit = slp > slope_param;
             }
             const unsigned adr = RP[i];
-            if (fmt16) {
+            if (inplace) {
+                a.ssrt16[base + i] = (uint16_t)adr;
+            } else if (fmt16) {
                 a.ssrt16[base + i] = (uint16_t)((two.nruns == 2 && adr >= two.a1) ? two.c0 + (adr - two.a1) : adr - two.a0);
             } else {
-                const unsigned sl = a.sslot[sb + adr];
-                a.ssrt[base + i] = (sl & URF_SLOT_OFF) ? 0xffffffffu : (adr & ~(URF_TILE - 1u)) + sl;
+                a.ssrt[base + i] = slot_of(adr);
             }
             a.wsg[base + i] = urf_sg{ slp, g };
         }
@@ -1378,7 +1518,12 @@
     unsigned v = 0xffffffffu;
     if (hit_i && hit_i < n) {
         const urf_sec_run two = a.sec_run[(size_t)s * K + k];
-        if (two.nruns <= 2 && n <= URF_STAR_MID_CAP_) {
+        if (a.star_inplace && a.front_ok[s]) {
+            const unsigned o = a.ssrt16[base + hit_i];
+            v = (unsigned)a.sec_firs[((size_t)s * K + k) * 8u + (o >> 6)] * 64u + (o & 63u);
+            if ((a.rec[urf_sbase(a, s) + v] & 0x7fu) == URF_FRONT_RING_NONE)
+                v = 0xffffffffu;
+        } else if (two.nruns <= 2 && n <= URF_STAR_MID_CAP_) {
             const unsigned i0 = a.ssrt16[base + hit_i];
             const unsigned adr = i0 < two.c0 ? two.a0 + i0 : two.a1 + (i0 - two.c0);
             const unsigned sl = a.sslot[urf_sbase(a, s) + adr];
diff --git a/urban_road_filter_amd/csrc/urf_k_table.hpp b/urban_road_filter_amd/csrc/urf_k_table.hpp
--- a/urban_road_filter_amd/csrc/urf_k_table.hpp
+++ b/urban_road_filter_amd/csrc/urf_k_table.hpp
@@ -489,6 +489,9 @@
             if (tid < (unsigned)dp.p.channels)
                 a.front_ring_lane[(size_t)s * dp.p.channels + tid] = 0xffffffffu;
         }
+        if (a.star_inplace)
+            for (unsigned k = tid; k < (unsigned)dp.p.sectors; k += URF_TABLE_THREADS)
+                a.sec_nfir[(size_t)s * dp.p.sectors + k] = 0;
     }
     urf_ring_table_scan(a, dp, blockIdx.x, a.table_lookahead, T, true);
 }
```

Result: slower. 485,400 scans/s (-1.5%).
